# apache/cloudberry

Measured on NVIDIA H100. Metric: TPC-H SF100 Q1 rows/sec, higher is better.
Workload: dtype int64

## Files before the change

### cloudberry_b200/capi.py

```python
import ctypes as C
import os
import re

import numpy as np

from . import plan as P
from .relation import HostRelation, NP_DTYPE

HERE = os.path.dirname(os.path.abspath(__file__))
ROOT = os.path.dirname(HERE)
_GPU = None
_EXEC = None


class CbgpuError(RuntimeError):
    def __init__(self, code, msg):
        super().__init__("cbgpu error %d: %s" % (code, msg))
        self.code = code


class CbgpuVisimapEntry(C.Structure):
    _fields_ = [("first_row_num", C.c_int64), ("data", C.c_void_p), ("len", C.c_int32)]


# ... 222 lines not shown
    global _GPU
    if _GPU is None:
        so = os.path.join(os.environ.get("CBGPU_LIBDIR") or HERE, "libcbgpu.so")
        if not os.path.exists(so):
            raise CbgpuError(-1, "libcbgpu.so is not built (run __graft_entry__.build()); there is no CPU fallback")
        _preload_bundled_nccl()
        L = C.CDLL(so, mode=C.RTLD_GLOBAL)
        vp, i32, i64, u64, dbl = C.c_void_p, C.c_int32, C.c_int64, C.c_uint64, C.c_double
        sig = {
            "cbgpu_ctx_create": (C.c_int, [C.c_int, C.POINTER(vp)]),
            "cbgpu_ctx_destroy": (None, [vp]),
            "cbgpu_last_error": (C.c_char_p, [vp]),
            "cbgpu_sync": (C.c_int, [vp]),
            "cbgpu_check_status": (C.c_int, [vp]),
            "cbgpu_device_count": (C.c_int, []),
            "cbgpu_sm_count": (C.c_int, [vp]),
            "cbgpu_kernel_launches": (i64, [vp]),
            "cbgpu_timer_start": (C.c_int, [vp]),
            "cbgpu_timer_stop_ms": (C.c_int, [vp, C.POINTER(dbl)]),
            "cbgpu_last_kernel_ms": (dbl, [vp]),
            "cbgpu_last_kernel_name": (C.c_char_p, [vp]),
            "cbgpu_kernel_log_reset": (None, [vp]),
            "cbgpu_kernel_log_longest": (C.c_int, [vp, C.c_char_p, C.c_int, C.POINTER(dbl)]),
            "cbgpu_trace_begin": (C.c_int, [vp]),
            "cbgpu_trace_end": (C.c_int, [vp]),
            "cbgpu_trace_get": (C.c_int, [vp, C.c_int, C.c_char_p, C.c_int, C.POINTER(dbl)]),
            "cbgpu_flush_l2": (C.c_int, [vp]),
            "cbgpu_host_alloc": (vp, [C.c_size_t]),
            "cbgpu_host_free": (None, [vp]),
            "cbgpu_hashbpchar": (C.c_uint32, [C.c_char_p, i32]),
            "cbgpu_rel_create": (C.c_int, [vp, i64, i32, C.POINTER(i32), C.POINTER(i32), C.POINTER(vp)]),
            "cbgpu_rel_free": (None, [vp]),
            "cbgpu_rel_nrows": (i64, [vp]),
            "cbgpu_rel_ncols": (i32, [vp]),
            "cbgpu_rel_col_type": (i32, [vp, i32]),
            "cbgpu_rel_col_dscale": (i32, [vp, i32]),
            "cbgpu_rel_load_column": (C.c_int, [vp, i32, vp, vp]),
            "cbgpu_rel_load_column_narrow": (C.c_int, [vp, i32, vp, i32]),
            "cbgpu_rel_read_column": (C.c_int, [vp, i32, i64, i64, vp, vp]),
            "cbgpu_rel_set_visimap": (C.c_int, [vp, vp]),
            "cbgpu_rel_read_visimap": (C.c_int, [vp, vp]),
            "cbgpu_dict_create": (C.c_int, [vp, i32, i64, i32, C.POINTER(vp)]),
            "cbgpu_dict_free": (None, [vp]),
            "cbgpu_aocs_dict_collect": (C.c_int, [vp, vp, i64, i32, i32, i32, vp]),
            "cbgpu_dict_finalize": (C.c_int, [vp, C.POINTER(i32)]),
            "cbgpu_dict_entry": (C.c_int, [vp, i32, C.POINTER(C.c_char_p), C.POINTER(i32)]),
            "cbgpu_dict_lookup": (i32, [vp, C.c_char_p, i32]),
            "cbgpu_aocs_decode_dict_column": (C.c_int, [vp, vp, i64, i32, i32, i32, vp, vp, i32, i64, C.POINTER(i64)]),
            "cbgpu_aocs_apply_visimap": (C.c_int, [vp, vp, i64, i32, vp, i32, vp, i64, C.POINTER(i64)]),
            "cbgpu_rel_set_dict_hash": (C.c_int, [vp, i32, vp, i32]),
            "cbgpu_rel_set_nrows": (C.c_int, [vp, i64]),
            "cbgpu_rel_copy_rows": (C.c_int, [vp, i64, vp, i64, i64]),
            "cbgpu_rel_col_devptr": (vp, [vp, i32]),
            "cbgpu_rel_nbytes": (C.c_size_t, [vp]),
            "cbgpu_ht_build": (C.c_int, [vp, vp, C.POINTER(i32), i32, C.POINTER(vp)]),
            "cbgpu_ht_free": (None, [vp]),
            "cbgpu_ht_nrows": (i64, [vp]),
            "cbgpu_ht_has_duplicates": (C.c_int, [vp]),
            "cbgpu_ht_probe_pairs": (C.c_int, [vp, vp, vp, C.POINTER(i32), i32, vp, i64, vp]),
            "cbgpu_pairs_free": (None, [vp]),
            "cbgpu_merge_sorted_runs": (C.c_int, [vp, vp, C.POINTER(i32), C.POINTER(i32), C.POINTER(i32), i32, i32, C.POINTER(vp),
                                                  C.POINTER(i32)]),
            "cbgpu_dev_free": (None, [vp, vp]),
            "cbgpu_read_u32": (C.c_int, [vp, vp, i64, vp]),
            "cbgpu_motion_unique_id": (C.c_int, [vp]),
            "cbgpu_motion_create": (C.c_int, [vp, C.c_int, C.c_int, vp, C.POINTER(vp)]),
            "cbgpu_motion_create_boot": (C.c_int, [vp, C.c_int, C.c_int, vp, vp, C.POINTER(vp)]),
            "cbgpu_motion_destroy": (None, [vp]),
            "cbgpu_motion_abort": (None, [vp]),
            "cbgpu_motion_host_syncs": (i64, [vp]),
            "cbgpu_motion_collectives": (i64, [vp]),
            "cbgpu_motion_bytes_sent": (i64, [vp]),
            "cbgpu_motion_direct_bytes": (i64, [vp]),
            "cbgpu_motion_direct_available": (C.c_int, [vp]),
            "cbgpu_gen_lineitem": (C.c_int, [vp, vp, u64, i64, i64, i64]),
            "cbgpu_gen_orders": (C.c_int, [vp, vp, u64, i64, i64]),
            "cbgpu_gen_customer": (C.c_int, [vp, vp, u64]),
            "cbgpu_gen_supplier": (C.c_int, [vp, vp, u64]),
            "cbgpu_aocs_decode_column": (C.c_int, [vp, vp, i64, i32, i32, i32, i32, vp, i32, i64, C.POINTER(i64)]),
            "cbgpu_aocs_decode_column_ex": (C.c_int, [vp, vp, i64, i32, i32, i32, i32, i32, vp, i32, i64, C.POINTER(i64)]),
            "cbgpu_gen_customer_range": (C.c_int, [vp, vp, u64, i64]),
            "cbgpu_gen_supplier_range": (C.c_int, [vp, vp, u64, i64]),
            "cbgpu_gen_ssb_lineorder": (C.c_int, [vp, vp, u64, i64, i64, i64, i64]),
        }
        for name, (res, args) in sig.items():
            f = getattr(L, name)
            f.restype = res
            f.argtypes = args
        _GPU = L
    return _GPU


def ex():
    global _EXEC
    if _EXEC is None:
        gpu()
        so = os.path.join(os.environ.get("CBGPU_LIBDIR") or HERE, "libcbexec.so")
        if not os.path.exists(so):
            raise CbgpuError(-1, "libcbexec.so is not built (run __graft_entry__.build())")
        L = C.CDLL(so)
        vp = C.c_void_p
        L.cb_CreateExecutorState.restype = C.POINTER(CbEState)
        L.cb_CreateExecutorState.argtypes = [vp, C.POINTER(vp), C.c_int32]
        L.cb_FreeExecutorState.argtypes = [C.POINTER(CbEState)]
        L.cb_estate_error.restype = C.c_char_p
        L.cb_estate_error.argtypes = [C.POINTER(CbEState)]
# ... 474 lines not shown
```

### cloudberry_b200/csrc/agg.cu

```cuda
#include "common.cuh"

#include <stdlib.h>

static int64_t
next_pow2(int64_t v)
{
	int64_t		p = 1;

	while (p < v)
		p <<= 1;
	return p;
}

struct AggKinds
{
	int32_t		k[CBP_MAX_AGGS];
};

__global__ void
k_agg_init(AggDev t, const AggKinds kk)
{
	const int32_t *kinds = kk.k;
	size_t		cap = (size_t) t.mask + 1;
	size_t		i = (size_t) blockIdx.x * blockDim.x + threadIdx.x;
// ... 403 lines not shown
	int			rc = cbgpu_agg_ngroups(t, &ng);
	int32_t		types[CBP_MAX_KEYS + CBP_MAX_AGGS * 3];
	int			ncols = t->d.nkeys + t->d.naccs * 3;
	cbgpu_rel  *rel;
	AggRelOut	o;
	int			h_flag = 0;

	if (rc)
		return rc;
	for (int k = 0; k < t->d.nkeys; k++)
		types[k] = keytypes[k];
	for (int a = 0; a < t->d.naccs * 3; a++)
		types[t->d.nkeys + a] = CB_INT8;
	rc = cbgpu_rel_create(ctx, ng, ncols, types, NULL, &rel);
	if (rc)
		return rc;
	memset(&o, 0, sizeof(o));
	int			blocks = (int) ((t->capacity + 255) / 256);

	if (blocks > ctx->sm_count * 8)
		blocks = ctx->sm_count * 8;
	h_flag = t->anynull;
	for (int k = 0; k < t->d.nkeys; k++)
	{
		o.key[k] = rel->data[k];
		o.keytype[k] = keytypes[k];
		if (h_flag && ng > 0)
		{
			CB_CUDA(ctx, cudaMallocAsync(&rel->nulls[k], (size_t) ng, ctx->stream));
			o.keynulls[k] = rel->nulls[k];
		}
	}
	for (int a = 0; a < t->d.naccs * 3; a++)
		o.acc[a] = (int64_t *) rel->data[t->d.nkeys + a];
	CB_CUDA(ctx, cudaMallocAsync(&o.counter, sizeof(int32_t), ctx->stream));
	CB_CUDA(ctx, cudaMemsetAsync(o.counter, 0, sizeof(int32_t), ctx->stream));
	if (ng > 0)
	{
		k_agg_to_rel<<<blocks, 256, 0, ctx->stream>>>(t->d, o);
		CB_LAUNCHED(ctx, "k_agg_to_rel");
	}
	CB_CUDA(ctx, cudaFreeAsync(o.counter, ctx->stream));
	*out = rel;
	return CBGPU_OK;
}

#define TOPN_MAXK 64
#define TOPN_MAXKEYS 4

struct TopnParams
{
	const void *key[TOPN_MAXKEYS];
	int32_t		keytype[TOPN_MAXKEYS];
	int32_t		desc[TOPN_MAXKEYS];
	int32_t		uns[TOPN_MAXKEYS];
	int32_t		nkeys;
	int32_t		k;
	const uint32_t *in_idx;
	int64_t		nin;
	uint32_t   *out_idx;
};

__device__ __forceinline__ bool
topn_before(const TopnParams &p, const int64_t *ka, uint32_t ra, const int64_t *kb, uint32_t rb)
{
	for (int i = 0; i < p.nkeys; i++)
	{
		int64_t		x = ka[i],
					y = kb[i];

		if (x == y)
			continue;
		bool		lt = p.uns[i] ? ((uint64_t) x < (uint64_t) y) : (x < y);

		return p.desc[i] ? !lt : lt;
	}
	return ra < rb;
}

__global__ void
k_topn(TopnParams p)
{
	uint32_t	best_row[TOPN_MAXK];
	int64_t		best_key[TOPN_MAXK][TOPN_MAXKEYS];
	int			nbest = 0;
	int64_t		tid = (int64_t) blockIdx.x * blockDim.x + threadIdx.x;
	int64_t		stride = (int64_t) gridDim.x * blockDim.x;

	for (int64_t i = tid; i < p.nin; i += stride)
	{
		uint32_t	row = p.in_idx ? p.in_idx[i] : (uint32_t) i;
		int64_t		key[TOPN_MAXKEYS];

		if (row == 0xFFFFFFFFu)
			continue;
		for (int k = 0; k < p.nkeys; k++)
			key[k] = cb_load_widen(p.key[k], p.keytype[k], row);
		if (nbest == p.k && !topn_before(p, key, row, best_key[nbest - 1], best_row[nbest - 1]))
			continue;
		int			pos = nbest < p.k ? nbest : p.k - 1;

		while (pos > 0 && topn_before(p, key, row, best_key[pos - 1], best_row[pos - 1]))
		{
			best_row[pos] = best_row[pos - 1];
			for (int k = 0; k < p.nkeys; k++)
				best_key[pos][k] = best_key[pos - 1][k];
			pos--;
		}
		best_row[pos] = row;
		for (int k = 0; k < p.nkeys; k++)
			best_key[pos][k] = key[k];
		if (nbest < p.k)
			nbest++;
	}
	for (int j = 0; j < p.k; j++)
		p.out_idx[tid * p.k + j] = j < nbest ? best_row[j] : 0xFFFFFFFFu;
}

#define TOPN_BLOCKS 1024
#define TOPN_CAND 4096

__device__ __forceinline__ unsigned long long
topn_ukey(const TopnParams &p, int i, uint32_t row)
{
	unsigned long long u = (unsigned long long) cb_load_widen(p.key[i], p.keytype[i], row);

	if (!p.uns[i])
		u ^= 0x8000000000000000ull;
	return p.desc[i] ? ~u : u;
}

__global__ void __launch_bounds__(256)
k_topn_min(TopnParams p, int keyi, unsigned long long *bmin, unsigned long long *bmax)
{
	__shared__ unsigned long long smin[8], smax[8];
	unsigned long long lo = ~0ull,
				hi = 0;

	for (int64_t i = (int64_t) blockIdx.x * blockDim.x + threadIdx.x; i < p.nin; i += (int64_t) gridDim.x * blockDim.x)
	{
		const unsigned long long u = topn_ukey(p, keyi, (uint32_t) i);

		lo = u < lo ? u : lo;
		hi = u > hi ? u : hi;
	}
	for (int o = 16; o > 0; o >>= 1)
	{
		const unsigned long long a = __shfl_xor_sync(0xffffffffu, lo, o);
		const unsigned long long b = __shfl_xor_sync(0xffffffffu, hi, o);

		lo = a < lo ? a : lo;
		hi = b > hi ? b : hi;
	}
	if ((threadIdx.x & 31) == 0)
	{
		smin[threadIdx.x >> 5] = lo;
		smax[threadIdx.x >> 5] = hi;
	}
	__syncthreads();
	if (threadIdx.x == 0)
	{
		for (int w = 1; w < 8; w++)
		{
			lo = smin[w] < lo ? smin[w] : lo;
			hi = smax[w] > hi ? smax[w] : hi;
		}
		bmin[blockIdx.x] = lo;
		bmax[blockIdx.x] = hi;
	}
}

__global__ void __launch_bounds__(TOPN_BLOCKS)
k_topn_kth(const unsigned long long *bmin, const unsigned long long *bmax, int nblocks, int k, unsigned long long *out)
{
	__shared__ unsigned long long v[TOPN_BLOCKS];
	__shared__ unsigned long long gmax;
	const int	t = threadIdx.x;

// ... 14 lines not shown

			if (partner > t)
			{
				const bool	up = (t & size) == 0;
				const unsigned long long a = v[t],
							b = v[partner];

				if ((a > b) == up)
				{
					v[t] = b;
					v[partner] = a;
				}
			}
			__syncthreads();
		}
	if (t == 0)
	{
		out[0] = nblocks >= k ? v[k - 1] : gmax;
		out[1] = v[0];
		out[2] = gmax;
	}
}

__global__ void __launch_bounds__(256)
k_topn_filter(TopnParams p, int keyi, const unsigned long long *thr, uint32_t *cand, int *ncand)
{
	const unsigned long long T = thr[0];

	for (int64_t i = (int64_t) blockIdx.x * blockDim.x + threadIdx.x; i < p.nin; i += (int64_t) gridDim.x * blockDim.x)
		if (topn_ukey(p, keyi, (uint32_t) i) <= T)
		{
			const int	pos = atomicAdd(ncand, 1);

			if (pos < TOPN_CAND)
				cand[pos] = (uint32_t) i;
		}
}

__global__ void __launch_bounds__(1024)
k_topn_final(TopnParams p, const uint32_t *cand, const int *ncand, int64_t nall, uint32_t *out)
{
	const int	m = cand ? (*ncand < TOPN_CAND ? *ncand : TOPN_CAND) : (int) nall;

	for (int j = threadIdx.x; j < p.k; j += blockDim.x)
		out[j] = 0xFFFFFFFFu;
	__syncthreads();
	for (int i = threadIdx.x; i < m; i += blockDim.x)
	{
		const uint32_t ri = cand ? cand[i] : (uint32_t) i;
		int64_t		ki[TOPN_MAXKEYS];
		int			rank = 0;

		for (int k = 0; k < p.nkeys; k++)
			ki[k] = cb_load_widen(p.key[k], p.keytype[k], ri);
		for (int j = 0; j < m && rank < p.k; j++)
		{
			const uint32_t rj = cand ? cand[j] : (uint32_t) j;
			int64_t		kj[TOPN_MAXKEYS];

			if (j == i)
				continue;
			for (int k = 0; k < p.nkeys; k++)
				kj[k] = cb_load_widen(p.key[k], p.keytype[k], rj);
			rank += topn_before(p, kj, rj, ki, ri);
		}
		if (rank < p.k)
			out[rank] = ri;
	}
}

#define MERGE_MAXRUNS 64

struct MergeParams
{
	const void *key[TOPN_MAXKEYS];
	const uint8_t *nulls[TOPN_MAXKEYS];
	int32_t		keytype[TOPN_MAXKEYS];
	int32_t		desc[TOPN_MAXKEYS];
	int32_t		uns[TOPN_MAXKEYS];
	int32_t		nkeys;
	int32_t		nruns;
	int64_t		n;
	int64_t		start[MERGE_MAXRUNS + 1];
	int32_t    *nfound;
	unsigned long long *found;
	uint32_t   *order;
};

__device__ __forceinline__ int
merge_cmp(const MergeParams &p, int64_t a, int64_t b)
{
	for (int i = 0; i < p.nkeys; i++)
	{
		const bool	an = p.nulls[i] && p.nulls[i][a];
		const bool	bn = p.nulls[i] && p.nulls[i][b];
		int			c;

		if (an || bn)
			c = (an && bn) ? 0 : (an ? 1 : -1);
		else
		{
			const int64_t x = cb_load_widen(p.key[i], p.keytype[i], (uint32_t) a);
			const int64_t y = cb_load_widen(p.key[i], p.keytype[i], (uint32_t) b);

			if (x == y)
				c = 0;
			else if (p.uns[i])
				c = (uint64_t) x < (uint64_t) y ? -1 : 1;
			else
				c = x < y ? -1 : 1;
		}
		if (p.desc[i])
			c = -c;
		if (c)
			return c;
	}
	return 0;
}

__global__ void
k_merge_find_runs(MergeParams p)
{
	int64_t		i = (int64_t) blockIdx.x * blockDim.x + threadIdx.x + 1;
	const int64_t stride = (int64_t) gridDim.x * blockDim.x;

	for (; i < p.n; i += stride)
		if (merge_cmp(p, i, i - 1) < 0)
		{
			const int	at = atomicAdd(p.nfound, 1);

			if (at < MERGE_MAXRUNS)
				p.found[at] = (unsigned long long) i;
		}
}

__global__ void
k_merge_place(MergeParams p)
{
	int64_t		i = (int64_t) blockIdx.x * blockDim.x + threadIdx.x;
	const int64_t stride = (int64_t) gridDim.x * blockDim.x;

	for (; i < p.n; i += stride)
	{
		int			r = 0;
		int64_t		pos;

		while (r + 1 < p.nruns && p.start[r + 1] <= i)
			r++;
		pos = i - p.start[r];
		for (int q = 0; q < p.nruns; q++)
		{
			int64_t		lo = p.start[q],
						hi = p.start[q + 1];

			if (q == r)
				continue;
			while (lo < hi)
			{
				const int64_t mid = lo + (hi - lo) / 2;
				const int	c = merge_cmp(p, mid, i);

				if (c < 0 || (c == 0 && q < r))
					lo = mid + 1;
				else
					hi = mid;
			}
			pos += lo - p.start[q];
		}
		p.order[pos] = (uint32_t) i;
	}
}

extern "C" int
cbgpu_merge_sorted_runs(cbgpu_ctx *ctx, cbgpu_rel *rel, const int32_t *keycols, const int32_t *descending, const int32_t *unsigned_cmp,
						int32_t nkeys, int32_t max_runs, uint32_t **order_dev, int32_t *nruns_out)
{
	MergeParams p;
	int32_t		nfound = 0;
	unsigned long long found[MERGE_MAXRUNS];
	int			blocks;

	*order_dev = NULL;
	if (nruns_out)
		*nruns_out = rel->nrows > 0;
	if (nkeys < 1 || nkeys > TOPN_MAXKEYS || max_runs < 1 || max_runs > MERGE_MAXRUNS)
		return cb_fail(ctx, CBGPU_ERR_UNSUPPORTED, "merge receive supports 1..4 sort keys and up to 64 senders (%s got %lld keys)", "", nkeys);
	memset(&p, 0, sizeof(p));
	for (int i = 0; i < nkeys; i++)
	{
		if (keycols[i] < 0 || keycols[i] >= rel->ncols)
			return cb_fail(ctx, CBGPU_ERR_INVALID, "cbgpu_merge_sorted_runs: bad key column%s %lld", "", keycols[i]);
		p.key[i] = rel->data[keycols[i]];
		p.nulls[i] = rel->nulls[keycols[i]];
		p.keytype[i] = rel->types[keycols[i]];
		p.desc[i] = descending[i];
		p.uns[i] = unsigned_cmp ? unsigned_cmp[i] : 0;
		if (p.keytype[i] == CB_FLOAT8)
			return cb_fail(ctx, CBGPU_ERR_UNSUPPORTED, "merge receive over a float8 key%s", "", 0);
	}
	p.nkeys = nkeys;
	p.n = rel->nrows;
	if (rel->nrows < 2)
		return CBGPU_OK;
	blocks = (int) ((rel->nrows + 255) / 256);
	if (blocks > ctx->sm_count * 8)
		blocks = ctx->sm_count * 8;
	CB_CUDA(ctx, cudaMallocAsync(&p.nfound, sizeof(int32_t) + MERGE_MAXRUNS * sizeof(unsigned long long) + 8, ctx->stream));
	p.found = (unsigned long long *) ((char *) p.nfound + 8);
	CB_CUDA(ctx, cudaMemsetAsync(p.nfound, 0, sizeof(int32_t), ctx->stream));
	k_merge_find_runs<<<blocks, 256, 0, ctx->stream>>>(p);
	CB_LAUNCHED(ctx, "k_merge_find_runs");
	CB_CUDA(ctx, cudaMemcpyAsync(&nfound, p.nfound, sizeof(int32_t), cudaMemcpyDeviceToHost, ctx->stream));
	CB_CUDA(ctx, cudaMemcpyAsync(found, p.found, sizeof(found), cudaMemcpyDeviceToHost, ctx->stream));
	CB_CUDA(ctx, cudaStreamSynchronize(ctx->stream));
	CB_CUDA(ctx, cudaFreeAsync(p.nfound, ctx->stream));
	if (nfound + 1 > max_runs)
		return cb_fail(ctx, CBGPU_ERR_INVALID, "merge receive: %s%lld sorted runs arrived from fewer senders - a sender's stream is not in the Motion's sort order",
					   "", (long long) nfound + 1);
	if (nruns_out)
		*nruns_out = nfound + 1;
	if (nfound == 0)
		return CBGPU_OK;
	for (int a = 1; a < nfound; a++)
		for (int b = a; b > 0 && found[b] < found[b - 1]; b--)
		{
			unsigned long long t = found[b];

			found[b] = found[b - 1];
			found[b - 1] = t;
		}
	p.nruns = nfound + 1;
	p.start[0] = 0;
	for (int a = 0; a < nfound; a++)
		p.start[a + 1] = (int64_t) found[a];
	p.start[p.nruns] = rel->nrows;
	CB_CUDA(ctx, cudaMallocAsync(&p.order, (size_t) rel->nrows * sizeof(uint32_t), ctx->stream));
	k_merge_place<<<blocks, 256, 0, ctx->stream>>>(p);
	CB_LAUNCHED(ctx, "k_merge_place");
	*order_dev = p.order;
	return CBGPU_OK;
}

extern "C" int
cbgpu_topn(cbgpu_ctx *ctx, cbgpu_rel *rel, const int32_t *keycols, const int32_t *descending, const int32_t *unsigned_cmp,
		   int32_t nkeys, int64_t limit, uint32_t *host_idx, int64_t *nout)
{
	TopnParams	p;
	uint32_t   *cand1 = NULL,
			   *cand2 = NULL;
	int64_t		n1,
				n2;

	if (nkeys < 1 || nkeys > TOPN_MAXKEYS || limit < 1 || limit > TOPN_MAXK)
		return cb_fail(ctx, CBGPU_ERR_UNSUPPORTED, "device top-N supports 1..4 sort keys and LIMIT <= 64 (%s got %lld)", "", limit);
	memset(&p, 0, sizeof(p));
	for (int i = 0; i < nkeys; i++)
	{
		if (keycols[i] < 0 || keycols[i] >= rel->ncols)
			return cb_fail(ctx, CBGPU_ERR_INVALID, "cbgpu_topn: bad key column%s %lld", "", keycols[i]);
		if (rel->nulls[keycols[i]])
			return cb_fail(ctx, CBGPU_ERR_UNSUPPORTED, "device top-N over a nullable sort key (%s column %lld)", "", keycols[i]);
		p.key[i] = rel->data[keycols[i]];
		p.keytype[i] = rel->types[keycols[i]];
		p.desc[i] = descending[i];
		p.uns[i] = unsigned_cmp ? unsigned_cmp[i] : 0;
		if (p.keytype[i] == CB_FLOAT8)
			return cb_fail(ctx, CBGPU_ERR_UNSUPPORTED, "device top-N over a float8 key%s", "", 0);
	}
	p.nkeys = nkeys;
	p.k = (int32_t) limit;
	*nout = 0;
	if (rel->nrows == 0)
		return CBGPU_OK;
	{
		unsigned long long *scratch = NULL;
		uint32_t   *cand = NULL;
		int		   *ncand = NULL;
		unsigned long long h3[3];
		int			hn = 0;
		bool		done = false;

		p.in_idx = NULL;
		p.nin = rel->nrows;
		CB_CUDA(ctx, cudaMallocAsync(&cand1, (TOPN_MAXK + 1) * sizeof(uint32_t), ctx->stream));
		if (rel->nrows <= TOPN_CAND)
		{
			k_topn_final<<<1, 1024, 0, ctx->stream>>>(p, NULL, NULL, rel->nrows, cand1);
			CB_LAUNCHED(ctx, "k_topn_final");
			done = true;
		}
		else
		{
			int			nblocks = (int) ((rel->nrows + 63) / 64);

			if (nblocks > TOPN_BLOCKS)
				nblocks = TOPN_BLOCKS;
			CB_CUDA(ctx, cudaMallocAsync(&scratch, (2 * TOPN_BLOCKS + 3) * sizeof(unsigned long long), ctx->stream));
			CB_CUDA(ctx, cudaMallocAsync(&cand, TOPN_CAND * sizeof(uint32_t), ctx->stream));
			CB_CUDA(ctx, cudaMallocAsync(&ncand, sizeof(int), ctx->stream));
			for (int keyi = 0; keyi < nkeys && !done; keyi++)
			{
				k_topn_min<<<nblocks, 256, 0, ctx->stream>>>(p, keyi, scratch, scratch + TOPN_BLOCKS);
				CB_LAUNCHED(ctx, "k_topn_min");
				k_topn_kth<<<1, TOPN_BLOCKS, 0, ctx->stream>>>(scratch, scratch + TOPN_BLOCKS, nblocks, p.k, scratch + 2 * TOPN_BLOCKS);
				CB_LAUNCHED(ctx, "k_topn_kth");
				CB_CUDA(ctx, cudaMemcpyAsync(h3, scratch + 2 * TOPN_BLOCKS, sizeof(h3), cudaMemcpyDeviceToHost, ctx->stream));
				CB_CUDA(ctx, cudaStreamSynchronize(ctx->stream));
				if (h3[1] == h3[2])
					continue;
				CB_CUDA(ctx, cudaMemsetAsync(ncand, 0, sizeof(int), ctx->stream));
				k_topn_filter<<<nblocks, 256, 0, ctx->stream>>>(p, keyi, scratch + 2 * TOPN_BLOCKS, cand, ncand);
				CB_LAUNCHED(ctx, "k_topn_filter");
				CB_CUDA(ctx, cudaMemcpyAsync(&hn, ncand, sizeof(int), cudaMemcpyDeviceToHost, ctx->stream));
				CB_CUDA(ctx, cudaStreamSynchronize(ctx->stream));
				if (hn <= TOPN_CAND)
				{
// ... 68 lines not shown
```

### cloudberry_b200/csrc/aocs.cu

```cuda
#include "common.cuh"
#include "inflate.cuh"
#include "zstd_dec.cuh"

#include <stdlib.h>
#include <string.h>

struct AocsDir
{
	long long	hoff;
	int32_t		overall;
	int32_t		clen;
	long long	zoff;
	long long	off;
	long long	rowbase;
	long long	first;
	int32_t		rows;
	int32_t		dlen;
};

struct DictSlot
{
	unsigned long long tag;
	uint32_t	off;
	uint32_t	len;
// ... 1227 lines not shown
	int32_t		finalized;
	int32_t		n;
	char	   *texts;
	uint32_t   *off, *len;
	int32_t    *sorted;
};

static int	aocs_decode_impl(cbgpu_ctx *ctx, const void *file_bytes, int64_t nbytes, int32_t checksum, int32_t compress_kind, int32_t attlen,
							 int32_t varkind, int32_t typalign, cbgpu_rel *rel, int32_t col, int64_t row_offset, int64_t *nrows_out,
							 const cbgpu_dict *dict, int dmode);

extern "C" int
cbgpu_aocs_decode_column_ex(cbgpu_ctx *ctx, const void *file_bytes, int64_t nbytes, int32_t checksum, int32_t compress_kind,
							int32_t attlen, int32_t varkind, int32_t typalign, cbgpu_rel *rel, int32_t col, int64_t row_offset,
							int64_t *nrows_out)
{
	if (varkind == CBGPU_AOCS_VAR_DICT)
		return cb_fail(ctx, CBGPU_ERR_INVALID, "dictionary columns are decoded by cbgpu_aocs_decode_dict_column%s (%lld)", "", varkind);
	return aocs_decode_impl(ctx, file_bytes, nbytes, checksum, compress_kind, attlen, varkind, typalign, rel, col, row_offset, nrows_out,
							NULL, 0);
}

static int
aocs_decode_impl(cbgpu_ctx *ctx, const void *file_bytes, int64_t nbytes, int32_t checksum, int32_t compress_kind, int32_t attlen,
				 int32_t varkind, int32_t typalign, cbgpu_rel *rel, int32_t col, int64_t row_offset, int64_t *nrows_out,
				 const cbgpu_dict *dict, int dmode)
{
	const uint8_t *raw = (const uint8_t *) file_bytes;
	AocsDir    *dir = NULL;
	AocsWalk	W;
	int64_t		ndir = 0,
				rows = 0,
				ztotal = 0,
				ncompressed = 0;
	bool		anynull = false;
	int		   *d_flag = NULL;
	uint8_t    *d_scratch = NULL;
	AocsParams	P;
	uint8_t    *d_raw = NULL;
	AocsDir    *d_dir = NULL;
	int			outw;
	int			nblk;

	*nrows_out = 0;
	if (dmode != 1)
	{
		if (col < 0 || col >= rel->ncols)
			return cb_fail(ctx, CBGPU_ERR_INVALID, "cbgpu_aocs_decode_column: bad column%s %lld", "", col);
		outw = cb_type_w(rel->types[col]);
		if (attlen > 0 ? (attlen != outw || (attlen != 1 && attlen != 2 && attlen != 4 && attlen != 8))
			: !((varkind == CBGPU_AOCS_VAR_NUMERIC && rel->types[col] == CB_NUMERIC) || (varkind == CBGPU_AOCS_VAR_BPCHAR1 && outw == 1) ||
				(varkind == CBGPU_AOCS_VAR_DICT && (rel->types[col] == CB_DICT8 || rel->types[col] == CB_DICT32))))
			return cb_fail(ctx, CBGPU_ERR_UNSUPPORTED, "AOCS column of length %s%lld does not decode into this relation column", "", attlen);
	}
	else
		outw = 0;
	if (typalign != 1 && typalign != 2 && typalign != 4 && typalign != 8)
		return cb_fail(ctx, CBGPU_ERR_INVALID, "type alignment %s%lld", "", typalign);
	{
		const int	rc = aocs_walk(ctx, raw, nbytes, checksum, compress_kind < 0 ? 0 : compress_kind, row_offset, &W);

		if (rc)
			return rc;
		dir = W.dir;
		ndir = W.ndir;
		rows = W.rows;
		ztotal = W.ztotal;
		ncompressed = W.ncompressed;
		anynull = W.anynull;
	}
	if (dmode != 1 && (row_offset < 0 || row_offset + rows > rel->capacity))
	{
		free(dir);
		return cb_fail(ctx, CBGPU_ERR_INVALID, "AOCS column file holds %s%lld rows: more than the relation has room for", "", rows);
	}
	if (ndir == 0)
	{
		free(dir);
		return CBGPU_OK;
	}
	CB_CUDA(ctx, cudaSetDevice(ctx->device));
	CB_CUDA(ctx, cudaMallocAsync(&d_raw, (size_t) ((nbytes + 15) / 16 * 16 + ztotal + 16), ctx->stream));
	CB_CUDA(ctx, cudaMallocAsync(&d_dir, sizeof(AocsDir) * (size_t) ndir, ctx->stream));
	CB_CUDA(ctx, cudaMemcpyAsync(d_raw, raw, (size_t) nbytes, cudaMemcpyHostToDevice, ctx->stream));
	CB_CUDA(ctx, cudaMemcpyAsync(d_dir, dir, sizeof(AocsDir) * (size_t) ndir, cudaMemcpyHostToDevice, ctx->stream));
	if (ctx->trace_on)
		cb_trace_mark(ctx, "aocs:h2d");
	nblk = (int) ((ndir + AOCS_WARPS - 1) / AOCS_WARPS);
	if (nblk > ctx->sm_count * 16)
		nblk = ctx->sm_count * 16;
	if (checksum)
	{
		k_aocs_verify<<<nblk, AOCS_WARPS * 32, 0, ctx->stream>>>(d_raw, d_dir, (int) ndir, ctx->d_status);
		CB_LAUNCHED(ctx, "k_aocs_verify");
	}
	if (ncompressed)
	{
		int			flag = 0;

		CB_CUDA(ctx, cudaMallocAsync(&d_flag, sizeof(int), ctx->stream));
		CB_CUDA(ctx, cudaMemsetAsync(d_flag, 0, sizeof(int), ctx->stream));
		if (compress_kind == CBGPU_AOCS_COMPRESS_ZSTD)
		{
			const int	zblk = nblk < ctx->sm_count * 4 ? nblk : ctx->sm_count * 4;

			CB_CUDA(ctx, cudaMallocAsync(&d_scratch, (size_t) zblk * AOCS_WARPS * ZSTD_SCRATCH, ctx->stream));
// ... 586 lines not shown
```

### cloudberry_b200/csrc/common.cuh

```cuda
#pragma once

#include <cuda_runtime.h>
#include <stdint.h>
#include <stdio.h>
#include <string.h>

#include "../../include/cbgpu.h"

#include <stdlib.h>
#include <string.h>

#define CB_MAX_COLS_REL 64

struct cbgpu_ctx
{
	int			device;
	cudaStream_t stream;
	char		err[512];
	int			sm_count;
	int64_t		launches;
	cudaEvent_t ev_t0, ev_t1, ev_k0, ev_k1;
	double		last_kernel_ms;
	const char *last_kernel_name;
	bool		kernel_timed;
// ... 14 lines not shown
	int64_t		status_seen_at;
	bool		opt_debug, opt_no_early_filter, opt_no_keyslot, opt_no_fuse0, opt_no_spec0, opt_no_smem_ht, opt_l2_direct, opt_no_prefilter, opt_prefilter_tma, opt_pf_spec, opt_pf_occ6;
	int			opt_bloom_div;
	int			opt_htb_u;
#define CB_SCRATCH_SLOTS 8
	void	   *scratch[CB_SCRATCH_SLOTS];
	size_t		scratch_bytes[CB_SCRATCH_SLOTS];
#define CB_EARLY_CACHE 16
	struct
	{
		const void *keydata;
		int64_t		nrows;
		const void *red0;
		int			worth;
	}			early_cache[CB_EARLY_CACHE];
	int			early_cache_n;
	uint64_t	pf_cache[32];
	int			pf_cache_n;
	int			opt_pf_keep_div;
	int64_t		opt_pf_min_rows;
	struct AggSnap *agg_snap;
	void	   *small_dev;
	size_t		small_dev_bytes;
};

static inline void *
cb_scratch(cbgpu_ctx *ctx, int slot, size_t bytes)
{
	if (ctx->scratch_bytes[slot] < bytes)
	{
		free(ctx->scratch[slot]);
		ctx->scratch[slot] = malloc(bytes);
		ctx->scratch_bytes[slot] = ctx->scratch[slot] ? bytes : 0;
	}
	if (ctx->scratch[slot])
		memset(ctx->scratch[slot], 0, bytes);
	return ctx->scratch[slot];
}

struct cbgpu_rel
{
	cbgpu_ctx  *ctx;
	int64_t		nrows;
	int64_t		capacity;
	int32_t		ncols;
	int32_t		types[CB_MAX_COLS_REL];
	int32_t		dscales[CB_MAX_COLS_REL];
	void	   *data[CB_MAX_COLS_REL];
	uint8_t	   *nulls[CB_MAX_COLS_REL];
	uint32_t   *dict_hash[CB_MAX_COLS_REL];
	int32_t		dict_n[CB_MAX_COLS_REL];
	uint8_t	   *visimap;
	bool		owns[CB_MAX_COLS_REL];
	void	   *slab;
};

struct AggDev
{
	uint32_t	mask;
	int32_t		nkeys;
	int32_t		naccs;
	int32_t		npart;
	int32_t		part_shift;
	int32_t		part_id;
	int32_t    *state;
	uint32_t   *hash;
	int64_t    *keys;
	uint32_t   *keynull;
	int64_t    *n;
	unsigned long long *sum;
	int32_t    *ngroups;
	int32_t    *full;
};

#define AGG_SNAP_MAXG 64
#define AGG_SNAP_MAXCAP 4096
struct AggSnap
{
	int32_t		ngroups;
	int32_t		full;
	int32_t		anynull;
	int32_t		retry;
	int32_t		audit;
	int32_t		pad[3];
	uint32_t	keynull[AGG_SNAP_MAXG];
	int64_t		keys[AGG_SNAP_MAXG][CBP_MAX_KEYS];
	int64_t		n[AGG_SNAP_MAXG][CBP_MAX_AGGS];
	int64_t		lo[AGG_SNAP_MAXG][CBP_MAX_AGGS];
	int64_t		hi[AGG_SNAP_MAXG][CBP_MAX_AGGS];
};

struct cbgpu_aggtable
{
	cbgpu_ctx  *ctx;
	AggDev		d;
	void	   *base;
	int64_t		capacity;
	int32_t		kinds[CBP_MAX_AGGS];
	bool		counted;
	int64_t		ngroups;
	int32_t		anynull;
	bool		snap_valid;
	AggSnap    *snap;
};

#ifdef __CUDACC__
// ... 429 lines not shown
	asm volatile("ld.global.nc.L1::no_allocate.L2::cache_hint.u64 %0, [%1], %2;" : "=l"(v) : "l"(a), "l"(pol));
	return v;
}
#endif

#ifdef __CUDACC__
__device__ __forceinline__ uint32_t
smem_u32(const void *p)
{
	return (uint32_t) __cvta_generic_to_shared(p);
}

__device__ __forceinline__ void
mbar_init(uint64_t *bar, unsigned count)
{
	asm volatile("mbarrier.init.shared::cta.b64 [%0], %1;" :: "r"(smem_u32(bar)), "r"(count));
}

__device__ __forceinline__ void
mbar_expect_tx(uint64_t *bar, unsigned bytes)
{
	asm volatile("mbarrier.arrive.expect_tx.shared::cta.b64 _, [%0], %1;" :: "r"(smem_u32(bar)), "r"(bytes) : "memory");
}

__device__ __forceinline__ void
mbar_arrive(uint64_t *bar)
{
	asm volatile("mbarrier.arrive.shared::cta.b64 _, [%0];" :: "r"(smem_u32(bar)) : "memory");
}

__device__ __forceinline__ void
mbar_wait(uint64_t *bar, unsigned parity)
{
	asm volatile(
		"{\n"
		".reg .pred p;\n"
		"WAIT_%=:\n"
		"mbarrier.try_wait.parity.shared::cta.b64 p, [%0], %1;\n"
		"@p bra DONE_%=;\n"
		"bra WAIT_%=;\n"
		"DONE_%=:\n"
		"}\n" :: "r"(smem_u32(bar)), "r"(parity) : "memory");
}

__device__ __forceinline__ void
tma_load_1d(void *dst, const void *src, unsigned bytes, uint64_t *bar)
{
	asm volatile("cp.async.bulk.shared::cluster.global.mbarrier::complete_tx::bytes [%0], [%1], %2, [%3];"
				 :: "r"(smem_u32(dst)), "l"(src), "r"(bytes), "r"(smem_u32(bar)) : "memory");
}

#endif

__device__ __forceinline__ int64_t
cb_load_widen(const void *data, int type, uint32_t row)
{
	switch (type)
	{
		case CB_INT4: case CB_DATE: case CB_DICT32:
			return (int64_t) __ldg((const int32_t *) data + row);
		case CB_INT8: case CB_NUMERIC: case CB_FLOAT8:
			return __ldg((const long long *) data + row);
		default:
			return (int64_t) __ldg((const uint8_t *) data + row);
	}
}

__device__ __forceinline__ void
atomic_add128(unsigned long long *acc, unsigned long long lo, unsigned long long hi)
{
	if (lo)
	{
		unsigned long long old = atomicAdd(acc, lo);

		if (old + lo < old)
			hi += 1;
	}
	if (hi)
		atomicAdd(acc + 1, hi);
}

__device__ __forceinline__ void
atomic_add128_signed(unsigned long long *acc, long long v)
{
	atomic_add128(acc, (unsigned long long) v, v < 0 ? ~0ull : 0ull);
}

__device__ __forceinline__ int
agg_find_or_insert(const AggDev &t, uint32_t hash, const int64_t *keys, uint32_t nullmask)
{
	uint32_t	pos = hash & t.mask;
	uint32_t	probes = 0;
	int			result = -2;

	while (result == -2)
	{
		int			s = *((volatile int *) (t.state + pos));

		if (s == 0)
		{
			s = atomicCAS(t.state + pos, 0, 1);
			if (s == 0)
			{
				for (int k = 0; k < t.nkeys; k++)
					t.keys[(size_t) pos * t.nkeys + k] = keys[k];
				t.keynull[pos] = nullmask;
				t.hash[pos] = hash;
				__threadfence();
				*((volatile int *) (t.state + pos)) = 2;
				result = (int) pos;
			}
		}
		if (result == -2 && s == 2)
		{
			bool		same = false;

			__threadfence();
			if (*((volatile uint32_t *) (t.hash + pos)) == hash && *((volatile uint32_t *) (t.keynull + pos)) == nullmask)
			{
// ... 19 lines not shown
```

### cloudberry_b200/csrc/ctx.cu

```cuda
#include "common.cuh"

#include <nvtx3/nvToolsExt.h>

#include <stdlib.h>

extern "C" int
cbgpu_device_count(void)
{
	int			n = 0;

	if (cudaGetDeviceCount(&n) != cudaSuccess)
		return 0;
	return n;
}

extern "C" int
cbgpu_ctx_create(int device, cbgpu_ctx **out)
{
	cbgpu_ctx  *ctx = (cbgpu_ctx *) calloc(1, sizeof(cbgpu_ctx));
	cudaDeviceProp prop;

	if (!ctx)
		return CBGPU_ERR_NOMEM;
	*out = ctx;
	ctx->device = device;
	CB_CUDA(ctx, cudaSetDevice(device));
	CB_CUDA(ctx, cudaGetDeviceProperties(&prop, device));
	ctx->sm_count = prop.multiProcessorCount;
	CB_CUDA(ctx, cudaStreamCreateWithFlags(&ctx->stream, cudaStreamNonBlocking));
	{
		cudaMemPool_t pool;
		unsigned long long keep = ~0ull;

		CB_CUDA(ctx, cudaDeviceGetDefaultMemPool(&pool, device));
		CB_CUDA(ctx, cudaMemPoolSetAttribute(pool, cudaMemPoolAttrReleaseThreshold, &keep));
	}
	CB_CUDA(ctx, cudaEventCreate(&ctx->ev_t0));
	CB_CUDA(ctx, cudaEventCreate(&ctx->ev_t1));
	CB_CUDA(ctx, cudaEventCreate(&ctx->ev_k0));
	CB_CUDA(ctx, cudaEventCreate(&ctx->ev_k1));
	CB_CUDA(ctx, cudaMalloc(&ctx->d_status, sizeof(int)));
	CB_CUDA(ctx, cudaMemsetAsync(ctx->d_status, 0, sizeof(int), ctx->stream));
	CB_CUDA(ctx, cudaMallocHost(&ctx->h_status, sizeof(int)));
	*ctx->h_status = 0;
	CB_CUDA(ctx, cudaMallocHost(&ctx->agg_snap, sizeof(AggSnap)));
	memset(ctx->agg_snap, 0, sizeof(AggSnap));
	ctx->opt_debug = getenv("CBGPU_DEBUG") != NULL;
	ctx->opt_no_early_filter = getenv("CBGPU_NO_EARLY_FILTER") != NULL;
	ctx->opt_no_keyslot = getenv("CBGPU_NO_KEYSLOT") != NULL;
	ctx->opt_no_fuse0 = getenv("CBGPU_NO_FUSE0") != NULL;
	ctx->opt_no_spec0 = getenv("CBGPU_SPEC0") == NULL;
	ctx->opt_no_smem_ht = getenv("CBGPU_NO_SMEM_HT") != NULL;
	ctx->opt_no_prefilter = getenv("CBGPU_NO_PREFILTER") != NULL;
// ... 280 lines not shown
{
	void	   *p = NULL;

	if (cudaMallocHost(&p, bytes ? bytes : 1) != cudaSuccess)
		return NULL;
	return p;
}

extern "C" void
cbgpu_host_free(void *p)
{
	if (p)
		cudaFreeHost(p);
}

extern "C" uint32_t
cbgpu_hashbpchar(const char *s, int32_t len)
{
	while (len > 0 && s[len - 1] == ' ')
		len--;
	return pg_hash_bytes_host((const unsigned char *) s, len);
}

extern "C" int
cbgpu_rel_create(cbgpu_ctx *ctx, int64_t nrows, int32_t ncols, const int32_t *types, const int32_t *dscales,
				 cbgpu_rel **out)
{
	cbgpu_rel  *r;

	if (ncols < 0 || ncols > CB_MAX_COLS_REL || nrows < 0 || nrows > 0xFFFFFFF0ll)
		return cb_fail(ctx, CBGPU_ERR_INVALID, "cbgpu_rel_create: bad shape (%s nrows=%lld)", "", nrows);
	r = (cbgpu_rel *) calloc(1, sizeof(cbgpu_rel));
	if (!r)
		return CBGPU_ERR_NOMEM;
	r->ctx = ctx;
	r->nrows = nrows;
	r->capacity = nrows;
	r->ncols = ncols;
	CB_CUDA(ctx, cudaSetDevice(ctx->device));
	size_t		total = 0;
	size_t		colbytes[CB_MAX_COLS_REL];

	for (int i = 0; i < ncols; i++)
	{
		size_t		bytes = (size_t) (nrows ? nrows : 1) * cb_type_w(types[i]);

		if (cb_type_w(types[i]) == 0)
		{
			free(r);
			return cb_fail(ctx, CBGPU_ERR_INVALID, "cbgpu_rel_create: bad column type%s %lld", "", types[i]);
		}
		r->types[i] = types[i];
		r->dscales[i] = dscales ? dscales[i] : 0;
		colbytes[i] = (bytes + 255) & ~(size_t) 255;
		total += colbytes[i];
	}
	if (ncols > 1 && total <= ((size_t) 64 << 20))
	{
		char	   *base;

		CB_CUDA(ctx, cudaMallocAsync(&base, total, ctx->stream));
		r->slab = base;
		for (int i = 0; i < ncols; i++)
		{
			r->data[i] = base;
			r->owns[i] = false;
			base += colbytes[i];
		}
	}
	else
		for (int i = 0; i < ncols; i++)
		{
			CB_CUDA(ctx, cudaMallocAsync(&r->data[i], colbytes[i], ctx->stream));
			r->owns[i] = true;
		}
	*out = r;
	return CBGPU_OK;
}

extern "C" void
cbgpu_rel_free(cbgpu_rel *rel)
{
	if (!rel)
		return;
	cudaSetDevice(rel->ctx->device);
	for (int i = 0; i < rel->ncols; i++)
	{
		if (rel->owns[i] && rel->data[i])
			cudaFreeAsync(rel->data[i], rel->ctx->stream);
		if (rel->nulls[i])
			cudaFreeAsync(rel->nulls[i], rel->ctx->stream);
		if (rel->dict_hash[i] && rel->dict_n[i] >= 0)
			cudaFreeAsync(rel->dict_hash[i], rel->ctx->stream);
	}
	if (rel->visimap)
		cudaFreeAsync(rel->visimap, rel->ctx->stream);
	if (rel->slab)
		cudaFreeAsync(rel->slab, rel->ctx->stream);
	free(rel);
}

extern "C" int64_t
cbgpu_rel_nrows(const cbgpu_rel *rel)
{
	return rel->nrows;
}

extern "C" int32_t
cbgpu_rel_ncols(const cbgpu_rel *rel)
{
	return rel->ncols;
}

extern "C" int32_t
cbgpu_rel_col_type(const cbgpu_rel *rel, int32_t col)
{
	return (col >= 0 && col < rel->ncols) ? rel->types[col] : 0;
}

extern "C" int32_t
cbgpu_rel_col_dscale(const cbgpu_rel *rel, int32_t col)
{
	return (col >= 0 && col < rel->ncols) ? rel->dscales[col] : 0;
}

extern "C" int
cbgpu_rel_load_column(cbgpu_rel *rel, int32_t col, const void *host, const uint8_t *nulls)
{
	cbgpu_ctx  *ctx = rel->ctx;

	if (col < 0 || col >= rel->ncols)
		return cb_fail(ctx, CBGPU_ERR_INVALID, "cbgpu_rel_load_column: bad column%s %lld", "", col);
	if (rel->nrows == 0)
		return CBGPU_OK;
	CB_CUDA(ctx, cudaMemcpyAsync(rel->data[col], host, (size_t) rel->nrows * cb_type_w(rel->types[col]),
								 cudaMemcpyHostToDevice, ctx->stream));
	if (nulls)
	{
		if (!rel->nulls[col])
			CB_CUDA(ctx, cudaMallocAsync(&rel->nulls[col], (size_t) rel->capacity, ctx->stream));
		CB_CUDA(ctx, cudaMemcpyAsync(rel->nulls[col], nulls, (size_t) rel->nrows, cudaMemcpyHostToDevice, ctx->stream));
	}
	else if (rel->nulls[col])
	{
		cudaFreeAsync(rel->nulls[col], ctx->stream);
		rel->nulls[col] = NULL;
	}
	return CBGPU_OK;
}

template <typename NARROW, typename WIDE>
__global__ void
k_widen(const NARROW *__restrict__ src, WIDE *__restrict__ dst, int64_t n)
{
	int64_t		i = (int64_t) blockIdx.x * blockDim.x + threadIdx.x;
	const int64_t stride = (int64_t) gridDim.x * blockDim.x;

	for (; i < n; i += stride)
		dst[i] = (WIDE) src[i];
}

extern "C" int
cbgpu_rel_load_column_narrow(cbgpu_rel *rel, int32_t col, const void *host, int32_t host_width)
{
	cbgpu_ctx  *ctx = rel->ctx;
	void	   *stage;
	int			w;
	int			blocks;

	if (col < 0 || col >= rel->ncols)
		return cb_fail(ctx, CBGPU_ERR_INVALID, "cbgpu_rel_load_column_narrow: bad column%s %lld", "", col);
	w = cb_type_w(rel->types[col]);
	if (host_width == w)
		return cbgpu_rel_load_column(rel, col, host, NULL);
	if (rel->types[col] == CB_FLOAT8 || (w != 8 && w != 4) || (host_width != 1 && host_width != 2 && host_width != 4) || host_width > w)
		return cb_fail(ctx, CBGPU_ERR_INVALID, "cbgpu_rel_load_column_narrow: a %s%lld-byte host column cannot be widened into this column", "", host_width);
	if (rel->nrows == 0)
		return CBGPU_OK;
	CB_CUDA(ctx, cudaMallocAsync(&stage, (size_t) rel->nrows * host_width, ctx->stream));
	CB_CUDA(ctx, cudaMemcpyAsync(stage, host, (size_t) rel->nrows * host_width, cudaMemcpyHostToDevice, ctx->stream));
	blocks = ctx->sm_count * 8;
	if (w == 8)
	{
		if (host_width == 1)
			k_widen<int8_t, int64_t><<<blocks, 256, 0, ctx->stream>>>((const int8_t *) stage, (int64_t *) rel->data[col], rel->nrows);
		else if (host_width == 2)
			k_widen<int16_t, int64_t><<<blocks, 256, 0, ctx->stream>>>((const int16_t *) stage, (int64_t *) rel->data[col], rel->nrows);
		else
			k_widen<int32_t, int64_t><<<blocks, 256, 0, ctx->stream>>>((const int32_t *) stage, (int64_t *) rel->data[col], rel->nrows);
	}
	else
	{
		if (host_width == 1)
			k_widen<int8_t, int32_t><<<blocks, 256, 0, ctx->stream>>>((const int8_t *) stage, (int32_t *) rel->data[col], rel->nrows);
		else
			k_widen<int16_t, int32_t><<<blocks, 256, 0, ctx->stream>>>((const int16_t *) stage, (int32_t *) rel->data[col], rel->nrows);
	}
	CB_LAUNCHED(ctx, "k_widen");
	CB_CUDA(ctx, cudaFreeAsync(stage, ctx->stream));
	return CBGPU_OK;
}

extern "C" int
cbgpu_rel_read_column(cbgpu_rel *rel, int32_t col, int64_t lo, int64_t hi, void *host, uint8_t *nulls)
{
	cbgpu_ctx  *ctx = rel->ctx;
	int			w;

	if (col < 0 || col >= rel->ncols || lo < 0 || hi > rel->nrows || lo > hi)
		return cb_fail(ctx, CBGPU_ERR_INVALID, "cbgpu_rel_read_column: bad range%s %lld", "", lo);
	w = cb_type_w(rel->types[col]);
	if (hi > lo)
	{
		CB_CUDA(ctx, cudaMemcpyAsync(host, (char *) rel->data[col] + (size_t) lo * w, (size_t) (hi - lo) * w,
									 cudaMemcpyDeviceToHost, ctx->stream));
		if (nulls)
		{
			if (rel->nulls[col])
				CB_CUDA(ctx, cudaMemcpyAsync(nulls, rel->nulls[col] + lo, (size_t) (hi - lo), cudaMemcpyDeviceToHost, ctx->stream));
			else
				memset(nulls, 0, (size_t) (hi - lo));
		}
	}
	CB_CUDA(ctx, cudaStreamSynchronize(ctx->stream));
	return CBGPU_OK;
}

struct ReadRows
{
	const void *data[CB_MAX_COLS_REL];
	const uint8_t *nulls[CB_MAX_COLS_REL];
	int32_t		types[CB_MAX_COLS_REL];
	int32_t		ncols;
	const uint32_t *idx;
	int64_t		n;
	long long  *out;
	uint8_t    *outnull;
};

__global__ void
k_read_rows(ReadRows p)
{
	const int64_t total = p.n * p.ncols;

	for (int64_t i = (int64_t) blockIdx.x * blockDim.x + threadIdx.x; i < total; i += (int64_t) gridDim.x * blockDim.x)
	{
		const int64_t r = i / p.ncols;
		const int	c = (int) (i % p.ncols);
		const uint32_t row = p.idx ? p.idx[r] : (uint32_t) r;

		p.out[i] = cb_load_widen(p.data[c], p.types[c], row);
		p.outnull[i] = p.nulls[c] ? p.nulls[c][row] : (uint8_t) 0;
	}
}

extern "C" int
cbgpu_rel_read_rows(cbgpu_rel *rel, const uint32_t *host_idx, int64_t n, int64_t *out, uint8_t *outnull)
{
	cbgpu_ctx  *ctx = rel->ctx;
	ReadRows	p;
	uint32_t   *d_idx = NULL;
	char	   *d_buf = NULL;
	const int64_t total = n * rel->ncols;

	if (n < 0 || (!host_idx && n > rel->nrows) || rel->ncols > CB_MAX_COLS_REL)
		return cb_fail(ctx, CBGPU_ERR_INVALID, "cbgpu_rel_read_rows: bad row count%s %lld", "", n);
	if (total == 0)
		return CBGPU_OK;
	for (int64_t r = 0; host_idx && r < n; r++)
		if ((int64_t) host_idx[r] >= rel->nrows)
			return cb_fail(ctx, CBGPU_ERR_INVALID, "cbgpu_rel_read_rows: row %s%lld out of range", "", (long long) host_idx[r]);
	memset(&p, 0, sizeof(p));
	for (int c = 0; c < rel->ncols; c++)
	{
		p.data[c] = rel->data[c];
		p.nulls[c] = rel->nulls[c];
		p.types[c] = rel->types[c];
	}
	p.ncols = rel->ncols;
	p.n = n;
	CB_CUDA(ctx, cudaSetDevice(ctx->device));
	CB_CUDA(ctx, cudaMallocAsync(&d_buf, (size_t) total * 9, ctx->stream));
	p.out = (long long *) d_buf;
	p.outnull = (uint8_t *) (d_buf + (size_t) total * 8);
	if (host_idx)
	{
		CB_CUDA(ctx, cudaMallocAsync(&d_idx, (size_t) n * sizeof(uint32_t), ctx->stream));
		CB_CUDA(ctx, cudaMemcpyAsync(d_idx, host_idx, (size_t) n * sizeof(uint32_t), cudaMemcpyHostToDevice, ctx->stream));
		p.idx = d_idx;
	}
	{
		int			blocks = (int) ((total + 255) / 256);

		if (blocks > ctx->sm_count * 8)
			blocks = ctx->sm_count * 8;
		k_read_rows<<<blocks, 256, 0, ctx->stream>>>(p);
		CB_LAUNCHED(ctx, "k_read_rows");
	}
	CB_CUDA(ctx, cudaMemcpyAsync(out, p.out, (size_t) total * 8, cudaMemcpyDeviceToHost, ctx->stream));
	CB_CUDA(ctx, cudaMemcpyAsync(outnull, p.outnull, (size_t) total, cudaMemcpyDeviceToHost, ctx->stream));
	CB_CUDA(ctx, CB_STATUS_RIDE(ctx));
	CB_CUDA(ctx, cudaStreamSynchronize(ctx->stream));
	CB_STATUS_FETCHED(ctx);
	CB_CUDA(ctx, cudaFreeAsync(d_buf, ctx->stream));
	if (d_idx)
		CB_CUDA(ctx, cudaFreeAsync(d_idx, ctx->stream));
	return CBGPU_OK;
}

extern "C" int
cbgpu_rel_set_visimap(cbgpu_rel *rel, const uint8_t *bits)
{
	cbgpu_ctx  *ctx = rel->ctx;
	size_t		bytes = (size_t) ((rel->nrows + 7) / 8);

	if (!bits)
	{
		if (rel->visimap)
		{
			cudaFreeAsync(rel->visimap, ctx->stream);
			rel->visimap = NULL;
		}
		return CBGPU_OK;
	}
	if (!rel->visimap)
		CB_CUDA(ctx, cudaMallocAsync(&rel->visimap, ((bytes + 255) & ~(size_t) 255) + 256, ctx->stream));
	CB_CUDA(ctx, cudaMemcpyAsync(rel->visimap, bits, bytes, cudaMemcpyHostToDevice, ctx->stream));
	return CBGPU_OK;
}

// ... 2 lines not shown
{
	cbgpu_ctx  *ctx = rel->ctx;
	const size_t bytes = (size_t) ((rel->nrows + 7) / 8);

	if (!rel->visimap)
	{
		memset(bits, 0xFF, bytes);
		return CBGPU_OK;
	}
	CB_CUDA(ctx, cudaMemcpyAsync(bits, rel->visimap, bytes, cudaMemcpyDeviceToHost, ctx->stream));
	CB_CUDA(ctx, cudaStreamSynchronize(ctx->stream));
	return CBGPU_OK;
}

extern "C" int
cbgpu_rel_set_dict_hash(cbgpu_rel *rel, int32_t col, const uint32_t *hashes, int32_t n)
{
	cbgpu_ctx  *ctx = rel->ctx;

	if (col < 0 || col >= rel->ncols || n <= 0)
		return cb_fail(ctx, CBGPU_ERR_INVALID, "cbgpu_rel_set_dict_hash: bad argument%s %lld", "", col);
	if (rel->dict_hash[col])
	{
		cudaFreeAsync(rel->dict_hash[col], ctx->stream);
	}
	CB_CUDA(ctx, cudaMallocAsync(&rel->dict_hash[col], (size_t) n * sizeof(uint32_t), ctx->stream));
	CB_CUDA(ctx, cudaMemcpyAsync(rel->dict_hash[col], hashes, (size_t) n * sizeof(uint32_t), cudaMemcpyHostToDevice, ctx->stream));
	CB_CUDA(ctx, cudaStreamSynchronize(ctx->stream));
	rel->dict_n[col] = n;
	return CBGPU_OK;
}

extern "C" int
cbgpu_rel_set_nrows(cbgpu_rel *rel, int64_t nrows)
{
	if (nrows < 0 || nrows > rel->capacity)
		return cb_fail(rel->ctx, CBGPU_ERR_INVALID, "cbgpu_rel_set_nrows: beyond capacity%s %lld", "", nrows);
	rel->nrows = nrows;
	return CBGPU_OK;
}

extern "C" void *
cbgpu_rel_col_devptr(cbgpu_rel *rel, int32_t col)
{
	return (col >= 0 && col < rel->ncols) ? rel->data[col] : NULL;
}

extern "C" size_t
cbgpu_rel_nbytes(const cbgpu_rel *rel)
{
	size_t		b = 0;

	for (int i = 0; i < rel->ncols; i++)
		b += (size_t) rel->nrows * cb_type_w(rel->types[i]);
	return b;
}

extern "C" int
cbgpu_read_u32(cbgpu_ctx *ctx, const uint32_t *dev, int64_t n, uint32_t *host)
{
	if (n > 0)
		CB_CUDA(ctx, cudaMemcpyAsync(host, dev, (size_t) n * sizeof(uint32_t), cudaMemcpyDeviceToHost, ctx->stream));
	CB_CUDA(ctx, cudaStreamSynchronize(ctx->stream));
	return CBGPU_OK;
}

extern "C" int
cbgpu_dev_alloc(cbgpu_ctx *ctx, size_t bytes, void **dev)
{
	CB_CUDA(ctx, cudaSetDevice(ctx->device));
	CB_CUDA(ctx, cudaMallocAsync(dev, bytes ? bytes : 8, ctx->stream));
	CB_CUDA(ctx, cudaMemsetAsync(*dev, 0, bytes ? bytes : 8, ctx->stream));
	return CBGPU_OK;
}

extern "C" int
cbgpu_dev_read(cbgpu_ctx *ctx, const void *dev, size_t bytes, void *host)
{
	CB_CUDA(ctx, cudaMemcpyAsync(host, dev, bytes, cudaMemcpyDeviceToHost, ctx->stream));
	CB_CUDA(ctx, CB_STATUS_RIDE(ctx));
	CB_CUDA(ctx, cudaStreamSynchronize(ctx->stream));
	CB_STATUS_FETCHED(ctx);
	return CBGPU_OK;
}

extern "C" int
cbgpu_dev_write(cbgpu_ctx *ctx, void *dev, size_t bytes, const void *host)
{
	CB_CUDA(ctx, cudaMemcpyAsync(dev, host, bytes, cudaMemcpyHostToDevice, ctx->stream));
	CB_CUDA(ctx, cudaStreamSynchronize(ctx->stream));
	return CBGPU_OK;
}

extern "C" void
cbgpu_dev_free(cbgpu_ctx *ctx, void *dev)
{
	if (!dev)
		return;
	cudaSetDevice(ctx->device);
	cudaFreeAsync(dev, ctx->stream);
}

extern "C" int
cbgpu_rel_add_nullmap(cbgpu_rel *rel, int32_t col)
{
	cbgpu_ctx  *ctx = rel->ctx;

	if (col < 0 || col >= rel->ncols)
		return cb_fail(ctx, CBGPU_ERR_INVALID, "cbgpu_rel_add_nullmap: bad column%s %lld", "", col);
	if (rel->nulls[col])
		return CBGPU_OK;
	CB_CUDA(ctx, cudaMallocAsync(&rel->nulls[col], (size_t) (rel->capacity ? rel->capacity : 1), ctx->stream));
	CB_CUDA(ctx, cudaMemsetAsync(rel->nulls[col], 0, (size_t) (rel->capacity ? rel->capacity : 1), ctx->stream));
	return CBGPU_OK;
}

extern "C" int
cbgpu_rel_copy_rows(cbgpu_rel *dst, int64_t dst_lo, cbgpu_rel *src, int64_t src_lo, int64_t n)
{
	cbgpu_ctx  *ctx = dst->ctx;

	if (dst->ncols != src->ncols || dst_lo < 0 || src_lo < 0 || dst_lo + n > dst->capacity || src_lo + n > src->capacity)
		return cb_fail(ctx, CBGPU_ERR_INVALID, "cbgpu_rel_copy_rows: shape / range mismatch%s (%lld rows)", "", n);
	if (n == 0)
		return CBGPU_OK;
	for (int c = 0; c < dst->ncols; c++)
	{
		int			w = cb_type_w(dst->types[c]);

		if (dst->types[c] != src->types[c])
			return cb_fail(ctx, CBGPU_ERR_INVALID, "cbgpu_rel_copy_rows: column %s%lld type mismatch", "", c);
		CB_CUDA(ctx, cudaMemcpyAsync((char *) dst->data[c] + (size_t) dst_lo * w, (char *) src->data[c] + (size_t) src_lo * w,
									 (size_t) n * w, cudaMemcpyDeviceToDevice, ctx->stream));
		if (src->nulls[c])
		{
			int			rc = cbgpu_rel_add_nullmap(dst, c);

			if (rc)
				return rc;
			CB_CUDA(ctx, cudaMemcpyAsync(dst->nulls[c] + dst_lo, src->nulls[c] + src_lo, (size_t) n, cudaMemcpyDeviceToDevice, ctx->stream));
		}
	}
	return CBGPU_OK;
}

struct TakeRows
{
	const void *src[CB_MAX_COLS_REL];
	void	   *dst[CB_MAX_COLS_REL];
	const uint8_t *snull[CB_MAX_COLS_REL];
	uint8_t    *dnull[CB_MAX_COLS_REL];
	int32_t		width[CB_MAX_COLS_REL];
	int32_t		ncols;
	int64_t		n;
	const uint32_t *idx;
};

__global__ void
k_take_rows(TakeRows p)
{
	int64_t		i = (int64_t) blockIdx.x * blockDim.x + threadIdx.x;
	const int64_t stride = (int64_t) gridDim.x * blockDim.x;

	for (; i < p.n; i += stride)
	{
		const uint32_t r = p.idx[i];

		for (int c = 0; c < p.ncols; c++)
		{
			switch (p.width[c])
			{
				case 1: ((uint8_t *) p.dst[c])[i] = ((const uint8_t *) p.src[c])[r]; break;
				case 4: ((uint32_t *) p.dst[c])[i] = ((const uint32_t *) p.src[c])[r]; break;
				case 16: ((uint4 *) p.dst[c])[i] = ((const uint4 *) p.src[c])[r]; break;
				default: ((unsigned long long *) p.dst[c])[i] = ((const unsigned long long *) p.src[c])[r]; break;
			}
			if (p.dnull[c])
				p.dnull[c][i] = p.snull[c][r];
		}
	}
}

extern "C" int
cbgpu_rel_take_rows(cbgpu_rel *dst, cbgpu_rel *src, const uint32_t *dev_idx, int64_t n)
{
	cbgpu_ctx  *ctx = dst->ctx;
	TakeRows	p;

	if (dst->ncols != src->ncols || n < 0 || n > dst->capacity || dst->ncols > CB_MAX_COLS_REL)
		return cb_fail(ctx, CBGPU_ERR_INVALID, "cbgpu_rel_take_rows: shape / range mismatch%s (%lld rows)", "", n);
	if (n == 0)
		return CBGPU_OK;
	memset(&p, 0, sizeof(p));
	for (int c = 0; c < dst->ncols; c++)
	{
		if (dst->types[c] != src->types[c])
			return cb_fail(ctx, CBGPU_ERR_INVALID, "cbgpu_rel_take_rows: column %s%lld type mismatch", "", c);
		if (src->nulls[c])
		{
			int			rc = cbgpu_rel_add_nullmap(dst, c);

			if (rc)
				return rc;
		}
		p.src[c] = src->data[c];
		p.dst[c] = dst->data[c];
		p.snull[c] = src->nulls[c];
		p.dnull[c] = src->nulls[c] ? dst->nulls[c] : NULL;
		p.width[c] = cb_type_w(dst->types[c]);
	}
	p.ncols = dst->ncols;
	p.n = n;
	p.idx = dev_idx;
	{
		int			blocks = (int) ((n + 255) / 256);

		if (blocks > ctx->sm_count * 8)
			blocks = ctx->sm_count * 8;
		k_take_rows<<<blocks, 256, 0, ctx->stream>>>(p);
		CB_LAUNCHED(ctx, "k_take_rows");
	}
	if (dst->nrows < n)
		dst->nrows = n;
	return CBGPU_OK;
}

extern "C" int
cbgpu_rel_has_nulls(const cbgpu_rel *rel, int32_t col)
{
	return (col >= 0 && col < rel->ncols && rel->nulls[col]) ? 1 : 0;
}

extern "C" const uint32_t *
cbgpu_rel_dict_hash_dev(const cbgpu_rel *rel, int32_t col)
{
	return (col >= 0 && col < rel->ncols) ? rel->dict_hash[col] : NULL;
}

extern "C" const uint8_t *
cbgpu_rel_nulls_dev(const cbgpu_rel *rel, int32_t col)
{
	return (col >= 0 && col < rel->ncols) ? rel->nulls[col] : NULL;
}

extern "C" const uint8_t *
cbgpu_rel_visimap_dev(const cbgpu_rel *rel)
{
	return rel->visimap;
}

extern "C" int
cbgpu_rel_share_dict_hash(cbgpu_rel *dst, int32_t dcol, const cbgpu_rel *src, int32_t scol)
{
	if (dcol < 0 || dcol >= dst->ncols || scol < 0 || scol >= src->ncols)
		return cb_fail(dst->ctx, CBGPU_ERR_INVALID, "cbgpu_rel_share_dict_hash: bad column%s %lld", "", dcol);
	dst->dict_hash[dcol] = src->dict_hash[scol];
	dst->dict_n[dcol] = src->dict_n[scol] > 0 ? -src->dict_n[scol] : (src->dict_n[scol] < 0 ? src->dict_n[scol] : -1);
	return CBGPU_OK;
}
```

### cloudberry_b200/csrc/exec/cb_aocs_load.c

```c
#include "../../../include/cb_exec.h"

#include <errno.h>
#include <fcntl.h>
#include <stdio.h>
#include <stdlib.h>
#include <string.h>
#include <sys/stat.h>
#include <unistd.h>

#define CB_AOCS_FILENUM_MULT 128
#define CB_AOCS_MAX_SEGNO 127

int
cb_aocs_segfile_path(const char *basepath, int segno, int filenum, char *out, size_t outsz)
{
	int			pseudo;
	int			n;

	if (!basepath || !out || segno < 0 || segno > CB_AOCS_MAX_SEGNO || filenum < 1)
		return -1;
	pseudo = (filenum - 1) * CB_AOCS_FILENUM_MULT + segno;
	if (pseudo > 0)
		n = snprintf(out, outsz, "%s.%u", basepath, (unsigned) pseudo);
	else
// ... 94 lines not shown
	if (nrows_out)
		*nrows_out = 0;
	if (nhidden_out)
		*nhidden_out = 0;
	if (err && errsz)
		err[0] = 0;
	if (ncols < 1 || !cols)
		return load_fail(err, errsz, CBGPU_ERR_INVALID, "no columns to load from %s (%lld)", basepath ? basepath : "", (long long) ncols);
	for (int c = 0; c < ncols && rc == CBGPU_OK; c++)
	{
		char		path[4096];
		unsigned char *buf = NULL;
		int64_t		len = 0,
					n = 0;

		if (cb_aocs_segfile_path(basepath, segno, cols[c].filenum, path, sizeof(path)) != 0)
		{
			rc = load_fail(err, errsz, CBGPU_ERR_INVALID, "bad segment file name for %s (column %lld)", basepath ? basepath : "", (long long) c);
			break;
		}
		rc = read_prefix(path, cols[c].eof, &buf, &len, err, errsz);
		if (rc != CBGPU_OK)
			break;
		if (cols[c].varkind == CBGPU_AOCS_VAR_DICT)
			rc = cbgpu_aocs_decode_dict_column(ctx, buf, len, checksum, cols[c].compresstype, cols[c].typalign, cols[c].dict, rel,
											   cols[c].relcol, row_offset, &n);
		else
			rc = cbgpu_aocs_decode_column_ex(ctx, buf, len, checksum, cols[c].compresstype, cols[c].attlen, cols[c].varkind,
											 cols[c].typalign, rel, cols[c].relcol, row_offset, &n);
		if (rc != CBGPU_OK)
		{
			if (err && errsz)
				snprintf(err, errsz, "%s: %s", path, cbgpu_last_error(ctx));
		}
		else if (nrows >= 0 && n != nrows)
			rc = load_fail(err, errsz, CBGPU_ERR_INVALID, "column file %s holds %lld rows, the segment file's other columns differ", path, (long long) n);
		else
			nrows = n;
		if (c == 0 && rc == CBGPU_OK)
		{
			first = buf;
			firstlen = len;
		}
		else
			free(buf);
	}
	if (rc == CBGPU_OK && (nentries > 0 || cbgpu_rel_visimap_dev(rel)) && nrows > 0)
	{
		rc = cbgpu_aocs_apply_visimap(ctx, first, firstlen, checksum, entries, nentries, rel, row_offset, nhidden_out);
		if (rc != CBGPU_OK && err && errsz)
			snprintf(err, errsz, "%s visimap: %s", basepath, cbgpu_last_error(ctx));
	}
	free(first);
	if (rc == CBGPU_OK && nrows_out)
		*nrows_out = nrows < 0 ? 0 : nrows;
	return rc;
}
```

### cloudberry_b200/csrc/exec/cb_exec.c

```c
#include <stdarg.h>
#include <stdio.h>
#include <stdlib.h>
#include <string.h>

#include "../../../include/cb_exec.h"

static int
es_fail(CbEState *es, int code, const char *fmt,...)
{
	va_list		ap;

	if (es->es_errcode == 0)
	{
		va_start(ap, fmt);
		vsnprintf(es->es_errmsg, sizeof(es->es_errmsg), fmt, ap);
		va_end(ap);
		es->es_errcode = code;
		if (es->es_error_hook)
			es->es_error_hook(es, code, es->es_errmsg);
	}
	return code;
}

#define GPU(es, call) \
// ... 147 lines not shown
	int			recv_ready;
	int			xstage;
	PExpr		send_pe[MAX_OUT];
	int			send_nout;
} NodePriv;

static NodePriv *
np(CbPlanState *ps)
{
	return (NodePriv *) ps->priv;
}

static int
pe_add(CbStream *s, const PExpr *e)
{
	for (int i = 0; i < s->npe; i++)
	{
		const PExpr *o = &s->pe[i];

		if (o->kind != e->kind || o->type != e->type || o->dscale != e->dscale)
			continue;
		if (e->kind == PE_COL && o->col == e->col)
			return i;
		if (e->kind == PE_CONST && o->imm == e->imm)
			return i;
		if (e->kind == PE_OP && o->op == e->op && o->l == e->l && o->r == e->r && o->imm == e->imm)
			return i;
		if (e->kind == PE_STATE && o->cn == e->cn && o->clo == e->clo && o->chi == e->chi && o->acckind == e->acckind &&
			o->aggfn == e->aggfn && o->final == e->final)
			return i;
	}
	if (s->npe >= MAX_PE)
		return -1;
	s->pe[s->npe] = *e;
	return s->npe++;
}

static int
stream_add_col(CbStream *s, cbgpu_rel *rel, int col, int src)
{
	const void *data = cbgpu_rel_col_devptr(rel, col);

	for (int i = 0; i < s->pipe.ncols; i++)
		if (s->pipe.cols[i].data == data && s->pipe.cols[i].src == src)
			return i;
	if (s->pipe.ncols >= CBP_MAX_COLS)
		return -1;
	CbpColumn  *c = &s->pipe.cols[s->pipe.ncols];

	c->data = data;
	c->nulls = cbgpu_rel_nulls_dev(rel, col);
	c->dict_hash = cbgpu_rel_dict_hash_dev(rel, col);
	c->type = cbgpu_rel_col_type(rel, col);
	c->src = src;
	s->col_rel[s->pipe.ncols] = rel;
	s->col_idx[s->pipe.ncols] = col;
	return s->pipe.ncols++;
}

static int
pe_col(CbStream *s, cbgpu_rel *rel, int col, int src, int force_nullable)
{
	PExpr		e;
	int			c = stream_add_col(s, rel, col, src);

	if (c < 0)
		return -1;
	memset(&e, 0, sizeof(e));
	e.kind = PE_COL;
	e.type = cbgpu_rel_col_type(rel, col);
	e.dscale = cbgpu_rel_col_dscale(rel, col);
	e.col = c;
	e.maybe_null = force_nullable || cbgpu_rel_has_nulls(rel, col);
	e.l = e.r = -1;
	return pe_add(s, &e);
}

static int
pe_const(CbStream *s, int type, int dscale, int64_t v)
{
	PExpr		e;

	memset(&e, 0, sizeof(e));
	e.kind = PE_CONST;
	e.type = type;
	e.dscale = dscale;
	e.imm = v;
	e.l = e.r = -1;
	return pe_add(s, &e);
}

static int
pe_op(CbStream *s, int op, int l, int r, int type, int dscale, int64_t imm)
{
	PExpr		e;

	memset(&e, 0, sizeof(e));
	e.kind = PE_OP;
	e.op = op;
	e.l = l;
	e.r = r;
	e.imm = imm;
	e.type = type;
	e.dscale = dscale;
	e.maybe_null = (l >= 0 && s->pe[l].maybe_null) || (r >= 0 && s->pe[r].maybe_null);
	return pe_add(s, &e);
// ... 3323 lines not shown
```

### cloudberry_b200/csrc/gen.cu

```cuda
#include "common.cuh"

__host__ __device__ __forceinline__ uint64_t
gen_mix(uint64_t x)
{
	x = (x ^ (x >> 30)) * 0xBF58476D1CE4E5B9ull;
	x = (x ^ (x >> 27)) * 0x94D049BB133111EBull;
	return x ^ (x >> 31);
}

__host__ __device__ __forceinline__ uint64_t
gen_u(uint64_t seed, uint64_t col, uint64_t idx)
{
	return gen_mix(seed * 0x9E3779B97F4A7C15ull + col * 0xD1B54A32D192ED03ull + idx);
}

#define GEN_STARTDATE (-2922)
#define GEN_CURRENTDATE (-1659)
#define GEN_DATE_SPAN 2406

__host__ __device__ __forceinline__ int64_t
gen_order_key(int64_t idx)
{
	return (idx / 8) * 32 + (idx % 8) + 1;
}
// ... 22 lines not shown
	{
		int64_t		j = g.row_lo + i;
		int64_t		oidx = (j / 28) * 7 + off28[j % 28];
		int64_t		odate = GEN_STARTDATE + (int64_t) (gen_u(g.seed, 12, (uint64_t) oidx) % GEN_DATE_SPAN);
		int64_t		qty = 1 + (int64_t) (gen_u(g.seed, 21, (uint64_t) j) % 50);
		int64_t		pk = 1 + (int64_t) (gen_u(g.seed, 22, (uint64_t) j) % g.n_part);
		int64_t		price = 90000 + (pk / 10) % 20001 + 100 * (pk % 1000);
		int64_t		ship = odate + 1 + (int64_t) (gen_u(g.seed, 25, (uint64_t) j) % 121);
		int64_t		receipt = ship + 1 + (int64_t) (gen_u(g.seed, 26, (uint64_t) j) % 30);
		uint8_t		ra = (gen_u(g.seed, 27, (uint64_t) j) % 2 == 0) ? 'R' : 'A';

		g.orderkey[i] = gen_order_key(oidx);
		g.suppkey[i] = (int32_t) (1 + gen_u(g.seed, 23, (uint64_t) j) % g.n_supp);
		g.quantity[i] = qty * 100;
		g.extendedprice[i] = qty * price;
		g.discount[i] = (int64_t) (gen_u(g.seed, 24, (uint64_t) j) % 11);
		g.tax[i] = (int64_t) (gen_u(g.seed, 28, (uint64_t) j) % 9);
		g.returnflag[i] = receipt <= GEN_CURRENTDATE ? ra : (uint8_t) 'N';
		g.linestatus[i] = ship > GEN_CURRENTDATE ? 'O' : 'F';
		g.shipdate[i] = (int32_t) ship;
	}
}

static int
gen_check(cbgpu_ctx *ctx, cbgpu_rel *rel, const int *types, int ncols, const char *name)
{
	if (rel->ncols != ncols)
		return cb_fail(ctx, CBGPU_ERR_INVALID, "generator: relation %s has the wrong column count (%lld)", name, rel->ncols);
	for (int i = 0; i < ncols; i++)
		if (rel->types[i] != types[i])
			return cb_fail(ctx, CBGPU_ERR_INVALID, "generator: relation %s column %lld has the wrong type", name, i);
	return CBGPU_OK;
}

static int
gen_blocks(cbgpu_ctx *ctx, int64_t n)
{
	int64_t		b = (n + 255) / 256;

	if (b > (int64_t) ctx->sm_count * 16)
		b = (int64_t) ctx->sm_count * 16;
	return b < 1 ? 1 : (int) b;
}

extern "C" int
cbgpu_gen_lineitem(cbgpu_ctx *ctx, cbgpu_rel *rel, uint64_t seed, int64_t row_lo, int64_t n_supp, int64_t n_part)
{
	const int	types[9] = {CB_INT8, CB_INT4, CB_NUMERIC, CB_NUMERIC, CB_NUMERIC, CB_NUMERIC, CB_BPCHAR1, CB_BPCHAR1, CB_DATE};
	int			rc = gen_check(ctx, rel, types, 9, "lineitem");
	GenLineitem g;

	if (rc)
		return rc;
	g.orderkey = (int64_t *) rel->data[0];
	g.suppkey = (int32_t *) rel->data[1];
	g.quantity = (int64_t *) rel->data[2];
	g.extendedprice = (int64_t *) rel->data[3];
	g.discount = (int64_t *) rel->data[4];
	g.tax = (int64_t *) rel->data[5];
	g.returnflag = (uint8_t *) rel->data[6];
	g.linestatus = (uint8_t *) rel->data[7];
	g.shipdate = (int32_t *) rel->data[8];
	g.n = rel->nrows;
	g.row_lo = row_lo;
	g.seed = seed;
	g.n_supp = (uint64_t) n_supp;
	g.n_part = (uint64_t) n_part;
	if (rel->nrows == 0)
		return CBGPU_OK;
	k_gen_lineitem<<<gen_blocks(ctx, rel->nrows), 256, 0, ctx->stream>>>(g);
	CB_LAUNCHED(ctx, "k_gen_lineitem");
	return CBGPU_OK;
}

__global__ void
k_gen_orders(int64_t *orderkey, int32_t *custkey, int32_t *orderdate, int32_t *shipprio, int64_t n, int64_t row_lo,
			 uint64_t seed, uint64_t n_cust)
{
	int64_t		i = (int64_t) blockIdx.x * blockDim.x + threadIdx.x;
	int64_t		stride = (int64_t) gridDim.x * blockDim.x;

	for (; i < n; i += stride)
	{
		int64_t		o = row_lo + i;

		orderkey[i] = gen_order_key(o);
		custkey[i] = (int32_t) (1 + gen_u(seed, 11, (uint64_t) o) % n_cust);
		orderdate[i] = (int32_t) (GEN_STARTDATE + (int64_t) (gen_u(seed, 12, (uint64_t) o) % GEN_DATE_SPAN));
		shipprio[i] = 0;
	}
}

extern "C" int
cbgpu_gen_orders(cbgpu_ctx *ctx, cbgpu_rel *rel, uint64_t seed, int64_t row_lo, int64_t n_cust)
{
	const int	types[4] = {CB_INT8, CB_INT4, CB_DATE, CB_INT4};
	int			rc = gen_check(ctx, rel, types, 4, "orders");

	if (rc)
		return rc;
	if (rel->nrows == 0)
		return CBGPU_OK;
	k_gen_orders<<<gen_blocks(ctx, rel->nrows), 256, 0, ctx->stream>>>((int64_t *) rel->data[0], (int32_t *) rel->data[1],
																		  (int32_t *) rel->data[2], (int32_t *) rel->data[3],
																		  rel->nrows, row_lo, seed, (uint64_t) n_cust);
	CB_LAUNCHED(ctx, "k_gen_orders");
	return CBGPU_OK;
}

__global__ void
k_gen_keyed(int32_t *key, int32_t *nation, uint8_t *seg, int64_t n, int64_t row_lo, uint64_t seed, uint64_t col_nation,
			uint64_t col_seg)
{
	int64_t		i = (int64_t) blockIdx.x * blockDim.x + threadIdx.x;
	int64_t		stride = (int64_t) gridDim.x * blockDim.x;

	for (; i < n; i += stride)
	{
		const int64_t r = row_lo + i;

		key[i] = (int32_t) (r + 1);
		nation[i] = (int32_t) (gen_u(seed, col_nation, (uint64_t) r) % 25);
		if (seg)
			seg[i] = (uint8_t) (gen_u(seed, col_seg, (uint64_t) r) % 5);
// ... 134 lines not shown
```

### cloudberry_b200/csrc/hashtable.cu

```cuda
#include "common.cuh"

#include <stdlib.h>

struct BuildParams
{
	HtDev		ht;
	int64_t		nrows;
	int		   *flags;
};

__device__ __forceinline__ bool
ht_row_hash(const HtDev &ht, uint32_t row, uint32_t *hash, int64_t *key0)
{
	uint32_t	h = 0;

	for (int k = 0; k < ht.nkeys; k++)
	{
		if (ht.keynulls[k] && ht.keynulls[k][row])
			return false;
		int64_t		v = cb_load_widen(ht.keydata[k], ht.keytype[k], row);

		if (k == 0)
			*key0 = v;
		h = pg_hash_combine(h, jh_hash_datum(ht.keytype[k], v, ht.keydict[k]), false);
	}
	*hash = h;
	return true;
}

__device__ __forceinline__ bool
ht_keys_equal_rows(const HtDev &ht, uint32_t ra, uint32_t rb)
{
	for (int k = 0; k < ht.nkeys; k++)
		if (cb_load_widen(ht.keydata[k], ht.keytype[k], ra) != cb_load_widen(ht.keydata[k], ht.keytype[k], rb))
			return false;
	return true;
}

__global__ void
k_ht_clear(unsigned long long *slots, size_t n)
{
	size_t		i = (size_t) blockIdx.x * blockDim.x + threadIdx.x;
	size_t		stride = (size_t) gridDim.x * blockDim.x;

	for (; i < n; i += stride)
		slots[i] = HT_EMPTY;
}

template <int HTB_U>
__global__ void __launch_bounds__(256)
k_ht_build(BuildParams p)
{
	const int64_t stride = (int64_t) gridDim.x * blockDim.x;
	int			inserted = 0;
	bool		dup = false;
	bool		outside = false;

	for (int64_t i0 = (int64_t) blockIdx.x * blockDim.x + threadIdx.x; i0 < p.nrows; i0 += stride * HTB_U)
	{
		uint32_t	h[HTB_U], pos[HTB_U], w[HTB_U], bits[HTB_U], word[HTB_U];
		unsigned long long cur[HTB_U], e[HTB_U];
		bool		v[HTB_U];

#pragma unroll
		for (int u = 0; u < HTB_U; u++)
		{
			const int64_t i = i0 + (int64_t) u * stride;
			int64_t		key0 = 0;

			h[u] = 0;
			v[u] = i < p.nrows && ht_row_hash(p.ht, (uint32_t) i, &h[u], &key0);
			if (v[u] && !ht_in_batch(p.ht.nbatch, p.ht.batch_shift, p.ht.batch_id, h[u]))
				v[u] = false;
			if (v[u] && p.ht.keyslot && !ht_key_in_domain(p.ht.keyslot, key0))
			{
				outside = true;
				v[u] = false;
			}
			e[u] = ((unsigned long long) (p.ht.keyslot ? (uint32_t) key0 : h[u]) << 32) | (uint32_t) i;
			pos[u] = h[u] & p.ht.mask;
			bits[u] = ht_bloom_bits(h[u], &w[u], p.ht.bloom_mask);
		}
		if (p.ht.bloom)
		{
#pragma unroll
			for (int u = 0; u < HTB_U; u++)
				word[u] = v[u] ? p.ht.bloom[w[u]] : 0xFFFFFFFFu;
// ... 297 lines not shown
{
	return ht->d.nbatch > 1 ? ht->total_rows : ht->ninserted;
}

extern "C" int
cbgpu_ht_has_duplicates(const cbgpu_hashtable *ht)
{
	return ht->has_dups;
}

extern "C" const uint32_t *
cbgpu_ht_key_dict_hash(const cbgpu_hashtable *ht, int32_t k)
{
	return (k >= 0 && k < ht->d.nkeys) ? ht->d.keydict[k] : NULL;
}

struct ProbeParams
{
	HtDev		ht;
	const void *okey[CBP_MAX_KEYS];
	const uint8_t *onulls[CBP_MAX_KEYS];
	const uint32_t *odict[CBP_MAX_KEYS];
	int32_t		otype[CBP_MAX_KEYS];
	const uint32_t *sel;
	int64_t		n;
	int32_t		left;
	uint8_t    *matched;
	int64_t		ninner;
	unsigned long long *counts;
	uint32_t   *out_outer;
	uint32_t   *out_inner;
};

template <bool WRITE>
__global__ void __launch_bounds__(256)
k_ht_probe_pairs(ProbeParams p)
{
	int64_t		i = (int64_t) blockIdx.x * blockDim.x + threadIdx.x;
	int64_t		stride = (int64_t) gridDim.x * blockDim.x;

	for (; i < p.n; i += stride)
	{
		uint32_t	row = p.sel ? p.sel[i] : (uint32_t) i;
		uint32_t	h = 0;
		int64_t		key[CBP_MAX_KEYS];
		bool		isnull = false;
		unsigned long long cnt = 0;
		unsigned long long base = WRITE ? p.counts[i] : 0;

		for (int k = 0; k < p.ht.nkeys; k++)
		{
			if (p.onulls[k] && p.onulls[k][row])
				isnull = true;
			key[k] = cb_load_widen(p.okey[k], p.otype[k], row);
			h = pg_hash_combine(h, jh_hash_datum(p.otype[k], key[k], p.odict[k]), false);
		}
		if (!isnull && p.ht.bloom)
		{
			uint32_t	w;
			uint32_t	bits = ht_bloom_bits(h, &w, p.ht.bloom_mask);

			if ((__ldg(p.ht.bloom + w) & bits) != bits)
				isnull = true;
		}
		if (!isnull && p.ht.keyslot && !ht_key_in_domain(p.ht.keyslot, key[0]))
			isnull = true;
		if (!isnull && !ht_in_batch(p.ht.nbatch, p.ht.batch_shift, p.ht.batch_id, h))
			isnull = true;
		if (!isnull)
		{
			uint32_t	pos = h & p.ht.mask;

			for (;;)
			{
				unsigned long long e = p.ht.slots[pos];

				if (e == HT_EMPTY)
					break;
				if ((uint32_t) (e >> 32) == (p.ht.keyslot ? (uint32_t) key[0] : h))
				{
					uint32_t	irow = (uint32_t) e;
					bool		eq = true;

					for (int k = 0; k < p.ht.nkeys && !p.ht.keyslot; k++)
						if (cb_load_widen(p.ht.keydata[k], p.ht.keytype[k], irow) != key[k])
							eq = false;
					if (eq)
					{
						if (WRITE)
						{
							p.out_outer[base + cnt] = row;
							p.out_inner[base + cnt] = irow;
						}
						else if (p.matched)
							p.matched[irow] = 1;
						cnt++;
					}
				}
				pos = (pos + 1) & p.ht.mask;
			}
		}
		if (p.left && cnt == 0 && ht_in_batch(p.ht.nbatch, p.ht.batch_shift, p.ht.batch_id, h))
		{
			if (WRITE)
			{
				p.out_outer[base] = row;
				p.out_inner[base] = 0xFFFFFFFFu;
			}
			cnt = 1;
		}
		if (!WRITE)
			p.counts[i] = cnt;
	}
}

__global__ void
k_exclusive_scan_u64(unsigned long long *a, int64_t n)
{
	__shared__ unsigned long long carry;
	__shared__ unsigned long long warp_tot[32];

	if (threadIdx.x == 0)
		carry = 0;
	__syncthreads();
	for (int64_t base = 0; base < n; base += blockDim.x)
	{
		int64_t		i = base + threadIdx.x;
		unsigned long long v = i < n ? a[i] : 0;
		unsigned long long x = v;
		int			lane = threadIdx.x & 31,
					w = threadIdx.x >> 5;

		for (int o = 1; o < 32; o <<= 1)
		{
			unsigned long long y = __shfl_up_sync(0xffffffffu, x, o);

			if (lane >= o)
				x += y;
// ... 185 lines not shown
```

### cloudberry_b200/csrc/motion.cu

```cuda
#include "common.cuh"

#include <nccl.h>
#include <stdlib.h>
#include <string.h>

#include "../../include/cb_chan.h"

struct DxCtl
{
	unsigned long long counter;
	unsigned long long pad[31];
	unsigned long long done[64];
	unsigned long long nmask[64];
	unsigned long long ready[64];
};

struct DxPeers
{
	DxCtl	   *ctl[64];
};

struct DxResult
{
	unsigned long long got;
// ... 440 lines not shown
exchange_rows(cbgpu_motion *m, cbgpu_rel *send, cbgpu_rel *recv, const int64_t *send_off, const int64_t *send_cnt,
			  const int64_t *recv_off, const int64_t *recv_cnt)
{
	cbgpu_ctx  *ctx = m->ctx;
	int			n = m->nranks;

	CB_NCCL(ctx, ncclGroupStart());
	for (int c = 0; c < send->ncols; c++)
	{
		size_t		w = (size_t) cb_type_w(send->types[c]);

		for (int pass = 0; pass < (send->nulls[c] ? 2 : 1); pass++)
		{
			char	   *sp = pass ? (char *) send->nulls[c] : (char *) send->data[c];
			char	   *rp = pass ? (char *) recv->nulls[c] : (char *) recv->data[c];
			size_t		ww = pass ? 1 : w;

			for (int peer = 0; peer < n; peer++)
			{
				if (peer == m->rank)
					continue;
				if (send_cnt[peer] > 0)
				{
					CB_NCCL(ctx, ncclSend(sp + (size_t) send_off[peer] * ww, (size_t) send_cnt[peer] * ww, ncclInt8, peer, m->comm, ctx->stream));
					m->bytes_sent += send_cnt[peer] * (int64_t) ww;
				}
				if (recv_cnt[peer] > 0)
					CB_NCCL(ctx, ncclRecv(rp + (size_t) recv_off[peer] * ww, (size_t) recv_cnt[peer] * ww, ncclInt8, peer, m->comm, ctx->stream));
			}
		}
	}
	CB_NCCL(ctx, ncclGroupEnd());
	if (send_cnt[m->rank] > 0)
		for (int c = 0; c < send->ncols; c++)
		{
			size_t		w = (size_t) cb_type_w(send->types[c]);

			CB_CUDA(ctx, cudaMemcpyAsync((char *) recv->data[c] + (size_t) recv_off[m->rank] * w,
										 (char *) send->data[c] + (size_t) send_off[m->rank] * w,
										 (size_t) send_cnt[m->rank] * w, cudaMemcpyDeviceToDevice, ctx->stream));
			if (send->nulls[c])
				CB_CUDA(ctx, cudaMemcpyAsync(recv->nulls[c] + recv_off[m->rank], send->nulls[c] + send_off[m->rank],
											 (size_t) send_cnt[m->rank], cudaMemcpyDeviceToDevice, ctx->stream));
		}
	if (ctx->trace_on)
		cb_trace_mark(ctx, "nccl:rows");
	m->exchanges++;
	return CBGPU_OK;
}

extern "C" int
cbgpu_motion_redistribute(cbgpu_motion *m, cbgpu_rel *send, const int64_t *counts, const int64_t *offsets, cbgpu_rel **recv)
{
	int			n = m->nranks;
	int64_t    *matrix;
	int64_t		send_off[64], send_cnt[64], recv_off[64], recv_cnt[64];
	int64_t		total = 0;
	int			rc;

	*recv = NULL;
	NEED_NCCL(m, "a staged Redistribute Motion");
	if (n > 64)
		return cb_fail(m->ctx, CBGPU_ERR_UNSUPPORTED, "more than 64 segments%s", "", 0);
	matrix = (int64_t *) calloc((size_t) n * n, sizeof(int64_t));
	if (!matrix)
		return CBGPU_ERR_NOMEM;
	rc = exchange_counts(m, send, counts, matrix);
	if (rc == CBGPU_OK)
	{
		for (int s = 0; s < n; s++)
		{
			send_off[s] = offsets[s];
			send_cnt[s] = counts[s];
			recv_off[s] = total;
			recv_cnt[s] = matrix[(size_t) s * n + m->rank];
			total += recv_cnt[s];
		}
		rc = make_recv(m, send, total, recv);
	}
	if (rc == CBGPU_OK)
		rc = exchange_rows(m, send, *recv, send_off, send_cnt, recv_off, recv_cnt);
	free(matrix);
	return rc;
}

__device__ __forceinline__ unsigned long long
dx_ld_acquire(const unsigned long long *p)
{
	unsigned long long v;

	asm volatile("ld.acquire.sys.global.u64 %0, [%1];" : "=l"(v) : "l"(p) : "memory");
	return v;
}

__device__ __forceinline__ void
dx_st_relaxed(unsigned long long *p, unsigned long long v)
{
	asm volatile("st.relaxed.sys.global.u64 [%0], %1;" :: "l"(p), "l"(v) : "memory");
}

__device__ __forceinline__ unsigned long long
dx_now_ns(void)
{
	unsigned long long t;

	asm volatile("mov.u64 %0, %%globaltimer;" : "=l"(t));
// ... 494 lines not shown
			{
				CopyCols	cc;
				size_t		o = 0;
				int			parts = 0;

				if (res.cnt[s] == 0)
					continue;
				for (int c = 0; c < send->ncols; c++)
				{
					const size_t w = (size_t) cb_type_w(send->types[c]);

					cc.dst[parts] = (char *) (*recv)->data[c] + (size_t) at * w;
					cc.src[parts] = m->win + buf + GX_HDR + (size_t) s * slot + o;
					cc.bytes[parts] = (size_t) res.cnt[s] * w;
					o += gx_pad(cc.bytes[parts]);
					parts++;
				}
				k_copy_cols<<<parts, 256, 0, ctx->stream>>>(cc);
				CB_LAUNCHED(ctx, "k_copy_cols");
				parts = 0;
				for (int c = 0; c < send->ncols; c++)
					if (((unsigned long long) res.sent[s] >> c) & 1)
					{
						cc.dst[parts] = (char *) (*recv)->nulls[c] + (size_t) at;
						cc.src[parts] = m->win + buf + GX_HDR + (size_t) s * slot + o;
						cc.bytes[parts] = (size_t) res.cnt[s];
						o += gx_pad(cc.bytes[parts]);
						parts++;
					}
				if (parts)
				{
					k_copy_cols<<<parts, 256, 0, ctx->stream>>>(cc);
					CB_LAUNCHED(ctx, "k_copy_cols");
				}
				at += res.cnt[s];
			}
		}
		{
			int64_t		roww = 0;

			for (int c = 0; c < send->ncols; c++)
				roww += cb_type_w(send->types[c]);
			m->direct_bytes += nrows * roww * (root < 0 ? n - 1 : (m->rank != root ? 1 : 0));
		}
	}
	dx_release(m);
	m->direct_exchanges++;
	return 1;
}

extern "C" int
cbgpu_motion_gather(cbgpu_motion *m, int root, cbgpu_rel *send, int64_t nrows, cbgpu_rel **recv)
{
	int			n = m->nranks;
	int64_t    *matrix;
	int64_t		mine[64] = {0}, send_off[64], send_cnt[64], recv_off[64], recv_cnt[64];
	int64_t		total = 0;
	int			rc;

	*recv = NULL;
	if (n > 64 || root < 0 || root >= n)
		return cb_fail(m->ctx, CBGPU_ERR_UNSUPPORTED, "Gather Motion to segment %s%lld", "", root);
	rc = gather_direct(m, root, send, nrows, recv);
	if (rc != 0)
		return rc > 0 ? CBGPU_OK : -rc;
	NEED_NCCL(m, "a Gather Motion too large for the window's Gather slots");
	matrix = (int64_t *) calloc((size_t) n * n, sizeof(int64_t));
	if (!matrix)
		return CBGPU_ERR_NOMEM;
	for (int d = 0; d < n; d++)
		mine[d] = d == root ? nrows : 0;
	rc = exchange_counts(m, send, mine, matrix);
	if (rc == CBGPU_OK)
	{
		for (int s = 0; s < n; s++)
		{
			send_off[s] = 0;
			send_cnt[s] = mine[s];
			recv_off[s] = total;
			recv_cnt[s] = matrix[(size_t) s * n + m->rank];
			total += recv_cnt[s];
		}
		rc = make_recv(m, send, total, recv);
	}
	if (rc == CBGPU_OK)
		rc = exchange_rows(m, send, *recv, send_off, send_cnt, recv_off, recv_cnt);
	free(matrix);
	return rc;
}

extern "C" int
cbgpu_motion_broadcast(cbgpu_motion *m, cbgpu_rel *send, int64_t nrows, cbgpu_rel **recv)
{
	int			n = m->nranks;
	int64_t    *matrix;
	int64_t		mine[64] = {0}, send_off[64], send_cnt[64], recv_off[64], recv_cnt[64];
	int64_t		total = 0;
	int			rc;

	*recv = NULL;
	if (n > 64)
		return cb_fail(m->ctx, CBGPU_ERR_UNSUPPORTED, "more than 64 segments%s", "", 0);
	rc = gather_direct(m, -1, send, nrows, recv);
	if (rc != 0)
		return rc > 0 ? CBGPU_OK : -rc;
	NEED_NCCL(m, "a Broadcast Motion too large for the window's Gather slots");
	matrix = (int64_t *) calloc((size_t) n * n, sizeof(int64_t));
	if (!matrix)
		return CBGPU_ERR_NOMEM;
	for (int d = 0; d < n; d++)
		mine[d] = nrows;
	rc = exchange_counts(m, send, mine, matrix);
	if (rc == CBGPU_OK)
	{
		for (int s = 0; s < n; s++)
		{
			send_off[s] = 0;
			send_cnt[s] = nrows;
			recv_off[s] = total;
			recv_cnt[s] = matrix[(size_t) s * n + m->rank];
			total += recv_cnt[s];
		}
		rc = make_recv(m, send, total, recv);
	}
	if (rc == CBGPU_OK)
		rc = exchange_rows(m, send, *recv, send_off, send_cnt, recv_off, recv_cnt);
	free(matrix);
	return rc;
}

static int
win_chan_put(void *arg, int peer, size_t off, const void *src, size_t len)
{
	cbgpu_motion *m = (cbgpu_motion *) arg;

	if (peer < 0 || peer >= m->nranks || off + len > CH_REGION_BYTES)
		return -1;
	return cudaMemcpyAsync(m->peer_win[peer] + DX_CTL_BYTES + off, src, len, cudaMemcpyDefault, m->chan_stream) == cudaSuccess ? 0 : -1;
}

static int
win_chan_get(void *arg, size_t off, void *dst, size_t len)
{
	cbgpu_motion *m = (cbgpu_motion *) arg;

	if (off + len > CH_REGION_BYTES)
// ... 20 lines not shown
```

### cloudberry_b200/csrc/pipeline.cu

```cuda
#include "pipeline.cuh"

#include <stdlib.h>

int
cb_pipeline_to_dev(cbgpu_ctx *ctx, const CbPipeline *p, PipeDev *d)
{
	memset(d, 0, sizeof(*d));
	if (p->nrows < 0 || p->nrows > 0xFFFFFFF0ll)
		return cb_fail(ctx, CBGPU_ERR_UNSUPPORTED, "pipeline over %s%lld rows exceeds 32-bit row ids", "", p->nrows);
	if (p->ncols < 0 || p->ncols > CBP_MAX_COLS || p->nops < 1 || p->nops > CBP_MAX_OPS ||
		p->nprobes < 0 || p->nprobes > CBP_MAX_SRC - 1 || p->drv_nsrc < 0 || p->drv_nsrc > CBP_MAX_SRC)
		return cb_fail(ctx, CBGPU_ERR_UNSUPPORTED, "pipeline descriptor exceeds the GPU path's limits%s (%lld ops)", "", p->nops);
	d->nrows = p->nrows;
	d->visimap = p->visimap;
	d->drv_nsrc = p->drv_nsrc;
	for (int s = 0; s < CBP_MAX_SRC; s++)
		d->drv_idx[s] = s < p->drv_nsrc ? p->drv_idx[s] : NULL;
	d->ncols = p->ncols;
	for (int c = 0; c < p->ncols; c++)
	{
		d->cols[c] = p->cols[c];
		if (p->cols[c].src < 0 || p->cols[c].src >= CBP_MAX_SRC || cb_type_w(p->cols[c].type) == 0)
			return cb_fail(ctx, CBGPU_ERR_INVALID, "pipeline column %s%lld malformed", "", c);
	}
	d->nops = p->nops;
	int			depth = 0;

	for (int i = 0; i < p->nops; i++)
	{
		const CbpOp *op = &p->ops[i];

		d->ops[i] = *op;
		switch (op->code)
		{
			case CBP_LOAD:
				if (op->a < 0 || op->a >= p->ncols)
					return cb_fail(ctx, CBGPU_ERR_INVALID, "pipeline op %s%lld loads a missing column", "", i);
				depth++;
				break;
			case CBP_CONST:
				depth++;
				break;
			case CBP_DUP:
				if (op->a < 0 || op->a >= depth)
					return cb_fail(ctx, CBGPU_ERR_INVALID, "pipeline op %s%lld: DUP out of range", "", i);
				depth++;
				break;
			case CBP_ADD: case CBP_SUB: case CBP_MUL: case CBP_FADD: case CBP_FSUB: case CBP_FMUL:
			case CBP_EQ: case CBP_NE: case CBP_LT: case CBP_LE: case CBP_GT: case CBP_GE:
			case CBP_FEQ: case CBP_FNE: case CBP_FLT: case CBP_FLE: case CBP_FGT: case CBP_FGE:
			case CBP_AND: case CBP_OR:
				if (depth < 2)
					return cb_fail(ctx, CBGPU_ERR_INVALID, "pipeline op %s%lld underflows the stack", "", i);
				depth--;
				break;
			case CBP_NOT: case CBP_I2F: case CBP_F8ORD:
				if (depth < 1)
					return cb_fail(ctx, CBGPU_ERR_INVALID, "pipeline op %s%lld underflows the stack", "", i);
				break;
			case CBP_FILTER: case CBP_POP:
				if (depth < 1)
					return cb_fail(ctx, CBGPU_ERR_INVALID, "pipeline op %s%lld underflows the stack", "", i);
				depth--;
				break;
			case CBP_PROBE:
				if (op->a < 0 || op->a >= p->nprobes || depth < p->probes[op->a].nkeys)
					return cb_fail(ctx, CBGPU_ERR_INVALID, "pipeline op %s%lld: bad PROBE", "", i);
				depth -= p->probes[op->a].nkeys;
				break;
			case CBP_END:
				if (i != p->nops - 1)
					return cb_fail(ctx, CBGPU_ERR_INVALID, "pipeline op %s%lld: END before the last op", "", i);
				break;
			default:
				return cb_fail(ctx, CBGPU_ERR_INVALID, "pipeline op %s%lld: unknown opcode", "", i);
// ... 189 lines not shown
		}
		d->nsrc = d->src_base + p->nprobes;
		for (;;)
		{
			int			words = 0,
						probes = 0,
						pc = 0;

			for (int b = 0; b + 1 < ns; b++)
			{
				for (; pc < d->stage_pc[b + 1]; pc++)
					if (d->ops[pc].code == CBP_PROBE || d->ops[pc].code == XOP_PROBE_COLS)
						probes++;
				d->q_off[b] = words;
				d->q_ew[b] = d->src_base + probes + 1;
				words += 64 * d->q_ew[b];
			}
			d->q_words = words;
			if (words * 4 * 8 <= 24 * 1024 || ns <= 1)
				break;
			ns--;
		}
		d->nstages = ns;
		d->stage_pc[ns] = d->nops;
	}
	d->status = ctx->d_status;
	return CBGPU_OK;
}

__device__ __forceinline__ int
fcmp_pg(double x, double y)
{
	if (x != x)
		return (y != y) ? 0 : 1;
	if (y != y)
		return -1;
	return x < y ? -1 : (x > y ? 1 : 0);
}

__device__ __forceinline__ int64_t
gen_load_col(const PipeDev &P, int ci, const uint32_t *ridx, uint32_t rnull, bool alive, bool *isnull)
{
	const CbpColumn &c = P.cols[ci];
	bool		n = (rnull >> c.src) & 1;
	int64_t		v = 0;

	if (alive && !n)
	{
		uint32_t	r = ridx[c.src];

		if (c.nulls && c.nulls[r])
			n = true;
		else
			v = cb_load_widen(c.data, c.type, r);
	}
	*isnull = n;
	return v;
}

#define GEN_THREADS 256
#define GEN_QCAP 64

__global__ void __launch_bounds__(GEN_THREADS)
k_pipeline_generic(const __grid_constant__ PipeDev P)
{
	extern __shared__ uint32_t gen_smem[];
	const int	lane = threadIdx.x & 31;
	const int	warp_in_cta = threadIdx.x >> 5;
	const int	nq = P.nstages - 1;
	uint32_t   *myq = gen_smem + (size_t) warp_in_cta * P.q_words;
	int			qcnt[CBP_MAX_STAGES];
	const int64_t nchunks = (P.nrows + 31) / 32;
	int64_t		chunk = (int64_t) blockIdx.x * (GEN_THREADS / 32) + warp_in_cta;
	const int64_t chunk_stride = (int64_t) gridDim.x * (GEN_THREADS / 32);

#pragma unroll
	for (int s = 0; s < CBP_MAX_STAGES; s++)
		qcnt[s] = 0;

	for (;;)
	{
		int			stage = -1;
		int			navail = 0;

		for (int s = nq; s >= 1; s--)
			if (qcnt[s - 1] >= 32)
			{
				stage = s;
				navail = 32;
				break;
			}
		if (stage < 0)
		{
			if (chunk < nchunks)
				stage = 0;
			else
			{
				for (int s = 1; s <= nq; s++)
					if (qcnt[s - 1] > 0)
					{
						stage = s;
						navail = qcnt[s - 1];
						break;
					}
				if (stage < 0)
					break;
			}
// ... 121 lines not shown
					}
					snull &= (1ull << sp) - 1;
				}
				else
				{
					const uint64_t kc = (uint64_t) P.ops[pc].imm;

					for (int k = 0; k < pr.nkeys; k++)
					{
						bool		isn;

						key[k] = gen_load_col(P, (int) ((kc >> (8 * k)) & 0xff), ridx, rnull, alive, &isn);
						if (isn)
							knull = true;
					}
				}
				for (int k = 0; k < pr.nkeys; k++)
					h = pg_hash_combine(h, jh_hash_datum(pr.keytype[k], key[k], pr.keydict[k]), false);
				if (knull && pr.null_key_drops)
					alive = false;
				bool		maybe = alive && !knull;

				if (maybe && pr.ht.bloom)
				{
					uint32_t	w;
					uint32_t	bits = ht_bloom_bits(h, &w, pr.ht.bloom_mask);

					maybe = (__ldg(pr.ht.bloom + w) & bits) == bits;
				}
				if (alive && pr.ht.nbatch > 1 &&
					(knull ? pr.ht.batch_id != 0 : !ht_in_batch(pr.ht.nbatch, pr.ht.batch_shift, pr.ht.batch_id, h)))
				{
					alive = false;
					maybe = false;
				}
				if (maybe && pr.ht.keyslot && !ht_key_in_domain(pr.ht.keyslot, key[0]))
					maybe = false;
				if (maybe)
				{
					uint32_t	pos = h & pr.ht.mask;

					for (;;)
					{
						unsigned long long e = pr.ht.slots[pos];

						if (e == HT_EMPTY)
							break;
						if ((uint32_t) (e >> 32) == (pr.ht.keyslot ? (uint32_t) key[0] : h))
						{
							bool		eq = true;

							irow = (uint32_t) e;
							for (int k = 0; k < pr.nkeys && !pr.ht.keyslot; k++)
								if (cb_load_widen(pr.ht.keydata[k], pr.ht.keytype[k], irow) != key[k])
									eq = false;
							if (eq)
							{
								found = true;
								break;
							}
						}
						pos = (pos + 1) & pr.ht.mask;
					}
				}
				switch (pr.jointype)
				{
					case CB_JOIN_INNER:
					case CB_JOIN_SEMI:
						if (!found)
							alive = false;
						break;
					case CB_JOIN_ANTI:
						if (found)
							alive = false;
						break;
					case CB_JOIN_LEFT:
						if (!found)
							rnull |= 1u << (P.src_base + a);
						break;
				}
				ridx[P.src_base + a] = irow;
				continue;
			}
			switch (code)
			{
				case CBP_LOAD:
					{
						const CbpColumn &c = P.cols[a];
						bool		isnull = (rnull >> c.src) & 1;
						int64_t		v = 0;

						if (alive && !isnull)
						{
							uint32_t	r = ridx[c.src];

							if (c.nulls && c.nulls[r])
								isnull = true;
							else
								v = cb_load_widen(c.data, c.type, r);
						}
						st[sp] = v;
						snull = isnull ? (snull | (1ull << sp)) : (snull & ~(1ull << sp));
						sp++;
						break;
					}
				case CBP_CONST:
					st[sp] = P.ops[pc].imm;
					snull &= ~(1ull << sp);
					sp++;
					break;
				case CBP_DUP:
					st[sp] = st[a];
					snull = ((snull >> a) & 1) ? (snull | (1ull << sp)) : (snull & ~(1ull << sp));
					sp++;
					break;
				case CBP_POP:
					sp--;
					break;
				case CBP_ADD: case CBP_SUB: case CBP_MUL:
					{
						int64_t		y = st[sp - 1],
									x = st[sp - 2];
						bool		n = ((snull >> (sp - 1)) | (snull >> (sp - 2))) & 1;
						int64_t		r;
						bool		ovf;

						if (code == CBP_ADD)
						{
							r = (int64_t) ((uint64_t) x + (uint64_t) y);
							ovf = ((x ^ r) & (y ^ r)) < 0;
						}
						else if (code == CBP_SUB)
						{
							r = (int64_t) ((uint64_t) x - (uint64_t) y);
							ovf = ((x ^ y) & (x ^ r)) < 0;
						}
						else
						{
							r = (int64_t) ((uint64_t) x * (uint64_t) y);
							ovf = __mul64hi(x, y) != (r >> 63);
						}
						if (alive && !n && ovf)
							atomicExch(P.status, CBGPU_ERR_OVERFLOW);
						sp--;
						st[sp - 1] = r;
						snull = n ? (snull | (1ull << (sp - 1))) : (snull & ~(1ull << (sp - 1)));
						break;
					}
				case CBP_FADD: case CBP_FSUB: case CBP_FMUL:
					{
						double		y = __longlong_as_double(st[sp - 1]),
									x = __longlong_as_double(st[sp - 2]);
// ... 278 lines not shown
```

### cloudberry_b200/csrc/probe_chain.cu

```cuda
#include "pipeline.cuh"
#include "xmatch.h"

#include <stdio.h>
#include <stdlib.h>

#define PC_THREADS 256
#define PC_TILE 2048
#ifndef PC_BATCH
#define PC_BATCH 1024
#endif
#ifndef PC_OCC
#define PC_OCC 4
#endif
#define PC_U (PC_BATCH / PC_THREADS)
#define PC_Q0CAP (PC_BATCH + PC_TILE)
#define PC_QCAP (2 * PC_BATCH)
#define PC_MAXP 4
#define PC_MAXOUT 8
#define PC_NQ (2 * PC_MAXP + 1)

struct PcCol
{
	const void *data;
	const uint32_t *dict;
	int32_t		type;
	int32_t		src;
};

struct PcFilter
{
	const void *col;
	int32_t		width;
	int32_t		lo;
	uint32_t	span;
};

struct PcProbe
{
	HtDev		ht;
	int32_t		nkeys;
	int32_t		jointype;
	int32_t		kind;
	PcCol		key[2];
	int32_t		keytype[2];
	int32_t		mode;
	int32_t		smem_off;
};

#define PC_MAXEARLY 2
struct PcEarly
{
	const void *col;
	int32_t		width;
	int32_t		hashtype;
	const uint32_t *bloom;
	uint32_t	mask;
};

struct PcParams
{
	int64_t		nrows;
	const uint32_t *sel;
	const uint8_t *visimap;
	int32_t		nfilters;
	int32_t		np;
	PcFilter	filt[2];
	PcProbe		probe[PC_MAXP];
	int32_t		nearly;
	PcEarly		early[PC_MAXEARLY];
	uint32_t   *qmem;
	int64_t		q_cta_words;
	int32_t		q_off[PC_NQ];
	int32_t		q_cap[PC_NQ];
	int32_t		fuse0;
	int32_t		spec0;
	uint32_t	smem_table_bytes;
	int32_t		sink_kind;
	AggDev		agg;
	int32_t		nkeys;
	PcCol		key[CBP_MAX_KEYS];
	int32_t		naccs;
	int32_t		acc_term[CBP_MAX_AGGS];
	int32_t		nterms;
	int32_t		term_kind[2];
	PcCol		term_a[2], term_b[2];
	long long	term_k[2];
	int32_t		nout;
	PcCol		out[PC_MAXOUT];
	void	   *outcol[PC_MAXOUT];
	int32_t		outtype[PC_MAXOUT];
	unsigned long long *out_count;
	int64_t		out_capacity;
	int32_t		nhash;
	int32_t		hashtype[CBP_MAX_KEYS];
	const uint32_t *hashdict[CBP_MAX_KEYS];
	int32_t		nsegs;
	int64_t		seg_capacity;
	void *const *part_cols;
	unsigned long long *const *part_counts;
	int32_t    *part_flags;
	int64_t		seg_base[64];
	int64_t		seg_cap[64];
	int		   *status;
};

struct PcPart
{
	unsigned	count[64];
	unsigned long long base[64];
	uint8_t		seg[PC_BATCH];
	uint16_t	rank[PC_BATCH];
};

struct PcQ
{
	const uint32_t *q;
	uint32_t	cap;
	uint32_t	iota_base;
	const uint32_t *sel;
};

__device__ __forceinline__ uint32_t
pc_row(const PcQ &Q, int src, uint32_t e)
{
	return Q.q ? Q.q[(size_t) src * Q.cap + e] : (Q.sel ? Q.sel[Q.iota_base + e] : Q.iota_base + e);
}

__device__ __forceinline__ int64_t
pc_load(const PcCol &c, const PcQ &Q, uint32_t e)
{
	return cb_load_widen(c.data, c.type, pc_row(Q, c.src, e));
}

__device__ __forceinline__ uint32_t
pc_reserve(unsigned *cnt, bool alive)
{
	const unsigned m = __ballot_sync(0xffffffffu, alive);
	const int	lane = threadIdx.x & 31;
	unsigned	base = 0;

	if (m == 0)
		return 0;
	if (lane == (__ffs(m) - 1))
		base = atomicAdd(cnt, (unsigned) __popc(m));
	base = __shfl_sync(0xffffffffu, base, __ffs(m) - 1);
	return base + __popc(m & ((1u << lane) - 1));
}

template <int KIND>
__device__ __forceinline__ uint32_t
pc_key_hash(const PcProbe &pr, int64_t k0, int64_t k1)
{
	if (KIND == 0)
		return pg_hash_combine(0u, jh_mix32((uint32_t) (int32_t) k0), false);
	if (KIND == 1)
		return pg_hash_combine(0u, jh_int8(k0), false);
	uint32_t	h = pg_hash_combine(0u, jh_hash_datum(pr.keytype[0], k0, pr.key[0].dict), false);

	if (pr.nkeys > 1)
		h = pg_hash_combine(h, jh_hash_datum(pr.keytype[1], k1, pr.key[1].dict), false);
	return h;
}

template <int KIND>
__device__ __forceinline__ int64_t
pc_load_key0(const PcProbe &pr, uint32_t row, uint64_t pol_stream)
{
	if (KIND == 0)
		return pr.key[0].src == 0 ? (int64_t) ldg_stream_s32((const int32_t *) pr.key[0].data + row, pol_stream)
			: (int64_t) __ldg((const int32_t *) pr.key[0].data + row);
	if (KIND == 1)
		return pr.key[0].src == 0 ? ldg_stream_s64((const long long *) pr.key[0].data + row, pol_stream)
			: __ldg((const long long *) pr.key[0].data + row);
	return cb_load_widen(pr.key[0].data, pr.key[0].type, row);
}

template <int KIND>
__device__ __noinline__ void
pc_stage_bloom(const PcProbe &pr, int j, PcQ Q, unsigned base, unsigned n, uint32_t *out, unsigned ocap, unsigned *ocnt)
{
	const bool	use_bloom = pr.ht.bloom != NULL && pr.jointype != CB_JOIN_ANTI;
	const uint64_t pol_stream = l2_policy_evict_first();
	const uint64_t pol_keep = l2_policy_evict_last();
	const int	lane = threadIdx.x & 31;
	uint32_t	e[PC_U], h[PC_U], w[PC_U], bits[PC_U], word[PC_U], bal[PC_U];
	int64_t		k0[PC_U], k1[PC_U];
	bool		v[PC_U];

#pragma unroll
	for (int u = 0; u < PC_U; u++)
	{
		const unsigned i = u * PC_THREADS + threadIdx.x;
		uint32_t	r0;

		v[u] = i < n;
		e[u] = base + (v[u] ? i : 0u);
		r0 = pc_row(Q, pr.key[0].src, e[u]);
		k0[u] = pc_load_key0<KIND>(pr, r0, pol_stream);
		k1[u] = (KIND == 2 && pr.nkeys > 1) ? pc_load(pr.key[1], Q, e[u]) : 0;
	}
#pragma unroll
	for (int u = 0; u < PC_U; u++)
	{
		h[u] = pc_key_hash<KIND>(pr, k0[u], k1[u]);
		bits[u] = ht_bloom_bits(h[u], &w[u], pr.ht.bloom_mask);
	}
	if (use_bloom)
	{
#pragma unroll
		for (int u = 0; u < PC_U; u++)
			word[u] = ldg_hint_u32(pr.ht.bloom + w[u], pol_keep);
	}
	unsigned	tot = 0,
				wb = 0;

#pragma unroll
	for (int u = 0; u < PC_U; u++)
	{
		const bool	pass = v[u] && (!use_bloom || (word[u] & bits[u]) == bits[u]);

		bal[u] = __ballot_sync(0xffffffffu, pass);
		tot += __popc(bal[u]);
	}
	if (tot == 0)
		return;
	if (lane == 0)
		wb = atomicAdd(ocnt, tot);
// ... 26 lines not shown
#pragma unroll
	for (int u = 0; u < PC_U; u++)
	{
		const unsigned i = u * PC_THREADS + threadIdx.x;

		v[u] = i < n;
		e[u] = base + (v[u] ? i : 0u);
		h[u] = Q.q[(size_t) (j + 1) * Q.cap + e[u]];
		pos[u] = h[u] & pr.ht.mask;
	}
#pragma unroll
	for (int u = 0; u < PC_U; u++)
		slot[u] = v[u] ? __ldg(pr.ht.slots + pos[u]) : HT_EMPTY;
	unsigned	tot = 0,
				wb = 0;

#pragma unroll
	for (int u = 0; u < PC_U; u++)
	{
		bool		found = false;

		irow[u] = 0;
		if (slot[u] != HT_EMPTY)
		{
			const int64_t k0 = pc_load_key0<KIND>(pr, pc_row(Q, pr.key[0].src, e[u]), pol_stream);
			const int64_t k1 = (KIND == 2 && pr.nkeys > 1) ? pc_load(pr.key[1], Q, e[u]) : 0;
			unsigned long long x = slot[u];
			uint32_t	p = pos[u];

			if (pr.ht.keyslot)
			{
				const uint32_t tag = (uint32_t) k0;

				if (ht_key_in_domain(pr.ht.keyslot, k0))
					while (x != HT_EMPTY)
					{
						if ((uint32_t) (x >> 32) == tag)
						{
							found = true;
							irow[u] = (uint32_t) x;
							break;
						}
						p = (p + 1) & pr.ht.mask;
						x = __ldg(pr.ht.slots + p);
					}
			}
			else
				while (x != HT_EMPTY)
				{
					if ((uint32_t) (x >> 32) == h[u])
					{
						const uint32_t r = (uint32_t) x;

						if (cb_load_widen(pr.ht.keydata[0], pr.ht.keytype[0], r) == k0 &&
							(KIND != 2 || pr.nkeys < 2 || cb_load_widen(pr.ht.keydata[1], pr.ht.keytype[1], r) == k1))
						{
							found = true;
							irow[u] = r;
							break;
						}
					}
					p = (p + 1) & pr.ht.mask;
					x = __ldg(pr.ht.slots + p);
				}
		}
		bal[u] = __ballot_sync(0xffffffffu, v[u] && (pr.jointype == CB_JOIN_ANTI ? !found : found));
		tot += __popc(bal[u]);
	}
	if (tot == 0)
		return;
	if (lane == 0)
		wb = atomicAdd(ocnt, tot);
	wb = __shfl_sync(0xffffffffu, wb, 0);
#pragma unroll
	for (int u = 0; u < PC_U; u++)
	{
		if ((bal[u] >> lane) & 1)
		{
			const uint32_t opos = wb + __popc(bal[u] & ((1u << lane) - 1));

			for (int s = 0; s <= j; s++)
				out[(size_t) s * ocap + opos] = pc_row(Q, s, e[u]);
			out[(size_t) (j + 1) * ocap + opos] = irow[u];
		}
		wb += __popc(bal[u]);
	}
}

template <int KIND>
__device__ __noinline__ void
pc_stage_direct(const PcProbe &pr, int j, PcQ Q, unsigned base, unsigned n, uint32_t *out, unsigned ocap, unsigned *ocnt, const unsigned long long *slots)
{
	const uint64_t pol_stream = l2_policy_evict_first();
	const int	lane = threadIdx.x & 31;
	uint32_t	e[PC_U], h[PC_U], pos[PC_U], irow[PC_U], bal[PC_U];
	int64_t		k0[PC_U], k1[PC_U];
	unsigned long long slot[PC_U];
	bool		v[PC_U];

#pragma unroll
	for (int u = 0; u < PC_U; u++)
	{
		const unsigned i = u * PC_THREADS + threadIdx.x;

		v[u] = i < n;
		e[u] = base + (v[u] ? i : 0u);
		k0[u] = pc_load_key0<KIND>(pr, pc_row(Q, pr.key[0].src, e[u]), pol_stream);
		k1[u] = (KIND == 2 && pr.nkeys > 1) ? pc_load(pr.key[1], Q, e[u]) : 0;
	}
#pragma unroll
	for (int u = 0; u < PC_U; u++)
	{
		h[u] = pc_key_hash<KIND>(pr, k0[u], k1[u]);
		pos[u] = h[u] & pr.ht.mask;
	}
#pragma unroll
	for (int u = 0; u < PC_U; u++)
		slot[u] = v[u] ? slots[pos[u]] : HT_EMPTY;
	unsigned	tot = 0,
				wb = 0;

#pragma unroll
	for (int u = 0; u < PC_U; u++)
	{
		bool		found = false;
		unsigned long long x = slot[u];
		uint32_t	p = pos[u];

		irow[u] = 0;
		if (pr.ht.keyslot)
		{
			const uint32_t tag = (uint32_t) k0[u];

			if (ht_key_in_domain(pr.ht.keyslot, k0[u]))
				while (x != HT_EMPTY)
				{
					if ((uint32_t) (x >> 32) == tag)
					{
						found = true;
						irow[u] = (uint32_t) x;
						break;
					}
					p = (p + 1) & pr.ht.mask;
					x = slots[p];
				}
		}
		else
			while (x != HT_EMPTY)
			{
				if ((uint32_t) (x >> 32) == h[u])
				{
					const uint32_t r = (uint32_t) x;

					if (cb_load_widen(pr.ht.keydata[0], pr.ht.keytype[0], r) == k0[u] &&
						(KIND != 2 || pr.nkeys < 2 || cb_load_widen(pr.ht.keydata[1], pr.ht.keytype[1], r) == k1[u]))
					{
						found = true;
						irow[u] = r;
						break;
					}
				}
				p = (p + 1) & pr.ht.mask;
				x = slots[p];
			}
		bal[u] = __ballot_sync(0xffffffffu, v[u] && (pr.jointype == CB_JOIN_ANTI ? !found : found));
		tot += __popc(bal[u]);
	}
	if (tot == 0)
		return;
	if (lane == 0)
		wb = atomicAdd(ocnt, tot);
	wb = __shfl_sync(0xffffffffu, wb, 0);
#pragma unroll
	for (int u = 0; u < PC_U; u++)
	{
		if ((bal[u] >> lane) & 1)
		{
			const uint32_t opos = wb + __popc(bal[u] & ((1u << lane) - 1));

			for (int s = 0; s <= j; s++)
				out[(size_t) s * ocap + opos] = pc_row(Q, s, e[u]);
			out[(size_t) (j + 1) * ocap + opos] = irow[u];
		}
		wb += __popc(bal[u]);
	}
}

__device__ __noinline__ void
pc_stage_sink(const PcParams &P, PcQ Q, unsigned base, unsigned n, unsigned long long *s_obase, PcPart *part)
{
	if (P.sink_kind == CBP_SINK_AGG)
	{
		for (unsigned b = 0; b < n; b += PC_THREADS)
		{
			const unsigned i = b + threadIdx.x;

			if (i < n)
			{
				const uint32_t e = base + i;
				int64_t		kv[CBP_MAX_KEYS];
				uint32_t	h = 0;

				for (int k = 0; k < P.nkeys; k++)
				{
					kv[k] = pc_load(P.key[k], Q, e);
					h = pg_hash_combine(h, pg_hash_datum(P.key[k].type, kv[k], P.key[k].dict), false);
				}
				h = pg_murmurhash32(h);
// ... 878 lines not shown
			Q.iota_base = 0;
			Q.sel = NULL;
		}
		if (s == last)
			pc_stage_sink(P, Q, base, n, &s_obase, &part);
		else
		{
			const int	j = (s - 1) >> 1;
			const PcProbe &pr = sprobe[j];
			uint32_t   *out = qg + P.q_off[s];

			if ((s & 1) && pr.mode != 0)
			{
				const unsigned long long *slots = pr.mode == 2 ? s_tables + pr.smem_off : pr.ht.slots;
				uint32_t   *out2 = qg + P.q_off[s + 1];

				if (pr.kind == 0)
					pc_stage_direct<0>(pr, j, Q, base, n, out2, (unsigned) P.q_cap[s + 1], &cnt[s + 1], slots);
				else if (pr.kind == 1)
					pc_stage_direct<1>(pr, j, Q, base, n, out2, (unsigned) P.q_cap[s + 1], &cnt[s + 1], slots);
				else
					pc_stage_direct<2>(pr, j, Q, base, n, out2, (unsigned) P.q_cap[s + 1], &cnt[s + 1], slots);
			}
			else if (s & 1)
			{
				if (pr.kind == 0)
					pc_stage_bloom<0>(pr, j, Q, base, n, out, (unsigned) P.q_cap[s], &cnt[s]);
				else if (pr.kind == 1)
					pc_stage_bloom<1>(pr, j, Q, base, n, out, (unsigned) P.q_cap[s], &cnt[s]);
				else
					pc_stage_bloom<2>(pr, j, Q, base, n, out, (unsigned) P.q_cap[s], &cnt[s]);
			}
			else
			{
				if (pr.kind == 0)
					pc_stage_ht<0>(pr, j, Q, base, n, out, (unsigned) P.q_cap[s], &cnt[s]);
				else if (pr.kind == 1)
					pc_stage_ht<1>(pr, j, Q, base, n, out, (unsigned) P.q_cap[s], &cnt[s]);
				else
					pc_stage_ht<2>(pr, j, Q, base, n, out, (unsigned) P.q_cap[s], &cnt[s]);
			}
		}
	}
}

static bool
pc_col(const CbPipeline *p, int c, PcCol *out, int base)
{
	if (p->cols[c].nulls != NULL || p->cols[c].type == CB_FLOAT8 || p->cols[c].type == CB_NUMERIC128)
		return false;
	out->data = p->cols[c].data;
	out->dict = p->cols[c].dict_hash;
	out->type = p->cols[c].type;
	out->src = p->cols[c].src == 0 ? 0 : p->cols[c].src - base + 1;
	return true;
}

struct PcEarlyBuild
{
	int64_t		nrows;
	HtDev		self;
	int32_t		kc;
	int32_t		hashtype;
	int32_t		nred;
	HtDev		red[PC_MAXP];
	int32_t		red_nkeys[PC_MAXP];
	PcCol		red_key[PC_MAXP][2];
	int32_t		red_keytype[PC_MAXP][2];
	uint32_t   *bloom;
	uint32_t	mask;
	unsigned long long *passed;
};

__global__ void
k_pc_early_build(PcEarlyBuild B)
{
	for (int64_t r = (int64_t) blockIdx.x * blockDim.x + threadIdx.x; r < B.nrows; r += (int64_t) gridDim.x * blockDim.x)
	{
		bool		ok = true;

		for (int k = 0; k < B.self.nkeys; k++)
			if (B.self.keynulls[k] && B.self.keynulls[k][r])
				ok = false;
		for (int m = 0; m < B.nred && ok; m++)
		{
			const HtDev &T = B.red[m];
			int64_t		kv[2] = {0, 0};
			uint32_t	h = 0;
			bool		found = false;

			for (int i = 0; i < B.red_nkeys[m]; i++)
			{
				kv[i] = cb_load_widen(B.red_key[m][i].data, B.red_key[m][i].type, (uint32_t) r);
				h = pg_hash_combine(h, jh_hash_datum(B.red_keytype[m][i], kv[i], B.red_key[m][i].dict), false);
			}
			uint32_t	pos = h & T.mask;

			for (; !(T.keyslot && !ht_key_in_domain(T.keyslot, kv[0]));)
			{
				const unsigned long long e = T.slots[pos];

				if (e == HT_EMPTY)
					break;
				if ((uint32_t) (e >> 32) == (T.keyslot ? (uint32_t) kv[0] : h))
				{
					const uint32_t ir = (uint32_t) e;

					if (T.keyslot || (cb_load_widen(T.keydata[0], T.keytype[0], ir) == kv[0] &&
									  (B.red_nkeys[m] < 2 || cb_load_widen(T.keydata[1], T.keytype[1], ir) == kv[1])))
					{
						found = true;
						break;
					}
				}
				pos = (pos + 1) & T.mask;
			}
			ok = found;
		}
		if (ok && !B.bloom)
			atomicAdd(B.passed, 1ull);
		if (ok && B.bloom)
		{
			uint32_t	w;
			const int64_t kv = cb_load_widen(B.self.keydata[B.kc], B.self.keytype[B.kc], (uint32_t) r);
			const uint32_t bits = ht_bloom_bits(pg_hash_combine(0u, jh_hash_datum(B.hashtype, kv, NULL), false), &w, B.mask);

			atomicOr(B.bloom + w, bits);
		}
	}
}

#define PC_REJECT(n) \
	do { \
		if (ctx->opt_debug) \
			fprintf(stderr, "k_probe_chain: pipeline not matched (reason %d, line %d)\n", n, __LINE__); \
		return CBGPU_OK; \
	} while (0)

int
cb_try_probe_chain(cbgpu_ctx *ctx, const CbPipeline *p, const PipeDev *d, bool *handled)
{
	XProg	   *xp = (XProg *) cb_scratch(ctx, 2, sizeof(XProg));
	PcParams   *Pp = (PcParams *) cb_scratch(ctx, 3, sizeof(PcParams));
	if (!xp || !Pp)
		return CBGPU_ERR_NOMEM;
	XProg	   &x = *xp;
	PcParams   &P = *Pp;
	const CbpSink *s = &p->sink;
	int			np = 0;
	int			base = 1;
	int			term_node[2] = {-1, -1};

	*handled = false;
	if (p->nprobes < 0 || p->nprobes > PC_MAXP || p->drv_nsrc != 0)
		PC_REJECT(1);
	if (s->kind != CBP_SINK_AGG && s->kind != CBP_SINK_MATERIALIZE && s->kind != CBP_SINK_PARTITION)
		PC_REJECT(2);
	if (s->kind == CBP_SINK_PARTITION && s->nsegs > 64)
		PC_REJECT(2);
	if (!xm_decompile(p, &x))
		PC_REJECT(3);
	memset(&P, 0, sizeof(P));
	for (int i = 0; i < x.nsections; i++)
	{
		XSection   *sec = &x.sections[i];

		if (sec->kind == 0)
		{
			int			code, col;
			int64_t		v, lo = INT32_MIN, hi = INT32_MAX;

			if (np > 0)
				PC_REJECT(4);
			if (!xm_is_cmp_const(&x, sec->node, &code, &col, &v) || p->cols[col].src != 0 || p->cols[col].nulls ||
				(cb_type_w(p->cols[col].type) != 4 && cb_type_w(p->cols[col].type) != 1))
				PC_REJECT(5);
			if (cb_type_w(p->cols[col].type) == 1)
// ... 538 lines not shown
```

### cloudberry_b200/csrc/scan_agg.cu

```cuda
#include "pipeline.cuh"
#include "xmatch.h"

#define SA_NSUM 6

struct SmallAggParams
{
	int64_t		nrows;
	const long long *colA;
	const long long *colB;
	const long long *colC;
	const long long *colD;
	long long	k,
				k2;
	const int32_t *fcol;
	int32_t		flo;
	uint32_t	fspan;
	const uint8_t *key0;
	const uint8_t *key1;
	const uint8_t *visimap;
	AggDev		agg;
	int32_t		nkeys;
	int32_t		keytype[2];
	const uint32_t *keydict[2];
	int32_t		naccs;
	int32_t		accsum[CBP_MAX_AGGS];
	int32_t		want_chg;
	int		   *status;
	int		   *retry;
	int		   *audit;
	AggSnap    *snap;
	int			snap_groups;
	unsigned long long *scratch;
	unsigned   *skeys;
};

template <int G>
struct SaAcc
{
	unsigned	cnt[G];
	long long	s[G][SA_NSUM];
};

template <bool NARROW>
__device__ __forceinline__ void
sa_madd(long long &acc, unsigned hit, long long v)
{
	if (NARROW)
		asm("mad.wide.u32 %0, %1, %2, %0;" : "+l"(acc) : "r"(hit), "r"((unsigned) v));
	else
		asm("{\n\t"
			".reg .b32 vlo, vhi, tlo, thi;\n\t"
			".reg .b64 t;\n\t"
			"mov.b64 {vlo, vhi}, %2;\n\t"
			"mad.wide.u32 t, %1, vlo, %0;\n\t"
			"mov.b64 {tlo, thi}, t;\n\t"
			"mad.lo.u32 thi, %1, vhi, thi;\n\t"
			"mov.b64 %0, {tlo, thi};\n\t"
			"}"
			: "+l"(acc) : "r"(hit), "l"(v));
}

template <int G>
__device__ __noinline__ void
sa_insert_key(unsigned *gkeys, unsigned key, int *retry)
{
	bool		placed = false;

	for (int g = 0; g < G && !placed; g++)
	{
		unsigned	cur = ((volatile unsigned *) gkeys)[g];

		if (cur == 0)
			cur = atomicCAS(gkeys + g, 0u, key);
		if (cur == 0 || cur == key)
			placed = true;
	}
	if (!placed)
		atomicExch(retry, 1);
}

#define SA_TILE 896
#define SA_STAGES 5
#define SA_NCONS(G) ((G) <= 4 ? 448 : 224)

struct __align__(128) SaStage
{
	long long	a[SA_TILE];
	long long	b[SA_TILE];
	long long	c[SA_TILE];
	long long	d[SA_TILE];
	int32_t		f[SA_TILE];
	uint8_t		k0[SA_TILE];
	uint8_t		k1[SA_TILE];
};

template <int G>
struct SaState
{
	SaAcc<G>	acc;
	unsigned	gk[G];
	unsigned long long magAB,
				magC, magD;
	unsigned	rows_seen;
};

template <int G, int MASK, bool NARROW, int SHAPE, bool CHECK>
__device__ __forceinline__ void
sa_row(const SmallAggParams &P, SaState<G> &S, unsigned *gkeys, const SaStage *st, int r, int rows, int64_t r0)
{
	const bool	hasF = SHAPE ? true : P.fcol != NULL;
	const bool	hasK0 = SHAPE == 1 ? true : (SHAPE == 2 ? false : P.key0 != NULL);
	const bool	hasK1 = SHAPE == 1 ? true : (SHAPE == 2 ? false : P.key1 != NULL);
	bool		pass = true;
	long long	a = (MASK & 1) ? st->a[r] : 0;
	long long	b = st->b[r];
	long long	c = st->c[r];
	long long	d = (MASK & 0x28) ? st->d[r] : 0;
	int32_t		f = hasF ? st->f[r] : P.flo;
	unsigned	k0 = hasK0 ? st->k0[r] : 0;
	unsigned	k1 = hasK1 ? st->k1[r] : 0;

	if (CHECK)
	{
		pass = r < rows;
		if (!pass)
			a = b = c = d = 0;
		if (P.visimap && pass)
		{
			const int64_t gr = r0 + r;

			pass = (__ldg(P.visimap + (gr >> 3)) >> (gr & 7)) & 1;
		}
	}
	pass = pass && ((unsigned) (f - P.flo) <= P.fspan);
	long long	kc = P.k - c;
	long long	rev = b * kc;
	long long	chg = (MASK & 0x20) ? rev * (P.k2 + d) : 0;
	unsigned	key = pass ? (0x10000u | k0 | (k1 << 8)) : 0xFFFFFFFFu;
	unsigned	hit[G];
	unsigned	known = 0;

#pragma unroll
	for (int g = 0; g < G; g++)
	{
		hit[g] = key == S.gk[g] ? 1u : 0u;
		known |= hit[g];
	}
	if (pass && !known)
	{
		sa_insert_key<G>(gkeys, key, P.retry);
#pragma unroll
		for (int g = 0; g < G; g++)
		{
			S.gk[g] = ((volatile unsigned *) gkeys)[g];
			hit[g] = key == S.gk[g] ? 1u : 0u;
		}
	}
	S.magAB |= (unsigned long long) (a | b);
	S.magC |= (unsigned long long) c;
	S.magD |= (unsigned long long) d;
	S.rows_seen += pass ? 1u : 0u;
#pragma unroll
	for (int g = 0; g < G; g++)
	{
		S.acc.cnt[g] += hit[g];
		if (MASK & 0x01)
			sa_madd<NARROW>(S.acc.s[g][0], hit[g], a);
		if (MASK & 0x02)
			sa_madd<NARROW>(S.acc.s[g][1], hit[g], b);
		if (MASK & 0x04)
			sa_madd<NARROW>(S.acc.s[g][2], hit[g], c);
		if (MASK & 0x08)
			sa_madd<NARROW>(S.acc.s[g][3], hit[g], d);
		if (MASK & 0x10)
			sa_madd<NARROW>(S.acc.s[g][4], hit[g], rev);
		if (MASK & 0x20)
			sa_madd<false>(S.acc.s[g][5], hit[g], chg);
	}
}

template <int G, int MASK, bool NARROW, int SHAPE>
__global__ void __launch_bounds__(SA_NCONS(G) + 32, 1)
k_scan_agg_small(const __grid_constant__ SmallAggParams P)
{
	extern __shared__ __align__(128) unsigned char smem_raw[];
	SaStage    *stages = (SaStage *) smem_raw;
	__shared__ uint64_t full_bar[SA_STAGES];
	__shared__ uint64_t empty_bar[SA_STAGES];
	__shared__ unsigned gkeys[G];
	__shared__ unsigned long long red[G][SA_NSUM + 1][2];
	constexpr int NCONS = SA_NCONS(G);
	SaState<G>	S;
	const int	warp = threadIdx.x >> 5;
	const int	lane = threadIdx.x & 31;
	const int64_t ntiles = (P.nrows + SA_TILE - 1) / SA_TILE;

	if (threadIdx.x == 0)
	{
		for (int s = 0; s < SA_STAGES; s++)
		{
			mbar_init(&full_bar[s], 1);
			mbar_init(&empty_bar[s], NCONS / 32);
		}
		asm volatile("fence.mbarrier_init.release.cluster;" ::: "memory");
	}
	if (threadIdx.x < G)
		gkeys[threadIdx.x] = 0;
	for (int i = threadIdx.x; i < G * (SA_NSUM + 1) * 2; i += blockDim.x)
		(&red[0][0][0])[i] = 0;
	S.magAB = S.magC = S.magD = 0;
	S.rows_seen = 0;
#pragma unroll
	for (int g = 0; g < G; g++)
	{
		S.acc.cnt[g] = 0;
		S.gk[g] = 0;
#pragma unroll
		for (int s = 0; s < SA_NSUM; s++)
			S.acc.s[g][s] = 0;
	}
	__syncthreads();

	if (warp == 0)
	{
		if (lane == 0)
		{
			int			it = 0;

			for (int64_t t = blockIdx.x; t < ntiles; t += gridDim.x, it++)
			{
				const int	s = it % SA_STAGES;
				const unsigned ph = (it / SA_STAGES) & 1;
				const int64_t r0 = t * SA_TILE;
				const int64_t rows = P.nrows - r0 < SA_TILE ? P.nrows - r0 : SA_TILE;
				const unsigned b8 = (unsigned) (rows * 8 + 15) & ~15u;
				const unsigned b4 = (unsigned) (rows * 4 + 15) & ~15u;
				const unsigned b1 = (unsigned) (rows + 15) & ~15u;
				const bool	wantA = (MASK & 1) != 0;
				const bool	wantD = (MASK & 0x28) != 0;
				unsigned	total = 2 * b8 + (wantA ? b8 : 0) + (wantD ? b8 : 0) + (P.fcol ? b4 : 0) +
					(P.key0 ? b1 : 0) + (P.key1 ? b1 : 0);
				SaStage    *st = &stages[s];

				mbar_wait(&empty_bar[s], ph ^ 1);
				mbar_expect_tx(&full_bar[s], total);
				tma_load_1d(st->b, P.colB + r0, b8, &full_bar[s]);
				tma_load_1d(st->c, P.colC + r0, b8, &full_bar[s]);
				if (wantA)
					tma_load_1d(st->a, P.colA + r0, b8, &full_bar[s]);
				if (wantD)
					tma_load_1d(st->d, P.colD + r0, b8, &full_bar[s]);
				if (P.fcol)
					tma_load_1d(st->f, P.fcol + r0, b4, &full_bar[s]);
				if (P.key0)
					tma_load_1d(st->k0, P.key0 + r0, b1, &full_bar[s]);
				if (P.key1)
					tma_load_1d(st->k1, P.key1 + r0, b1, &full_bar[s]);
			}
		}
	}
	else
	{
		const int	ct = threadIdx.x - 32;
		int			it = 0;

		for (int64_t t = blockIdx.x; t < ntiles; t += gridDim.x, it++)
		{
			const int	s = it % SA_STAGES;
			const unsigned ph = (it / SA_STAGES) & 1;
			const int64_t r0 = t * SA_TILE;
			const int	rows = (int) (P.nrows - r0 < SA_TILE ? P.nrows - r0 : SA_TILE);
			const SaStage *st = &stages[s];

			mbar_wait(&full_bar[s], ph);
			if (rows == SA_TILE && !P.visimap)
			{
#pragma unroll
				for (int j = 0; j < SA_TILE / NCONS; j++)
					sa_row<G, MASK, NARROW, SHAPE, false>(P, S, gkeys, st, ct + j * NCONS, rows, r0);
			}
			else
			{
#pragma unroll
				for (int j = 0; j < SA_TILE / NCONS; j++)
					sa_row<G, MASK, NARROW, SHAPE, true>(P, S, gkeys, st, ct + j * NCONS, rows, r0);
			}
			__syncwarp();
			if (lane == 0)
				mbar_arrive(&empty_bar[s]);
		}
	}

	{
		int			bab = 64 - __clzll(S.magAB),
					bc = 64 - __clzll(S.magC),
					bd = 64 - __clzll(S.magD);
		unsigned long long ak = (unsigned long long) (P.k < 0 ? -P.k : P.k),
					ak2 = (unsigned long long) (P.k2 < 0 ? -P.k2 : P.k2);
		int			bk = 64 - __clzll(ak),
					bk2 = 64 - __clzll(ak2);
		int			brev = bab + (bc > bk ? bc : bk) + 1;
		int			bchg = (MASK & 0x20) ? brev + (bd > bk2 ? bd : bk2) + 1 : 0;
		int			brows = 32 - __clz(S.rows_seen);
		int			worst = brev > bchg ? brev : bchg;

		if (bc > worst)
			worst = bc;
		if (bd > worst)
			worst = bd;
		if (worst + brows >= 63)
			atomicExch(P.audit, 1);
		if (NARROW && (bab > 32 || bc > 32 || bd > 32 || ((MASK & 0x10) && brev > 32)))
			atomicExch(P.audit, 1);
		if ((long long) (S.magAB | S.magC | S.magD) < 0)
			atomicExch(P.audit, 1);
	}

#pragma unroll
	for (int g = 0; g < G; g++)
	{
#pragma unroll
		for (int s = 0; s <= SA_NSUM; s++)
		{
			long long	v = s < SA_NSUM ? S.acc.s[g][s < SA_NSUM ? s : 0] : (long long) S.acc.cnt[g];

			if (s < SA_NSUM && !((MASK >> s) & 1))
				continue;
			unsigned long long lo = (unsigned long long) v;
			long long	hi = v < 0 ? -1 : 0;

#pragma unroll
			for (int o = 16; o; o >>= 1)
			{
				unsigned long long lo2 = __shfl_xor_sync(0xffffffffu, lo, o);
				long long	hi2 = __shfl_xor_sync(0xffffffffu, hi, o);
				unsigned long long nl = lo + lo2;

				hi = hi + hi2 + (nl < lo ? 1 : 0);
				lo = nl;
			}
			if (lane == 0 && (lo | (unsigned long long) hi))
			{
// ... 19 lines not shown
		if (threadIdx.x == 0)
		{
			P.snap->retry = *P.retry;
			P.snap->audit = *P.audit;
			P.snap->ngroups = -1;
			__threadfence_system();
		}
		return;
	}
	if (threadIdx.x == 0)
		P.snap->retry = P.snap->audit = 0;
	for (int e = blockIdx.x * blockDim.x + threadIdx.x; e < nblocks * G; e += gridDim.x * blockDim.x)
	{
		unsigned	key = P.skeys[e];
		const unsigned long long *r = P.scratch + (size_t) e * (SA_NSUM + 1) * 2;
		unsigned long long cnt = r[SA_NSUM * 2];

		if (key == 0 || cnt == 0)
			continue;
		int64_t		kv[2] = {(int64_t) (key & 0xff), (int64_t) ((key >> 8) & 0xff)};
		uint32_t	h = 0;

		for (int k = 0; k < P.nkeys; k++)
			h = pg_hash_combine(h, pg_hash_datum(P.keytype[k], kv[k], P.keydict[k]), false);
		h = pg_murmurhash32(h);
		int			slot = agg_find_or_insert(P.agg, h, kv, 0);

		if (slot < 0)
			continue;
		for (int a = 0; a < P.naccs; a++)
		{
			int			s = P.accsum[a];

			atomicAdd((unsigned long long *) (P.agg.n + (size_t) slot * P.agg.naccs + a), cnt);
			if (s >= 0)
				atomic_add128(P.agg.sum + ((size_t) slot * P.agg.naccs + a) * 2, r[s * 2], r[s * 2 + 1]);
		}
	}
	__syncthreads();
	if (P.snap_groups)
		agg_snapshot_block(P.agg, P.snap);
	else
	{
		if (threadIdx.x == 0)
			P.snap->ngroups = -1;
		__threadfence_system();
	}
}

static bool
col_plain(const CbPipeline *p, int c, int width)
{
	return p->cols[c].src == 0 && p->cols[c].nulls == NULL && cb_type_w(p->cols[c].type) == width &&
		p->cols[c].type != CB_FLOAT8;
}

static int
try_small_agg(cbgpu_ctx *ctx, const CbPipeline *p, const PipeDev *d, bool *handled)
{
	XProg	   *xp = (XProg *) cb_scratch(ctx, 5, sizeof(XProg));
	if (!xp)
		return CBGPU_ERR_NOMEM;
	XProg	   &x = *xp;
	SmallAggParams P;
	int			colB = -1,
				colC = -1,
				colD = -1,
				colA = -1;
	int64_t		k = 0,
				k2 = 0;
	bool		have_rev = false,
				have_chg = false;
	const CbpSink *s = &p->sink;

	*handled = false;
	if (s->kind != CBP_SINK_AGG || p->nprobes != 0 || p->drv_nsrc != 0 || s->nkeys > 2)
		return CBGPU_OK;
	if (!xm_decompile(p, &x) || x.depth < s->nkeys)
		return CBGPU_OK;
	memset(&P, 0, sizeof(P));
	P.fspan = 0xFFFFFFFFu;
	if (x.nsections > 1)
		return CBGPU_OK;
	if (x.nsections == 1)
	{
		int			code,
					col;
		int64_t		v;

		if (x.sections[0].kind != 0 || !xm_is_cmp_const(&x, x.sections[0].node, &code, &col, &v) ||
			!col_plain(p, col, 4) || v < INT32_MIN || v > INT32_MAX)
			return CBGPU_OK;
		int64_t		lo = INT32_MIN,
					hi = INT32_MAX;

		switch (code)
		{
			case CBP_EQ: lo = hi = v; break;
			case CBP_LT: hi = v - 1; break;
			case CBP_LE: hi = v; break;
			case CBP_GT: lo = v + 1; break;
			case CBP_GE: lo = v; break;
			default: return CBGPU_OK;
		}
		if (lo > hi)
			lo = hi = (int64_t) INT32_MAX + 1;
// ... 44 lines not shown
			if ((have_rev || have_chg) && (b != colB || c != colC || kk != k))
				return CBGPU_OK;
			colB = b; colC = c; k = kk;
			have_rev = true;
		}
	}
	if (!have_rev && !have_chg)
		return CBGPU_OK;
	P.naccs = s->naccs;
	for (int a = 0; a < s->naccs; a++)
	{
		int			b,
					c,
					dd,
					col;
		int64_t		kk,
					kk2;

		if (s->accs[a].kind == CBP_ACC_COUNT)
		{
			P.accsum[a] = -1;
			continue;
		}
		int			node = x.stack[s->nkeys + s->accs[a].arg];

		if (xm_is_chg(&x, node, &b, &kk, &c, &kk2, &dd))
			P.accsum[a] = 5;
		else if (xm_is_rev(&x, node, &b, &kk, &c))
			P.accsum[a] = 4;
		else if (xm_is_load(&x, node, &col))
		{
			if (col == colB)
				P.accsum[a] = 1;
			else if (col == colC)
				P.accsum[a] = 2;
			else if (col == colD)
				P.accsum[a] = 3;
			else if (colA < 0 || col == colA)
			{
				colA = col;
				P.accsum[a] = 0;
			}
			else if (colD < 0)
			{
				colD = col;
				P.accsum[a] = 3;
			}
			else
				return CBGPU_OK;
		}
		else
			return CBGPU_OK;
	}
	if (!col_plain(p, colB, 8) || !col_plain(p, colC, 8) || (colA >= 0 && !col_plain(p, colA, 8)) ||
		(colD >= 0 && !col_plain(p, colD, 8)))
		return CBGPU_OK;
	P.nrows = p->nrows;
	P.colA = colA >= 0 ? (const long long *) p->cols[colA].data : NULL;
	P.colB = (const long long *) p->cols[colB].data;
	P.colC = (const long long *) p->cols[colC].data;
	P.colD = colD >= 0 ? (const long long *) p->cols[colD].data : NULL;
	P.k = k;
	P.k2 = k2;
	P.visimap = p->visimap;
	P.agg = d->sink.agg;
	P.nkeys = s->nkeys;
	P.status = ctx->d_status;

	P.want_chg = have_chg;

	int			need = 0;

	for (int a = 0; a < s->naccs; a++)
		if (P.accsum[a] >= 0)
			need |= 1 << P.accsum[a];
	if (have_chg)
		need |= 0x20;

	static const int masks[3] = {0x10, 0x37, 0x3f};
	int			mask = -1;

	for (int i = 0; i < 3 && mask < 0; i++)
		if ((need & ~masks[i]) == 0 && (!(masks[i] & 0x01) || P.colA) && (!(masks[i] & 0x28) || P.colD))
			mask = masks[i];
	if (mask < 0)
		return CBGPU_OK;
	const int	shape = (P.fcol && P.key0 && P.key1) ? 1 : ((P.fcol && !P.key0 && !P.key1) ? 2 : 0);

	int		   *d_flags;
	int64_t		ntiles = (p->nrows + SA_TILE - 1) / SA_TILE;
	int			blocks = ctx->sm_count;
	const size_t smem = sizeof(SaStage) * SA_STAGES;
	int			G = 4;
	bool		narrow = true;

	if (blocks > ntiles)
		blocks = (int) ntiles;
	{
		const size_t sbytes = (size_t) blocks * 8 * (SA_NSUM + 1) * 2 * sizeof(unsigned long long);
		const size_t kbytes = (size_t) blocks * 8 * sizeof(unsigned);
		const size_t need = 256 + sbytes + ((kbytes + 255) & ~(size_t) 255);

		if (ctx->small_dev_bytes < need)
		{
			if (ctx->small_dev)
			{
				CB_CUDA(ctx, cudaStreamSynchronize(ctx->stream));
				CB_CUDA(ctx, cudaFree(ctx->small_dev));
				ctx->small_dev = NULL;
				ctx->small_dev_bytes = 0;
			}
			CB_CUDA(ctx, cudaMalloc(&ctx->small_dev, need));
			ctx->small_dev_bytes = need;
		}
		d_flags = (int *) ctx->small_dev;
		P.scratch = (unsigned long long *) ((char *) ctx->small_dev + 256);
		P.skeys = (unsigned *) ((char *) ctx->small_dev + 256 + sbytes);
	}
	P.retry = d_flags;
	P.audit = d_flags + 1;
	P.snap = ctx->agg_snap;
	P.snap_groups = s->agg->capacity <= AGG_SNAP_MAXCAP;
	for (;;)
	{
		CB_CUDA(ctx, cudaMemsetAsync(d_flags, 0, 2 * sizeof(int), ctx->stream));
		CB_CUDA(ctx, cudaEventRecord(ctx->ev_k0, ctx->stream));
		int			kl = cb_klog_begin(ctx, "k_scan_agg_small");
#define SA_LAUNCH(GG, MM, NN, SS) \
		do { \
			static bool attr_done = false; \
			if (!attr_done) \
			{ \
				CB_CUDA(ctx, cudaFuncSetAttribute(k_scan_agg_small<GG, MM, NN, SS>, cudaFuncAttributeMaxDynamicSharedMemorySize, (int) smem)); \
				attr_done = true; \
			} \
			k_scan_agg_small<GG, MM, NN, SS><<<blocks, SA_NCONS(GG) + 32, smem, ctx->stream>>>(P); \
			ctx->last_kernel_name = "k_scan_agg_small<" #GG "," #MM "," #NN "," #SS ">"; \
			if (kl >= 0) \
				ctx->klog_name[kl] = ctx->last_kernel_name; \
		} while (0)
#define SA_PICK_SHAPE(MM, NN) \
		do { \
			if (shape == 1) SA_LAUNCH(4, MM, NN, 1); \
			else if (shape == 2) SA_LAUNCH(4, MM, NN, 2); \
			else SA_LAUNCH(4, MM, NN, 0); \
		} while (0)
#define SA_PICK(NN) \
		do { \
			if (mask == 0x10) SA_PICK_SHAPE(0x10, NN); \
			else if (mask == 0x37) SA_PICK_SHAPE(0x37, NN); \
			else SA_PICK_SHAPE(0x3f, NN); \
		} while (0)
		if (G == 8)
		{
			if (!P.colA || !P.colD)
				break;
			SA_LAUNCH(8, 0x3f, false, 0);
		}
		else if (narrow)
			SA_PICK(true);
		else
			SA_PICK(false);
		CB_LAUNCHED(ctx, "k_scan_agg_small");
		cb_klog_end(ctx, kl);
		CB_CUDA(ctx, cudaEventRecord(ctx->ev_k1, ctx->stream));
		ctx->kernel_timed = true;
		ctx->agg_snap->ngroups = -1;
		ctx->agg_snap->retry = ctx->agg_snap->audit = 0;
		k_small_commit<<<1, 256, 0, ctx->stream>>>(P, G, blocks);
		CB_LAUNCHED(ctx, "k_small_commit");
		CB_CUDA(ctx, CB_STATUS_RIDE(ctx));
		CB_CUDA(ctx, cudaStreamSynchronize(ctx->stream));
		CB_STATUS_FETCHED(ctx);
		const int	h_flags[2] = {ctx->agg_snap->retry, ctx->agg_snap->audit};

		if (h_flags[1])
		{
			if (!narrow || G == 8)
				break;
			narrow = false;
			continue;
		}
		if (h_flags[0])
		{
			if (G == 8)
				break;
			G = 8;
			continue;
		}
		*handled = true;
		cb_agg_adopt_snapshot((cbgpu_aggtable *) s->agg, ctx->agg_snap);
		break;
	}
	return CBGPU_OK;
}

// ... 10 lines not shown
```

### include/cbgpu.h

```cpp
#ifndef CBGPU_H
#define CBGPU_H

#include <stdint.h>
#include <stddef.h>
#include "cb_plan.h"

#ifdef __cplusplus
extern "C" {
#endif

#define CBGPU_OK 0
#define CBGPU_ERR_CUDA (-1)
#define CBGPU_ERR_INVALID (-2)
#define CBGPU_ERR_UNSUPPORTED (-3)
#define CBGPU_ERR_OVERFLOW (-4)
#define CBGPU_ERR_NOMEM (-5)
#define CBGPU_ERR_CORRUPT (-6)
#define CBGPU_ERR_PEER (-7)
#define CBGPU_ERR_INTERRUPTED (-8)

typedef struct cbgpu_ctx cbgpu_ctx;
typedef struct cbgpu_rel cbgpu_rel;
typedef struct cbgpu_hashtable cbgpu_hashtable;
typedef struct cbgpu_aggtable cbgpu_aggtable;
typedef struct cbgpu_motion cbgpu_motion;

int			cbgpu_ctx_create(int device, cbgpu_ctx **out);
void		cbgpu_ctx_destroy(cbgpu_ctx *ctx);
const char *cbgpu_last_error(cbgpu_ctx *ctx);
int			cbgpu_sync(cbgpu_ctx *ctx);
int			cbgpu_check_status(cbgpu_ctx *ctx);
int			cbgpu_device_count(void);
int			cbgpu_sm_count(cbgpu_ctx *ctx);
int64_t		cbgpu_kernel_launches(cbgpu_ctx *ctx);
int			cbgpu_timer_start(cbgpu_ctx *ctx);
int			cbgpu_timer_stop_ms(cbgpu_ctx *ctx, double *ms);
double		cbgpu_last_kernel_ms(cbgpu_ctx *ctx);
void		cbgpu_kernel_log_reset(cbgpu_ctx *ctx);
int			cbgpu_kernel_log_longest(cbgpu_ctx *ctx, char *name, int namelen, double *ms);
const char *cbgpu_last_kernel_name(cbgpu_ctx *ctx);
int			cbgpu_trace_begin(cbgpu_ctx *ctx);
int			cbgpu_trace_end(cbgpu_ctx *ctx);
int			cbgpu_trace_get(cbgpu_ctx *ctx, int i, char *name, int namelen, double *ms);
void		cbgpu_range_push(const char *name);
void		cbgpu_range_pop(void);
int			cbgpu_flush_l2(cbgpu_ctx *ctx);
void	   *cbgpu_host_alloc(size_t bytes);
void		cbgpu_host_free(void *p);

uint32_t	cbgpu_hashbpchar(const char *s, int32_t len);

int			cbgpu_rel_create(cbgpu_ctx *ctx, int64_t nrows, int32_t ncols, const int32_t *types,
							 const int32_t *dscales, cbgpu_rel **out);
void		cbgpu_rel_free(cbgpu_rel *rel);
int64_t		cbgpu_rel_nrows(const cbgpu_rel *rel);
int32_t		cbgpu_rel_ncols(const cbgpu_rel *rel);
int32_t		cbgpu_rel_col_type(const cbgpu_rel *rel, int32_t col);
int32_t		cbgpu_rel_col_dscale(const cbgpu_rel *rel, int32_t col);
int			cbgpu_rel_load_column(cbgpu_rel *rel, int32_t col, const void *host, const uint8_t *nulls);
int			cbgpu_rel_load_column_narrow(cbgpu_rel *rel, int32_t col, const void *host, int32_t host_width);
int			cbgpu_rel_read_column(cbgpu_rel *rel, int32_t col, int64_t lo, int64_t hi, void *host, uint8_t *nulls);
int			cbgpu_rel_set_visimap(cbgpu_rel *rel, const uint8_t *bits);
int			cbgpu_rel_read_visimap(cbgpu_rel *rel, uint8_t *bits);
int			cbgpu_rel_set_dict_hash(cbgpu_rel *rel, int32_t col, const uint32_t *hashes, int32_t n);
int			cbgpu_rel_set_nrows(cbgpu_rel *rel, int64_t nrows);
int			cbgpu_rel_take_rows(cbgpu_rel *dst, cbgpu_rel *src, const uint32_t *dev_idx, int64_t n);
int			cbgpu_rel_read_rows(cbgpu_rel *rel, const uint32_t *host_idx, int64_t n, int64_t *out, uint8_t *outnull);
void	   *cbgpu_rel_col_devptr(cbgpu_rel *rel, int32_t col);
size_t		cbgpu_rel_nbytes(const cbgpu_rel *rel);

#define CBP_MAX_SRC 8
#define CBP_MAX_COLS 40
#define CBP_MAX_OPS 128
#define CBP_MAX_KEYS 4
#define CBP_MAX_AGGS 16
#define CBP_MAX_OUT 48
#define CBP_STACK 48

typedef enum CbpOpCode
{
	CBP_END = 0,
	CBP_LOAD,
	CBP_CONST,
	CBP_ADD, CBP_SUB, CBP_MUL,
	CBP_FADD, CBP_FSUB, CBP_FMUL,
	CBP_I2F,
	CBP_EQ, CBP_NE, CBP_LT, CBP_LE, CBP_GT, CBP_GE,
	CBP_FEQ, CBP_FNE, CBP_FLT, CBP_FLE, CBP_FGT, CBP_FGE,
	CBP_AND, CBP_OR, CBP_NOT,
	CBP_FILTER,
	CBP_PROBE,
	CBP_DUP,
	CBP_POP,
	CBP_F8ORD
} CbpOpCode;

typedef struct CbpOp
{
	int32_t		code;
	int32_t		a;
	int64_t		imm;
} CbpOp;

typedef struct CbpColumn
{
	const void *data;
	const uint8_t *nulls;
	const uint32_t *dict_hash;
	int32_t		type;
	int32_t		src;
} CbpColumn;

typedef struct CbpProbe
{
	const cbgpu_hashtable *ht;
	int32_t		jointype;
	int32_t		nkeys;
	int32_t		keytype[CBP_MAX_KEYS];
	const uint32_t *key_dict_hash[CBP_MAX_KEYS];
	int32_t		null_key_drops;
} CbpProbe;

typedef enum CbpSinkKind
{
	CBP_SINK_AGG = 1,
	CBP_SINK_MATERIALIZE,
	CBP_SINK_PARTITION
} CbpSinkKind;

typedef enum CbpAggKind
{
	CBP_ACC_COUNT = 1,
	CBP_ACC_SUM_INT,
	CBP_ACC_SUM_FLOAT,
	CBP_ACC_MIN, CBP_ACC_MAX,
	CBP_ACC_MERGE_INT,
	CBP_ACC_MERGE_FLOAT,
	CBP_ACC_MERGE_COUNT,
	CBP_ACC_MERGE_MIN,
	CBP_ACC_MERGE_MAX
} CbpAggKind;

typedef struct CbpAcc
{
	int32_t		kind;
	int32_t		arg;
} CbpAcc;

typedef struct CbpSink
{
	int32_t		kind;
	cbgpu_aggtable *agg;
	int32_t		nkeys;
	int32_t		keytype[CBP_MAX_KEYS];
	const uint32_t *key_dict_hash[CBP_MAX_KEYS];
	int32_t		naccs;
	CbpAcc		accs[CBP_MAX_AGGS];
	int32_t		nout;
	cbgpu_rel  *out;
	int64_t	   *out_count;
	int32_t		nhash;
	int32_t		hashtype[CBP_MAX_KEYS];
	const uint32_t *hash_dict_hash[CBP_MAX_KEYS];
// ... 175 lines not shown
```

Before: 77.16 billion.

## Store NUMERIC columns at narrowest fitting width and scan them narrow

At load time, NUMERIC columns are scanned for min/max and re-encoded to 1/2/4-byte storage when the values fit. Every consumer (top-N, row reads, copies, AOCS decode) gets a per-column width. The small-group scan-agg kernel TMA-loads narrow tiles with variable stage offsets, and the pipeline stage count now depends on shared-memory size. The aim is to cut HBM traffic in bandwidth-bound Q1 scans, at the cost of an extra minmax pass and host sync at load, widen kernels on readback, and wider code paths that could mis-handle width.

New measurement: 112.3 billion, median of 6. 45.6% higher.

```diff
diff --git a/cloudberry_b200/capi.py b/cloudberry_b200/capi.py
--- a/cloudberry_b200/capi.py
+++ b/cloudberry_b200/capi.py
@@ -298,6 +298,9 @@
             "cbgpu_rel_set_nrows": (C.c_int, [vp, i64]),
             "cbgpu_rel_copy_rows": (C.c_int, [vp, i64, vp, i64, i64]),
             "cbgpu_rel_col_devptr": (vp, [vp, i32]),
+            "cbgpu_rel_col_width": (i32, [vp, i32]),
+            "cbgpu_rel_narrow_column": (C.c_int, [vp, i32]),
+            "cbgpu_rel_read_rows": (C.c_int, [vp, vp, i64, vp, vp]),
             "cbgpu_rel_nbytes": (C.c_size_t, [vp]),
             "cbgpu_ht_build": (C.c_int, [vp, vp, C.POINTER(i32), i32, C.POINTER(vp)]),
             "cbgpu_ht_free": (None, [vp]),
diff --git a/cloudberry_b200/csrc/agg.cu b/cloudberry_b200/csrc/agg.cu
--- a/cloudberry_b200/csrc/agg.cu
+++ b/cloudberry_b200/csrc/agg.cu
@@ -479,6 +479,7 @@
 {
 	const void *key[TOPN_MAXKEYS];
 	int32_t		keytype[TOPN_MAXKEYS];
+	int32_t		width[TOPN_MAXKEYS];
 	int32_t		desc[TOPN_MAXKEYS];
 	int32_t		uns[TOPN_MAXKEYS];
 	int32_t		nkeys;
@@ -522,7 +523,7 @@
 		if (row == 0xFFFFFFFFu)
 			continue;
 		for (int k = 0; k < p.nkeys; k++)
-			key[k] = cb_load_widen(p.key[k], p.keytype[k], row);
+			key[k] = cb_load_widen(p.key[k], p.keytype[k], p.width[k], row);
 		if (nbest == p.k && !topn_before(p, key, row, best_key[nbest - 1], best_row[nbest - 1]))
 			continue;
 		int			pos = nbest < p.k ? nbest : p.k - 1;
@@ -550,7 +551,7 @@
 __device__ __forceinline__ unsigned long long
 topn_ukey(const TopnParams &p, int i, uint32_t row)
 {
-	unsigned long long u = (unsigned long long) cb_load_widen(p.key[i], p.keytype[i], row);
+	unsigned long long u = (unsigned long long) cb_load_widen(p.key[i], p.keytype[i], p.width[i], row);
 
 	if (!p.uns[i])
 		u ^= 0x8000000000000000ull;
@@ -671,7 +672,7 @@
 		int			rank = 0;
 
 		for (int k = 0; k < p.nkeys; k++)
-			ki[k] = cb_load_widen(p.key[k], p.keytype[k], ri);
+			ki[k] = cb_load_widen(p.key[k], p.keytype[k], p.width[k], ri);
 		for (int j = 0; j < m && rank < p.k; j++)
 		{
 			const uint32_t rj = cand ? cand[j] : (uint32_t) j;
@@ -680,7 +681,7 @@
 			if (j == i)
 				continue;
 			for (int k = 0; k < p.nkeys; k++)
-				kj[k] = cb_load_widen(p.key[k], p.keytype[k], rj);
+				kj[k] = cb_load_widen(p.key[k], p.keytype[k], p.width[k], rj);
 			rank += topn_before(p, kj, rj, ki, ri);
 		}
 		if (rank < p.k)
@@ -695,6 +696,7 @@
 	const void *key[TOPN_MAXKEYS];
 	const uint8_t *nulls[TOPN_MAXKEYS];
 	int32_t		keytype[TOPN_MAXKEYS];
+	int32_t		width[TOPN_MAXKEYS];
 	int32_t		desc[TOPN_MAXKEYS];
 	int32_t		uns[TOPN_MAXKEYS];
 	int32_t		nkeys;
@@ -719,8 +721,8 @@
 			c = (an && bn) ? 0 : (an ? 1 : -1);
 		else
 		{
-			const int64_t x = cb_load_widen(p.key[i], p.keytype[i], (uint32_t) a);
-			const int64_t y = cb_load_widen(p.key[i], p.keytype[i], (uint32_t) b);
+			const int64_t x = cb_load_widen(p.key[i], p.keytype[i], p.width[i], (uint32_t) a);
+			const int64_t y = cb_load_widen(p.key[i], p.keytype[i], p.width[i], (uint32_t) b);
 
 			if (x == y)
 				c = 0;
@@ -812,6 +814,7 @@
 		p.key[i] = rel->data[keycols[i]];
 		p.nulls[i] = rel->nulls[keycols[i]];
 		p.keytype[i] = rel->types[keycols[i]];
+		p.width[i] = rel->width[keycols[i]];
 		p.desc[i] = descending[i];
 		p.uns[i] = unsigned_cmp ? unsigned_cmp[i] : 0;
 		if (p.keytype[i] == CB_FLOAT8)
@@ -881,6 +884,7 @@
 			return cb_fail(ctx, CBGPU_ERR_UNSUPPORTED, "device top-N over a nullable sort key (%s column %lld)", "", keycols[i]);
 		p.key[i] = rel->data[keycols[i]];
 		p.keytype[i] = rel->types[keycols[i]];
+		p.width[i] = rel->width[keycols[i]];
 		p.desc[i] = descending[i];
 		p.uns[i] = unsigned_cmp ? unsigned_cmp[i] : 0;
 		if (p.keytype[i] == CB_FLOAT8)
diff --git a/cloudberry_b200/csrc/aocs.cu b/cloudberry_b200/csrc/aocs.cu
--- a/cloudberry_b200/csrc/aocs.cu
+++ b/cloudberry_b200/csrc/aocs.cu
@@ -1303,6 +1303,12 @@
 			: !((varkind == CBGPU_AOCS_VAR_NUMERIC && rel->types[col] == CB_NUMERIC) || (varkind == CBGPU_AOCS_VAR_BPCHAR1 && outw == 1) ||
 				(varkind == CBGPU_AOCS_VAR_DICT && (rel->types[col] == CB_DICT8 || rel->types[col] == CB_DICT32))))
 			return cb_fail(ctx, CBGPU_ERR_UNSUPPORTED, "AOCS column of length %s%lld does not decode into this relation column", "", attlen);
+		{
+			const int	rc = cb_rel_restore_wide(rel, col);
+
+			if (rc)
+				return rc;
+		}
 	}
 	else
 		outw = 0;
diff --git a/cloudberry_b200/csrc/common.cuh b/cloudberry_b200/csrc/common.cuh
--- a/cloudberry_b200/csrc/common.cuh
+++ b/cloudberry_b200/csrc/common.cuh
@@ -90,6 +90,7 @@
 	int32_t		dict_n[CB_MAX_COLS_REL];
 	uint8_t	   *visimap;
 	bool		owns[CB_MAX_COLS_REL];
+	int8_t		width[CB_MAX_COLS_REL];
 	void	   *slab;
 };
 
@@ -625,19 +626,47 @@
 
 #endif
 
+CB_HD int
+cb_full_w(int type)
+{
+	switch (type)
+	{
+		case CB_INT4: case CB_DATE: case CB_DICT32:
+			return 4;
+		case CB_INT8: case CB_NUMERIC: case CB_FLOAT8:
+			return 8;
+		default:
+			return 1;
+	}
+}
+
+#ifdef __CUDACC__
 __device__ __forceinline__ int64_t
-cb_load_widen(const void *data, int type, uint32_t row)
+cb_load_widen(const void *data, int type, int width, uint32_t row)
 {
 	switch (type)
 	{
 		case CB_INT4: case CB_DATE: case CB_DICT32:
 			return (int64_t) __ldg((const int32_t *) data + row);
-		case CB_INT8: case CB_NUMERIC: case CB_FLOAT8:
+		case CB_INT8: case CB_FLOAT8:
 			return __ldg((const long long *) data + row);
+		case CB_NUMERIC:
+			if (width == 8)
+				return __ldg((const long long *) data + row);
+			if (width == 4)
+				return (int64_t) __ldg((const int32_t *) data + row);
+			if (width == 2)
+				return (int64_t) __ldg((const int16_t *) data + row);
+			return (int64_t) (int8_t) __ldg((const uint8_t *) data + row);
 		default:
 			return (int64_t) __ldg((const uint8_t *) data + row);
 	}
 }
+#endif
+
+int			cb_rel_restore_wide(cbgpu_rel *rel, int col);
+int			cb_widen_copy(cbgpu_ctx *ctx, int64_t *dst, const void *src, int width, int64_t n);
+int			cb_rel_wide_copy(cbgpu_rel *rel, cbgpu_rel **out);
 
 __device__ __forceinline__ void
 atomic_add128(unsigned long long *acc, unsigned long long lo, unsigned long long hi)
diff --git a/cloudberry_b200/csrc/ctx.cu b/cloudberry_b200/csrc/ctx.cu
--- a/cloudberry_b200/csrc/ctx.cu
+++ b/cloudberry_b200/csrc/ctx.cu
@@ -1,4 +1,6 @@
 #include "common.cuh"
+
+#include <limits.h>
 
 #include <nvtx3/nvToolsExt.h>
 
@@ -385,6 +387,7 @@
 		}
 		r->types[i] = types[i];
 		r->dscales[i] = dscales ? dscales[i] : 0;
+		r->width[i] = (int8_t) cb_type_w(types[i]);
 		colbytes[i] = (bytes + 255) & ~(size_t) 255;
 		total += colbytes[i];
 	}
@@ -457,15 +460,243 @@
 	return (col >= 0 && col < rel->ncols) ? rel->dscales[col] : 0;
 }
 
+extern "C" int32_t
+cbgpu_rel_col_width(const cbgpu_rel *rel, int32_t col)
+{
+	return (col >= 0 && col < rel->ncols) ? rel->width[col] : 0;
+}
+
+static int
+rel_set_storage(cbgpu_rel *rel, int col, int width)
+{
+	cbgpu_ctx  *ctx = rel->ctx;
+	void	   *buf;
+	const size_t bytes = ((size_t) (rel->capacity ? rel->capacity : 1) * width + 255) & ~(size_t) 255;
+
+	if (rel->width[col] == width)
+		return CBGPU_OK;
+	if (!rel->owns[col] && width <= cb_type_w(rel->types[col]))
+	{
+		rel->width[col] = (int8_t) width;
+		return CBGPU_OK;
+	}
+	CB_CUDA(ctx, cudaMallocAsync(&buf, bytes, ctx->stream));
+	if (rel->owns[col])
+		CB_CUDA(ctx, cudaFreeAsync(rel->data[col], ctx->stream));
+	rel->data[col] = buf;
+	rel->owns[col] = true;
+	rel->width[col] = (int8_t) width;
+	return CBGPU_OK;
+}
+
+template <typename NARROW, typename WIDE>
+__global__ void k_widen(const NARROW *__restrict__ src, WIDE *__restrict__ dst, int64_t n);
+
+template <typename NARROW>
+__global__ void
+k_narrow(const long long *__restrict__ src, NARROW *__restrict__ dst, int64_t n)
+{
+	for (int64_t i = (int64_t) blockIdx.x * blockDim.x + threadIdx.x; i < n; i += (int64_t) gridDim.x * blockDim.x)
+		dst[i] = (NARROW) src[i];
+}
+
+static int
+launch_blocks(cbgpu_ctx *ctx, int64_t n)
+{
+	const int64_t b = (n + 255) / 256;
+
+	return (int) (b < 1 ? 1 : (b > ctx->sm_count * 8 ? ctx->sm_count * 8 : b));
+}
+
+int
+cb_widen_copy(cbgpu_ctx *ctx, int64_t *dst, const void *src, int width, int64_t n)
+{
+	const int	blocks = launch_blocks(ctx, n);
+
+	if (n <= 0)
+		return CBGPU_OK;
+	if (width == 8)
+	{
+		CB_CUDA(ctx, cudaMemcpyAsync(dst, src, (size_t) n * 8, cudaMemcpyDeviceToDevice, ctx->stream));
+		return CBGPU_OK;
+	}
+	if (width == 1)
+		k_widen<int8_t, int64_t><<<blocks, 256, 0, ctx->stream>>>((const int8_t *) src, dst, n);
+	else if (width == 2)
+		k_widen<int16_t, int64_t><<<blocks, 256, 0, ctx->stream>>>((const int16_t *) src, dst, n);
+	else
+		k_widen<int32_t, int64_t><<<blocks, 256, 0, ctx->stream>>>((const int32_t *) src, dst, n);
+	CB_LAUNCHED(ctx, "k_widen");
+	return CBGPU_OK;
+}
+
+static int
+narrow_copy(cbgpu_ctx *ctx, void *dst, const long long *src, int width, int64_t n)
+{
+	const int	blocks = launch_blocks(ctx, n);
+
+	if (n <= 0)
+		return CBGPU_OK;
+	if (width == 1)
+		k_narrow<int8_t><<<blocks, 256, 0, ctx->stream>>>(src, (int8_t *) dst, n);
+	else if (width == 2)
+		k_narrow<int16_t><<<blocks, 256, 0, ctx->stream>>>(src, (int16_t *) dst, n);
+	else
+		k_narrow<int32_t><<<blocks, 256, 0, ctx->stream>>>(src, (int32_t *) dst, n);
+	CB_LAUNCHED(ctx, "k_narrow");
+	return CBGPU_OK;
+}
+
+static int
+rel_reencode(cbgpu_rel *rel, int col, int width)
+{
+	cbgpu_ctx  *ctx = rel->ctx;
+	const int	ow = rel->width[col];
+	const int64_t n = rel->nrows;
+	void	   *old = rel->data[col];
+	void	   *dst = NULL,
+			   *src = old,
+			   *tmp = NULL;
+	cudaError_t e;
+	int			rc;
+
+	if (ow == width)
+		return CBGPU_OK;
+	if (rel->owns[col])
+		e = cudaMallocAsync(&dst, (((size_t) (rel->capacity ? rel->capacity : 1) * width) + 255) & ~(size_t) 255, ctx->stream);
+	else
+	{
+		dst = old;
+		e = cudaMallocAsync(&tmp, (size_t) (n ? n : 1) * ow, ctx->stream);
+		if (e == cudaSuccess)
+			e = cudaMemcpyAsync(tmp, old, (size_t) n * ow, cudaMemcpyDeviceToDevice, ctx->stream);
+		src = tmp;
+	}
+	if (e != cudaSuccess)
+	{
+		if (rel->owns[col] && dst)
+			cudaFreeAsync(dst, ctx->stream);
+		if (tmp)
+			cudaFreeAsync(tmp, ctx->stream);
+		(void) cudaGetLastError();
+		snprintf(ctx->err, sizeof(ctx->err), "re-encoding column %d: %s", col, cudaGetErrorString(e));
+		return e == cudaErrorMemoryAllocation ? CBGPU_ERR_NOMEM : CBGPU_ERR_CUDA;
+	}
+	rc = width < ow ? narrow_copy(ctx, dst, (const long long *) src, width, n)
+		: cb_widen_copy(ctx, (int64_t *) dst, src, ow, n);
+	if (rc)
+	{
+		if (rel->owns[col])
+			cudaFreeAsync(dst, ctx->stream);
+		if (tmp)
+			cudaFreeAsync(tmp, ctx->stream);
+		return rc;
+	}
+	CB_CUDA(ctx, cudaFreeAsync(rel->owns[col] ? old : tmp, ctx->stream));
+	rel->data[col] = dst;
+	rel->width[col] = (int8_t) width;
+	return CBGPU_OK;
+}
+
+int
+cb_rel_restore_wide(cbgpu_rel *rel, int col)
+{
+	return rel_reencode(rel, col, cb_type_w(rel->types[col]));
+}
+
+__global__ void
+k_minmax64(const long long *__restrict__ v, int64_t n, long long *out)
+{
+	long long	lo = LLONG_MAX,
+				hi = LLONG_MIN;
+
+	for (int64_t i = (int64_t) blockIdx.x * blockDim.x + threadIdx.x; i < n; i += (int64_t) gridDim.x * blockDim.x)
+	{
+		const long long x = __ldg(v + i);
+
+		lo = x < lo ? x : lo;
+		hi = x > hi ? x : hi;
+	}
+	for (int o = 16; o; o >>= 1)
+	{
+		const long long l2 = __shfl_xor_sync(0xffffffffu, lo, o),
+					h2 = __shfl_xor_sync(0xffffffffu, hi, o);
+
+		lo = l2 < lo ? l2 : lo;
+		hi = h2 > hi ? h2 : hi;
+	}
+	if ((threadIdx.x & 31) == 0)
+	{
+		atomicMin(out, lo);
+		atomicMax(out + 1, hi);
+	}
+}
+
+extern "C" int
+cbgpu_rel_narrow_column(cbgpu_rel *rel, int32_t col)
+{
+	cbgpu_ctx  *ctx = rel->ctx;
+	long long	h[2] = {LLONG_MAX, LLONG_MIN};
+	long long  *d;
+	int			w,
+				rc;
+	cudaError_t e;
+	bool		owned;
+
+	if (col < 0 || col >= rel->ncols)
+		return cb_fail(ctx, CBGPU_ERR_INVALID, "cbgpu_rel_narrow_column: bad column%s %lld", "", col);
+	if (rel->types[col] != CB_NUMERIC || rel->width[col] != 8 || rel->nrows == 0)
+		return CBGPU_OK;
+	CB_CUDA(ctx, cudaSetDevice(ctx->device));
+	CB_CUDA(ctx, cudaMallocAsync(&d, sizeof(h), ctx->stream));
+	e = cudaMemcpyAsync(d, h, sizeof(h), cudaMemcpyHostToDevice, ctx->stream);
+	if (e == cudaSuccess)
+	{
+		k_minmax64<<<launch_blocks(ctx, rel->nrows), 256, 0, ctx->stream>>>((const long long *) rel->data[col], rel->nrows, d);
+		ctx->launches++;
+		e = cudaGetLastError();
+	}
+	if (e == cudaSuccess)
+		e = cudaMemcpyAsync(h, d, sizeof(h), cudaMemcpyDeviceToHost, ctx->stream);
+	if (e == cudaSuccess)
+		e = cudaStreamSynchronize(ctx->stream);
+	cudaFreeAsync(d, ctx->stream);
+	CB_CUDA(ctx, e);
+	if (h[0] >= INT8_MIN && h[1] <= INT8_MAX)
+		w = 1;
+	else if (h[0] >= INT16_MIN && h[1] <= INT16_MAX)
+		w = 2;
+	else if (h[0] >= INT32_MIN && h[1] <= INT32_MAX)
+		w = 4;
+	else
+		return CBGPU_OK;
+	owned = rel->owns[col];
+	rc = rel_reencode(rel, col, w);
+	if (rc || !owned)
+		return rc;
+	{
+		cudaMemPool_t pool;
+
+		CB_CUDA(ctx, cudaStreamSynchronize(ctx->stream));
+		CB_CUDA(ctx, cudaDeviceGetDefaultMemPool(&pool, ctx->device));
+		CB_CUDA(ctx, cudaMemPoolTrimTo(pool, 0));
+	}
+	return CBGPU_OK;
+}
+
 extern "C" int
 cbgpu_rel_load_column(cbgpu_rel *rel, int32_t col, const void *host, const uint8_t *nulls)
 {
 	cbgpu_ctx  *ctx = rel->ctx;
+	int			rc;
 
 	if (col < 0 || col >= rel->ncols)
 		return cb_fail(ctx, CBGPU_ERR_INVALID, "cbgpu_rel_load_column: bad column%s %lld", "", col);
 	if (rel->nrows == 0)
 		return CBGPU_OK;
+	rc = rel_set_storage(rel, col, cb_type_w(rel->types[col]));
+	if (rc)
+		return rc;
 	CB_CUDA(ctx, cudaMemcpyAsync(rel->data[col], host, (size_t) rel->nrows * cb_type_w(rel->types[col]),
 								 cudaMemcpyHostToDevice, ctx->stream));
 	if (nulls)
@@ -479,7 +710,7 @@
 		cudaFreeAsync(rel->nulls[col], ctx->stream);
 		rel->nulls[col] = NULL;
 	}
-	return CBGPU_OK;
+	return cbgpu_rel_narrow_column(rel, col);
 }
 
 template <typename NARROW, typename WIDE>
@@ -510,6 +741,20 @@
 		return cb_fail(ctx, CBGPU_ERR_INVALID, "cbgpu_rel_load_column_narrow: a %s%lld-byte host column cannot be widened into this column", "", host_width);
 	if (rel->nrows == 0)
 		return CBGPU_OK;
+	if (rel->types[col] == CB_NUMERIC)
+	{
+		int			rc = rel_set_storage(rel, col, host_width);
+
+		if (rc)
+			return rc;
+		if (rel->nulls[col])
+		{
+			cudaFreeAsync(rel->nulls[col], ctx->stream);
+			rel->nulls[col] = NULL;
+		}
+		CB_CUDA(ctx, cudaMemcpyAsync(rel->data[col], host, (size_t) rel->nrows * host_width, cudaMemcpyHostToDevice, ctx->stream));
+		return CBGPU_OK;
+	}
 	CB_CUDA(ctx, cudaMallocAsync(&stage, (size_t) rel->nrows * host_width, ctx->stream));
 	CB_CUDA(ctx, cudaMemcpyAsync(stage, host, (size_t) rel->nrows * host_width, cudaMemcpyHostToDevice, ctx->stream));
 	blocks = ctx->sm_count * 8;
@@ -543,10 +788,39 @@
 	if (col < 0 || col >= rel->ncols || lo < 0 || hi > rel->nrows || lo > hi)
 		return cb_fail(ctx, CBGPU_ERR_INVALID, "cbgpu_rel_read_column: bad range%s %lld", "", lo);
 	w = cb_type_w(rel->types[col]);
-	if (hi > lo)
-	{
+	if (hi > lo && rel->width[col] != w)
+	{
+		const int64_t chunk = (int64_t) 4 << 20;
+		const int	sw = rel->width[col];
+		int64_t    *stage;
+
+		CB_CUDA(ctx, cudaMallocAsync(&stage, (size_t) (hi - lo < chunk ? hi - lo : chunk) * 8, ctx->stream));
+		for (int64_t at = lo; at < hi; at += chunk)
+		{
+			const int64_t n = hi - at < chunk ? hi - at : chunk;
+			int			rc = cb_widen_copy(ctx, stage, (const char *) rel->data[col] + (size_t) at * sw, sw, n);
+
+			cudaError_t e = cudaSuccess;
+
+			if (rc == CBGPU_OK)
+				e = cudaMemcpyAsync((int64_t *) host + (at - lo), stage, (size_t) n * 8, cudaMemcpyDeviceToHost, ctx->stream);
+			if (rc == CBGPU_OK && e == cudaSuccess)
+				e = cudaStreamSynchronize(ctx->stream);
+			if (rc || e != cudaSuccess)
+			{
+				cudaFreeAsync(stage, ctx->stream);
+				if (rc)
+					return rc;
+				CB_CUDA(ctx, e);
+			}
+		}
+		CB_CUDA(ctx, cudaFreeAsync(stage, ctx->stream));
+	}
+	else if (hi > lo)
 		CB_CUDA(ctx, cudaMemcpyAsync(host, (char *) rel->data[col] + (size_t) lo * w, (size_t) (hi - lo) * w,
 									 cudaMemcpyDeviceToHost, ctx->stream));
+	if (hi > lo)
+	{
 		if (nulls)
 		{
 			if (rel->nulls[col])
@@ -564,6 +838,7 @@
 	const void *data[CB_MAX_COLS_REL];
 	const uint8_t *nulls[CB_MAX_COLS_REL];
 	int32_t		types[CB_MAX_COLS_REL];
+	int32_t		width[CB_MAX_COLS_REL];
 	int32_t		ncols;
 	const uint32_t *idx;
 	int64_t		n;
@@ -582,7 +857,7 @@
 		const int	c = (int) (i % p.ncols);
 		const uint32_t row = p.idx ? p.idx[r] : (uint32_t) r;
 
-		p.out[i] = cb_load_widen(p.data[c], p.types[c], row);
+		p.out[i] = cb_load_widen(p.data[c], p.types[c], p.width[c], row);
 		p.outnull[i] = p.nulls[c] ? p.nulls[c][row] : (uint8_t) 0;
 	}
 }
@@ -609,6 +884,7 @@
 		p.data[c] = rel->data[c];
 		p.nulls[c] = rel->nulls[c];
 		p.types[c] = rel->types[c];
+		p.width[c] = rel->width[c];
 	}
 	p.ncols = rel->ncols;
 	p.n = n;
@@ -717,7 +993,7 @@
 	size_t		b = 0;
 
 	for (int i = 0; i < rel->ncols; i++)
-		b += (size_t) rel->nrows * cb_type_w(rel->types[i]);
+		b += (size_t) rel->nrows * rel->width[i];
 	return b;
 }
 
@@ -792,11 +1068,24 @@
 	for (int c = 0; c < dst->ncols; c++)
 	{
 		int			w = cb_type_w(dst->types[c]);
+		int			sw,
+					rc;
 
 		if (dst->types[c] != src->types[c])
 			return cb_fail(ctx, CBGPU_ERR_INVALID, "cbgpu_rel_copy_rows: column %s%lld type mismatch", "", c);
-		CB_CUDA(ctx, cudaMemcpyAsync((char *) dst->data[c] + (size_t) dst_lo * w, (char *) src->data[c] + (size_t) src_lo * w,
-									 (size_t) n * w, cudaMemcpyDeviceToDevice, ctx->stream));
+		rc = cb_rel_restore_wide(dst, c);
+		if (rc)
+			return rc;
+		sw = src->width[c];
+		if (sw != w)
+		{
+			rc = cb_widen_copy(ctx, (int64_t *) dst->data[c] + dst_lo, (const char *) src->data[c] + (size_t) src_lo * sw, sw, n);
+			if (rc)
+				return rc;
+		}
+		else
+			CB_CUDA(ctx, cudaMemcpyAsync((char *) dst->data[c] + (size_t) dst_lo * w, (char *) src->data[c] + (size_t) src_lo * w,
+										 (size_t) n * w, cudaMemcpyDeviceToDevice, ctx->stream));
 		if (src->nulls[c])
 		{
 			int			rc = cbgpu_rel_add_nullmap(dst, c);
@@ -816,6 +1105,7 @@
 	const uint8_t *snull[CB_MAX_COLS_REL];
 	uint8_t    *dnull[CB_MAX_COLS_REL];
 	int32_t		width[CB_MAX_COLS_REL];
+	int32_t		swidth[CB_MAX_COLS_REL];
 	int32_t		ncols;
 	int64_t		n;
 	const uint32_t *idx;
@@ -833,7 +1123,9 @@
 
 		for (int c = 0; c < p.ncols; c++)
 		{
-			switch (p.width[c])
+			if (p.swidth[c] != p.width[c])
+				((long long *) p.dst[c])[i] = cb_load_widen(p.src[c], CB_NUMERIC, p.swidth[c], r);
+			else switch (p.width[c])
 			{
 				case 1: ((uint8_t *) p.dst[c])[i] = ((const uint8_t *) p.src[c])[r]; break;
 				case 4: ((uint32_t *) p.dst[c])[i] = ((const uint32_t *) p.src[c])[r]; break;
@@ -861,6 +1153,12 @@
 	{
 		if (dst->types[c] != src->types[c])
 			return cb_fail(ctx, CBGPU_ERR_INVALID, "cbgpu_rel_take_rows: column %s%lld type mismatch", "", c);
+		{
+			int			rc = cb_rel_restore_wide(dst, c);
+
+			if (rc)
+				return rc;
+		}
 		if (src->nulls[c])
 		{
 			int			rc = cbgpu_rel_add_nullmap(dst, c);
@@ -873,6 +1171,7 @@
 		p.snull[c] = src->nulls[c];
 		p.dnull[c] = src->nulls[c] ? dst->nulls[c] : NULL;
 		p.width[c] = cb_type_w(dst->types[c]);
+		p.swidth[c] = src->width[c];
 	}
 	p.ncols = dst->ncols;
 	p.n = n;
@@ -923,3 +1222,28 @@
 	dst->dict_n[dcol] = src->dict_n[scol] > 0 ? -src->dict_n[scol] : (src->dict_n[scol] < 0 ? src->dict_n[scol] : -1);
 	return CBGPU_OK;
 }
+
+int
+cb_rel_wide_copy(cbgpu_rel *rel, cbgpu_rel **out)
+{
+	bool		narrow = false;
+	int			rc;
+
+	*out = NULL;
+	for (int c = 0; c < rel->ncols; c++)
+		narrow |= rel->width[c] != cb_type_w(rel->types[c]);
+	if (!narrow)
+		return CBGPU_OK;
+	rc = cbgpu_rel_create(rel->ctx, rel->nrows, rel->ncols, rel->types, rel->dscales, out);
+	if (rc == CBGPU_OK)
+		rc = cbgpu_rel_copy_rows(*out, 0, rel, 0, rel->nrows);
+	for (int c = 0; c < rel->ncols && rc == CBGPU_OK; c++)
+		if (rel->dict_hash[c])
+			rc = cbgpu_rel_share_dict_hash(*out, c, rel, c);
+	if (rc && *out)
+	{
+		cbgpu_rel_free(*out);
+		*out = NULL;
+	}
+	return rc;
+}
diff --git a/cloudberry_b200/csrc/exec/cb_aocs_load.c b/cloudberry_b200/csrc/exec/cb_aocs_load.c
--- a/cloudberry_b200/csrc/exec/cb_aocs_load.c
+++ b/cloudberry_b200/csrc/exec/cb_aocs_load.c
@@ -170,6 +170,9 @@
 			snprintf(err, errsz, "%s visimap: %s", basepath, cbgpu_last_error(ctx));
 	}
 	free(first);
+	if (rc == CBGPU_OK && nrows > 0 && row_offset + nrows == cbgpu_rel_nrows(rel))
+		for (int c = 0; c < ncols && rc == CBGPU_OK; c++)
+			rc = cbgpu_rel_narrow_column(rel, cols[c].relcol);
 	if (rc == CBGPU_OK && nrows_out)
 		*nrows_out = nrows < 0 ? 0 : nrows;
 	return rc;
diff --git a/cloudberry_b200/csrc/exec/cb_exec.c b/cloudberry_b200/csrc/exec/cb_exec.c
--- a/cloudberry_b200/csrc/exec/cb_exec.c
+++ b/cloudberry_b200/csrc/exec/cb_exec.c
@@ -223,6 +223,7 @@
 	c->nulls = cbgpu_rel_nulls_dev(rel, col);
 	c->dict_hash = cbgpu_rel_dict_hash_dev(rel, col);
 	c->type = cbgpu_rel_col_type(rel, col);
+	c->width = cbgpu_rel_col_width(rel, col);
 	c->src = src;
 	s->col_rel[s->pipe.ncols] = rel;
 	s->col_idx[s->pipe.ncols] = col;
diff --git a/cloudberry_b200/csrc/gen.cu b/cloudberry_b200/csrc/gen.cu
--- a/cloudberry_b200/csrc/gen.cu
+++ b/cloudberry_b200/csrc/gen.cu
@@ -98,6 +98,12 @@
 
 	if (rc)
 		return rc;
+	for (int c = 2; c <= 5; c++)
+	{
+		rc = cb_rel_restore_wide(rel, c);
+		if (rc)
+			return rc;
+	}
 	g.orderkey = (int64_t *) rel->data[0];
 	g.suppkey = (int32_t *) rel->data[1];
 	g.quantity = (int64_t *) rel->data[2];
@@ -116,6 +122,12 @@
 		return CBGPU_OK;
 	k_gen_lineitem<<<gen_blocks(ctx, rel->nrows), 256, 0, ctx->stream>>>(g);
 	CB_LAUNCHED(ctx, "k_gen_lineitem");
+	for (int c = 2; c <= 5; c++)
+	{
+		rc = cbgpu_rel_narrow_column(rel, c);
+		if (rc)
+			return rc;
+	}
 	return CBGPU_OK;
 }
 
diff --git a/cloudberry_b200/csrc/hashtable.cu b/cloudberry_b200/csrc/hashtable.cu
--- a/cloudberry_b200/csrc/hashtable.cu
+++ b/cloudberry_b200/csrc/hashtable.cu
@@ -18,7 +18,7 @@
 	{
 		if (ht.keynulls[k] && ht.keynulls[k][row])
 			return false;
-		int64_t		v = cb_load_widen(ht.keydata[k], ht.keytype[k], row);
+		int64_t		v = cb_load_widen(ht.keydata[k], ht.keytype[k], cb_full_w(ht.keytype[k]), row);
 
 		if (k == 0)
 			*key0 = v;
@@ -32,7 +32,7 @@
 ht_keys_equal_rows(const HtDev &ht, uint32_t ra, uint32_t rb)
 {
 	for (int k = 0; k < ht.nkeys; k++)
-		if (cb_load_widen(ht.keydata[k], ht.keytype[k], ra) != cb_load_widen(ht.keydata[k], ht.keytype[k], rb))
+		if (cb_load_widen(ht.keydata[k], ht.keytype[k], cb_full_w(ht.keytype[k]), ra) != cb_load_widen(ht.keydata[k], ht.keytype[k], cb_full_w(ht.keytype[k]), rb))
 			return false;
 	return true;
 }
@@ -436,7 +436,7 @@
 		{
 			if (p.onulls[k] && p.onulls[k][row])
 				isnull = true;
-			key[k] = cb_load_widen(p.okey[k], p.otype[k], row);
+			key[k] = cb_load_widen(p.okey[k], p.otype[k], cb_full_w(p.otype[k]), row);
 			h = pg_hash_combine(h, jh_hash_datum(p.otype[k], key[k], p.odict[k]), false);
 		}
 		if (!isnull && p.ht.bloom)
@@ -467,7 +467,7 @@
 					bool		eq = true;
 
 					for (int k = 0; k < p.ht.nkeys && !p.ht.keyslot; k++)
-						if (cb_load_widen(p.ht.keydata[k], p.ht.keytype[k], irow) != key[k])
+						if (cb_load_widen(p.ht.keydata[k], p.ht.keytype[k], cb_full_w(p.ht.keytype[k]), irow) != key[k])
 							eq = false;
 					if (eq)
 					{
diff --git a/cloudberry_b200/csrc/motion.cu b/cloudberry_b200/csrc/motion.cu
--- a/cloudberry_b200/csrc/motion.cu
+++ b/cloudberry_b200/csrc/motion.cu
@@ -516,6 +516,19 @@
 extern "C" int
 cbgpu_motion_redistribute(cbgpu_motion *m, cbgpu_rel *send, const int64_t *counts, const int64_t *offsets, cbgpu_rel **recv)
 {
+	{
+		cbgpu_rel  *wide;
+		int			wrc = cb_rel_wide_copy(send, &wide);
+
+		if (wrc)
+			return wrc;
+		if (wide)
+		{
+			wrc = cbgpu_motion_redistribute(m, wide, counts, offsets, recv);
+			cbgpu_rel_free(wide);
+			return wrc;
+		}
+	}
 	int			n = m->nranks;
 	int64_t    *matrix;
 	int64_t		send_off[64], send_cnt[64], recv_off[64], recv_cnt[64];
@@ -1116,6 +1129,19 @@
 extern "C" int
 cbgpu_motion_gather(cbgpu_motion *m, int root, cbgpu_rel *send, int64_t nrows, cbgpu_rel **recv)
 {
+	{
+		cbgpu_rel  *wide;
+		int			wrc = cb_rel_wide_copy(send, &wide);
+
+		if (wrc)
+			return wrc;
+		if (wide)
+		{
+			wrc = cbgpu_motion_gather(m, root, wide, nrows, recv);
+			cbgpu_rel_free(wide);
+			return wrc;
+		}
+	}
 	int			n = m->nranks;
 	int64_t    *matrix;
 	int64_t		mine[64] = {0}, send_off[64], send_cnt[64], recv_off[64], recv_cnt[64];
@@ -1156,6 +1182,19 @@
 extern "C" int
 cbgpu_motion_broadcast(cbgpu_motion *m, cbgpu_rel *send, int64_t nrows, cbgpu_rel **recv)
 {
+	{
+		cbgpu_rel  *wide;
+		int			wrc = cb_rel_wide_copy(send, &wide);
+
+		if (wrc)
+			return wrc;
+		if (wide)
+		{
+			wrc = cbgpu_motion_broadcast(m, wide, nrows, recv);
+			cbgpu_rel_free(wide);
+			return wrc;
+		}
+	}
 	int			n = m->nranks;
 	int64_t    *matrix;
 	int64_t		mine[64] = {0}, send_off[64], send_cnt[64], recv_off[64], recv_cnt[64];
diff --git a/cloudberry_b200/csrc/pipeline.cu b/cloudberry_b200/csrc/pipeline.cu
--- a/cloudberry_b200/csrc/pipeline.cu
+++ b/cloudberry_b200/csrc/pipeline.cu
@@ -20,7 +20,10 @@
 	for (int c = 0; c < p->ncols; c++)
 	{
 		d->cols[c] = p->cols[c];
-		if (p->cols[c].src < 0 || p->cols[c].src >= CBP_MAX_SRC || cb_type_w(p->cols[c].type) == 0)
+		const int	w = p->cols[c].width;
+
+		if (p->cols[c].src < 0 || p->cols[c].src >= CBP_MAX_SRC || cb_type_w(p->cols[c].type) == 0 ||
+			(w != cb_type_w(p->cols[c].type) && (p->cols[c].type != CB_NUMERIC || (w != 1 && w != 2 && w != 4))))
 			return cb_fail(ctx, CBGPU_ERR_INVALID, "pipeline column %s%lld malformed", "", c);
 	}
 	d->nops = p->nops;
@@ -316,7 +319,7 @@
 		if (c.nulls && c.nulls[r])
 			n = true;
 		else
-			v = cb_load_widen(c.data, c.type, r);
+			v = cb_load_widen(c.data, c.type, c.width, r);
 	}
 	*isnull = n;
 	return v;
@@ -544,7 +547,7 @@
 
 							irow = (uint32_t) e;
 							for (int k = 0; k < pr.nkeys && !pr.ht.keyslot; k++)
-								if (cb_load_widen(pr.ht.keydata[k], pr.ht.keytype[k], irow) != key[k])
+								if (cb_load_widen(pr.ht.keydata[k], pr.ht.keytype[k], cb_full_w(pr.ht.keytype[k]), irow) != key[k])
 									eq = false;
 							if (eq)
 							{
@@ -589,7 +592,7 @@
 							if (c.nulls && c.nulls[r])
 								isnull = true;
 							else
-								v = cb_load_widen(c.data, c.type, r);
+								v = cb_load_widen(c.data, c.type, c.width, r);
 						}
 						st[sp] = v;
 						snull = isnull ? (snull | (1ull << sp)) : (snull & ~(1ull << sp));
diff --git a/cloudberry_b200/csrc/probe_chain.cu b/cloudberry_b200/csrc/probe_chain.cu
--- a/cloudberry_b200/csrc/probe_chain.cu
+++ b/cloudberry_b200/csrc/probe_chain.cu
@@ -24,7 +24,8 @@
 	const void *data;
 	const uint32_t *dict;
 	int32_t		type;
-	int32_t		src;
+	int16_t		width;
+	int16_t		src;
 };
 
 struct PcFilter
@@ -129,7 +130,7 @@
 __device__ __forceinline__ int64_t
 pc_load(const PcCol &c, const PcQ &Q, uint32_t e)
 {
-	return cb_load_widen(c.data, c.type, pc_row(Q, c.src, e));
+	return cb_load_widen(c.data, c.type, c.width, pc_row(Q, c.src, e));
 }
 
 __device__ __forceinline__ uint32_t
@@ -172,7 +173,7 @@
 	if (KIND == 1)
 		return pr.key[0].src == 0 ? ldg_stream_s64((const long long *) pr.key[0].data + row, pol_stream)
 			: __ldg((const long long *) pr.key[0].data + row);
-	return cb_load_widen(pr.key[0].data, pr.key[0].type, row);
+	return cb_load_widen(pr.key[0].data, pr.key[0].type, pr.key[0].width, row);
 }
 
 template <int KIND>
@@ -305,8 +306,8 @@
 					{
 						const uint32_t r = (uint32_t) x;
 
-						if (cb_load_widen(pr.ht.keydata[0], pr.ht.keytype[0], r) == k0 &&
-							(KIND != 2 || pr.nkeys < 2 || cb_load_widen(pr.ht.keydata[1], pr.ht.keytype[1], r) == k1))
+						if (cb_load_widen(pr.ht.keydata[0], pr.ht.keytype[0], cb_full_w(pr.ht.keytype[0]), r) == k0 &&
+							(KIND != 2 || pr.nkeys < 2 || cb_load_widen(pr.ht.keydata[1], pr.ht.keytype[1], cb_full_w(pr.ht.keytype[1]), r) == k1))
 						{
 							found = true;
 							irow[u] = r;
@@ -405,8 +406,8 @@
 				{
 					const uint32_t r = (uint32_t) x;
 
-					if (cb_load_widen(pr.ht.keydata[0], pr.ht.keytype[0], r) == k0[u] &&
-						(KIND != 2 || pr.nkeys < 2 || cb_load_widen(pr.ht.keydata[1], pr.ht.keytype[1], r) == k1[u]))
+					if (cb_load_widen(pr.ht.keydata[0], pr.ht.keytype[0], cb_full_w(pr.ht.keytype[0]), r) == k0[u] &&
+						(KIND != 2 || pr.nkeys < 2 || cb_load_widen(pr.ht.keydata[1], pr.ht.keytype[1], cb_full_w(pr.ht.keytype[1]), r) == k1[u]))
 					{
 						found = true;
 						irow[u] = r;
@@ -1391,7 +1392,8 @@
 	out->data = p->cols[c].data;
 	out->dict = p->cols[c].dict_hash;
 	out->type = p->cols[c].type;
-	out->src = p->cols[c].src == 0 ? 0 : p->cols[c].src - base + 1;
+	out->width = (int16_t) p->cols[c].width;
+	out->src = (int16_t) (p->cols[c].src == 0 ? 0 : p->cols[c].src - base + 1);
 	return true;
 }
 
@@ -1430,7 +1432,7 @@
 
 			for (int i = 0; i < B.red_nkeys[m]; i++)
 			{
-				kv[i] = cb_load_widen(B.red_key[m][i].data, B.red_key[m][i].type, (uint32_t) r);
+				kv[i] = cb_load_widen(B.red_key[m][i].data, B.red_key[m][i].type, B.red_key[m][i].width, (uint32_t) r);
 				h = pg_hash_combine(h, jh_hash_datum(B.red_keytype[m][i], kv[i], B.red_key[m][i].dict), false);
 			}
 			uint32_t	pos = h & T.mask;
@@ -1445,8 +1447,8 @@
 				{
 					const uint32_t ir = (uint32_t) e;
 
-					if (T.keyslot || (cb_load_widen(T.keydata[0], T.keytype[0], ir) == kv[0] &&
-									  (B.red_nkeys[m] < 2 || cb_load_widen(T.keydata[1], T.keytype[1], ir) == kv[1])))
+					if (T.keyslot || (cb_load_widen(T.keydata[0], T.keytype[0], cb_full_w(T.keytype[0]), ir) == kv[0] &&
+									  (B.red_nkeys[m] < 2 || cb_load_widen(T.keydata[1], T.keytype[1], cb_full_w(T.keytype[1]), ir) == kv[1])))
 					{
 						found = true;
 						break;
@@ -1461,7 +1463,7 @@
 		if (ok && B.bloom)
 		{
 			uint32_t	w;
-			const int64_t kv = cb_load_widen(B.self.keydata[B.kc], B.self.keytype[B.kc], (uint32_t) r);
+			const int64_t kv = cb_load_widen(B.self.keydata[B.kc], B.self.keytype[B.kc], cb_full_w(B.self.keytype[B.kc]), (uint32_t) r);
 			const uint32_t bits = ht_bloom_bits(pg_hash_combine(0u, jh_hash_datum(B.hashtype, kv, NULL), false), &w, B.mask);
 
 			atomicOr(B.bloom + w, bits);
diff --git a/cloudberry_b200/csrc/scan_agg.cu b/cloudberry_b200/csrc/scan_agg.cu
--- a/cloudberry_b200/csrc/scan_agg.cu
+++ b/cloudberry_b200/csrc/scan_agg.cu
@@ -6,10 +6,14 @@
 struct SmallAggParams
 {
 	int64_t		nrows;
-	const long long *colA;
-	const long long *colB;
-	const long long *colC;
-	const long long *colD;
+	const void *colA;
+	const void *colB;
+	const void *colC;
+	const void *colD;
+	int32_t		wa, wb, wc, wd;
+	int32_t		off_a, off_b, off_c, off_d, off_f, off_k0, off_k1;
+	int32_t		stage_bytes;
+	int32_t		nstages;
 	long long	k,
 				k2;
 	const int32_t *fcol;
@@ -80,19 +84,25 @@
 }
 
 #define SA_TILE 896
-#define SA_STAGES 5
+#define SA_SMEM (5 * SA_TILE * 38)
+#define SA_MAXSTAGES 16
+#define SA_WT(a, b, c, d) ((a) | (b) << 4 | (c) << 8 | (d) << 12)
+#define SA_WT_LINEITEM SA_WT(2, 4, 1, 1)
 #define SA_NCONS(G) ((G) <= 4 ? 448 : 224)
 
-struct __align__(128) SaStage
-{
-	long long	a[SA_TILE];
-	long long	b[SA_TILE];
-	long long	c[SA_TILE];
-	long long	d[SA_TILE];
-	int32_t		f[SA_TILE];
-	uint8_t		k0[SA_TILE];
-	uint8_t		k1[SA_TILE];
-};
+__device__ __forceinline__ long long
+sa_ld(const unsigned char *st, int off, int w, int r)
+{
+	const unsigned char *p = st + off;
+
+	if (w == 1)
+		return (signed char) p[r];
+	if (w == 2)
+		return ((const short *) p)[r];
+	if (w == 4)
+		return ((const int *) p)[r];
+	return ((const long long *) p)[r];
+}
 
 template <int G>
 struct SaState
@@ -106,19 +116,20 @@
 
 template <int G, int MASK, bool NARROW, int SHAPE, bool CHECK>
 __device__ __forceinline__ void
-sa_row(const SmallAggParams &P, SaState<G> &S, unsigned *gkeys, const SaStage *st, int r, int rows, int64_t r0)
+sa_row(const SmallAggParams &P, SaState<G> &S, unsigned *gkeys, const unsigned char *st, int r, int rows, int64_t r0)
 {
 	const bool	hasF = SHAPE ? true : P.fcol != NULL;
-	const bool	hasK0 = SHAPE == 1 ? true : (SHAPE == 2 ? false : P.key0 != NULL);
-	const bool	hasK1 = SHAPE == 1 ? true : (SHAPE == 2 ? false : P.key1 != NULL);
+	const bool	hasK0 = (SHAPE == 1 || SHAPE == 3) ? true : (SHAPE == 2 ? false : P.key0 != NULL);
+	const bool	hasK1 = (SHAPE == 1 || SHAPE == 3) ? true : (SHAPE == 2 ? false : P.key1 != NULL);
 	bool		pass = true;
-	long long	a = (MASK & 1) ? st->a[r] : 0;
-	long long	b = st->b[r];
-	long long	c = st->c[r];
-	long long	d = (MASK & 0x28) ? st->d[r] : 0;
-	int32_t		f = hasF ? st->f[r] : P.flo;
-	unsigned	k0 = hasK0 ? st->k0[r] : 0;
-	unsigned	k1 = hasK1 ? st->k1[r] : 0;
+	constexpr int WT = SHAPE == 1 ? SA_WT_LINEITEM : 0;
+	long long	a = (MASK & 1) ? sa_ld(st, P.off_a, WT ? (WT & 15) : P.wa, r) : 0;
+	long long	b = sa_ld(st, P.off_b, WT ? ((WT >> 4) & 15) : P.wb, r);
+	long long	c = sa_ld(st, P.off_c, WT ? ((WT >> 8) & 15) : P.wc, r);
+	long long	d = (MASK & 0x28) ? sa_ld(st, P.off_d, WT ? ((WT >> 12) & 15) : P.wd, r) : 0;
+	int32_t		f = hasF ? ((const int32_t *) (st + P.off_f))[r] : P.flo;
+	unsigned	k0 = hasK0 ? st[P.off_k0 + r] : 0;
+	unsigned	k1 = hasK1 ? st[P.off_k1 + r] : 0;
 
 	if (CHECK)
 	{
@@ -184,9 +195,8 @@
 k_scan_agg_small(const __grid_constant__ SmallAggParams P)
 {
 	extern __shared__ __align__(128) unsigned char smem_raw[];
-	SaStage    *stages = (SaStage *) smem_raw;
-	__shared__ uint64_t full_bar[SA_STAGES];
-	__shared__ uint64_t empty_bar[SA_STAGES];
+	__shared__ uint64_t full_bar[SA_MAXSTAGES];
+	__shared__ uint64_t empty_bar[SA_MAXSTAGES];
 	__shared__ unsigned gkeys[G];
 	__shared__ unsigned long long red[G][SA_NSUM + 1][2];
 	constexpr int NCONS = SA_NCONS(G);
@@ -197,7 +207,7 @@
 
 	if (threadIdx.x == 0)
 	{
-		for (int s = 0; s < SA_STAGES; s++)
+		for (int s = 0; s < P.nstages; s++)
 		{
 			mbar_init(&full_bar[s], 1);
 			mbar_init(&empty_bar[s], NCONS / 32);
@@ -225,52 +235,54 @@
 	{
 		if (lane == 0)
 		{
-			int			it = 0;
-
-			for (int64_t t = blockIdx.x; t < ntiles; t += gridDim.x, it++)
-			{
-				const int	s = it % SA_STAGES;
-				const unsigned ph = (it / SA_STAGES) & 1;
+			int			s = 0;
+			unsigned	ph = 0;
+
+			for (int64_t t = blockIdx.x; t < ntiles; t += gridDim.x)
+			{
 				const int64_t r0 = t * SA_TILE;
 				const int64_t rows = P.nrows - r0 < SA_TILE ? P.nrows - r0 : SA_TILE;
-				const unsigned b8 = (unsigned) (rows * 8 + 15) & ~15u;
-				const unsigned b4 = (unsigned) (rows * 4 + 15) & ~15u;
-				const unsigned b1 = (unsigned) (rows + 15) & ~15u;
+#define SA_BYTES(w) ((unsigned) (rows * (w) + 15) & ~15u)
 				const bool	wantA = (MASK & 1) != 0;
 				const bool	wantD = (MASK & 0x28) != 0;
-				unsigned	total = 2 * b8 + (wantA ? b8 : 0) + (wantD ? b8 : 0) + (P.fcol ? b4 : 0) +
-					(P.key0 ? b1 : 0) + (P.key1 ? b1 : 0);
-				SaStage    *st = &stages[s];
+				unsigned	total = SA_BYTES(P.wb) + SA_BYTES(P.wc) + (wantA ? SA_BYTES(P.wa) : 0) + (wantD ? SA_BYTES(P.wd) : 0) +
+					(P.fcol ? SA_BYTES(4) : 0) + (P.key0 ? SA_BYTES(1) : 0) + (P.key1 ? SA_BYTES(1) : 0);
+				unsigned char *st = smem_raw + (size_t) s * P.stage_bytes;
 
 				mbar_wait(&empty_bar[s], ph ^ 1);
 				mbar_expect_tx(&full_bar[s], total);
-				tma_load_1d(st->b, P.colB + r0, b8, &full_bar[s]);
-				tma_load_1d(st->c, P.colC + r0, b8, &full_bar[s]);
+				tma_load_1d(st + P.off_b, (const char *) P.colB + r0 * P.wb, SA_BYTES(P.wb), &full_bar[s]);
+				tma_load_1d(st + P.off_c, (const char *) P.colC + r0 * P.wc, SA_BYTES(P.wc), &full_bar[s]);
 				if (wantA)
-					tma_load_1d(st->a, P.colA + r0, b8, &full_bar[s]);
+					tma_load_1d(st + P.off_a, (const char *) P.colA + r0 * P.wa, SA_BYTES(P.wa), &full_bar[s]);
 				if (wantD)
-					tma_load_1d(st->d, P.colD + r0, b8, &full_bar[s]);
+					tma_load_1d(st + P.off_d, (const char *) P.colD + r0 * P.wd, SA_BYTES(P.wd), &full_bar[s]);
 				if (P.fcol)
-					tma_load_1d(st->f, P.fcol + r0, b4, &full_bar[s]);
+					tma_load_1d(st + P.off_f, P.fcol + r0, SA_BYTES(4), &full_bar[s]);
 				if (P.key0)
-					tma_load_1d(st->k0, P.key0 + r0, b1, &full_bar[s]);
+					tma_load_1d(st + P.off_k0, P.key0 + r0, SA_BYTES(1), &full_bar[s]);
 				if (P.key1)
-					tma_load_1d(st->k1, P.key1 + r0, b1, &full_bar[s]);
+					tma_load_1d(st + P.off_k1, P.key1 + r0, SA_BYTES(1), &full_bar[s]);
+#undef SA_BYTES
+				if (++s == P.nstages)
+				{
+					s = 0;
+					ph ^= 1;
+				}
 			}
 		}
 	}
 	else
 	{
 		const int	ct = threadIdx.x - 32;
-		int			it = 0;
-
-		for (int64_t t = blockIdx.x; t < ntiles; t += gridDim.x, it++)
-		{
-			const int	s = it % SA_STAGES;
-			const unsigned ph = (it / SA_STAGES) & 1;
+		int			s = 0;
+		unsigned	ph = 0;
+
+		for (int64_t t = blockIdx.x; t < ntiles; t += gridDim.x)
+		{
 			const int64_t r0 = t * SA_TILE;
 			const int	rows = (int) (P.nrows - r0 < SA_TILE ? P.nrows - r0 : SA_TILE);
-			const SaStage *st = &stages[s];
+			const unsigned char *st = smem_raw + (size_t) s * P.stage_bytes;
 
 			mbar_wait(&full_bar[s], ph);
 			if (rows == SA_TILE && !P.visimap)
@@ -288,6 +300,11 @@
 			__syncwarp();
 			if (lane == 0)
 				mbar_arrive(&empty_bar[s]);
+			if (++s == P.nstages)
+			{
+				s = 0;
+				ph ^= 1;
+			}
 		}
 	}
 
@@ -413,6 +430,13 @@
 col_plain(const CbPipeline *p, int c, int width)
 {
 	return p->cols[c].src == 0 && p->cols[c].nulls == NULL && cb_type_w(p->cols[c].type) == width &&
+		p->cols[c].width == width && p->cols[c].type != CB_FLOAT8;
+}
+
+static bool
+col_plain_int(const CbPipeline *p, int c)
+{
+	return p->cols[c].src == 0 && p->cols[c].nulls == NULL && cb_type_w(p->cols[c].type) == 8 &&
 		p->cols[c].type != CB_FLOAT8;
 }
 
@@ -563,14 +587,18 @@
 		else
 			return CBGPU_OK;
 	}
-	if (!col_plain(p, colB, 8) || !col_plain(p, colC, 8) || (colA >= 0 && !col_plain(p, colA, 8)) ||
-		(colD >= 0 && !col_plain(p, colD, 8)))
+	if (!col_plain_int(p, colB) || !col_plain_int(p, colC) || (colA >= 0 && !col_plain_int(p, colA)) ||
+		(colD >= 0 && !col_plain_int(p, colD)))
 		return CBGPU_OK;
 	P.nrows = p->nrows;
-	P.colA = colA >= 0 ? (const long long *) p->cols[colA].data : NULL;
-	P.colB = (const long long *) p->cols[colB].data;
-	P.colC = (const long long *) p->cols[colC].data;
-	P.colD = colD >= 0 ? (const long long *) p->cols[colD].data : NULL;
+	P.colA = colA >= 0 ? p->cols[colA].data : NULL;
+	P.colB = p->cols[colB].data;
+	P.colC = p->cols[colC].data;
+	P.colD = colD >= 0 ? p->cols[colD].data : NULL;
+	P.wa = colA >= 0 ? p->cols[colA].width : 8;
+	P.wb = p->cols[colB].width;
+	P.wc = p->cols[colC].width;
+	P.wd = colD >= 0 ? p->cols[colD].width : 8;
 	P.k = k;
 	P.k2 = k2;
 	P.visimap = p->visimap;
@@ -597,11 +625,25 @@
 	if (mask < 0)
 		return CBGPU_OK;
 	const int	shape = (P.fcol && P.key0 && P.key1) ? 1 : ((P.fcol && !P.key0 && !P.key1) ? 2 : 0);
-
+	const int	wt = SA_WT(P.colA ? P.wa : 0, P.wb, P.wc, P.colD ? P.wd : 0);
+
+	{
+		int			off = 0;
+
+		P.off_b = off; off += SA_TILE * P.wb;
+		P.off_c = off; off += SA_TILE * P.wc;
+		P.off_a = off; off += P.colA ? SA_TILE * P.wa : 0;
+		P.off_d = off; off += P.colD ? SA_TILE * P.wd : 0;
+		P.off_f = off; off += P.fcol ? SA_TILE * 4 : 0;
+		P.off_k0 = off; off += P.key0 ? SA_TILE : 0;
+		P.off_k1 = off; off += P.key1 ? SA_TILE : 0;
+		P.stage_bytes = (off + 127) & ~127;
+		P.nstages = SA_SMEM / P.stage_bytes < SA_MAXSTAGES ? SA_SMEM / P.stage_bytes : SA_MAXSTAGES;
+	}
 	int		   *d_flags;
 	int64_t		ntiles = (p->nrows + SA_TILE - 1) / SA_TILE;
 	int			blocks = ctx->sm_count;
-	const size_t smem = sizeof(SaStage) * SA_STAGES;
+	const size_t smem = (size_t) P.stage_bytes * P.nstages;
 	int			G = 4;
 	bool		narrow = true;
 
@@ -642,7 +684,7 @@
 			static bool attr_done = false; \
 			if (!attr_done) \
 			{ \
-				CB_CUDA(ctx, cudaFuncSetAttribute(k_scan_agg_small<GG, MM, NN, SS>, cudaFuncAttributeMaxDynamicSharedMemorySize, (int) smem)); \
+				CB_CUDA(ctx, cudaFuncSetAttribute(k_scan_agg_small<GG, MM, NN, SS>, cudaFuncAttributeMaxDynamicSharedMemorySize, SA_SMEM)); \
 				attr_done = true; \
 			} \
 			k_scan_agg_small<GG, MM, NN, SS><<<blocks, SA_NCONS(GG) + 32, smem, ctx->stream>>>(P); \
@@ -652,7 +694,8 @@
 		} while (0)
 #define SA_PICK_SHAPE(MM, NN) \
 		do { \
-			if (shape == 1) SA_LAUNCH(4, MM, NN, 1); \
+			if (shape == 1 && wt == SA_WT_LINEITEM) SA_LAUNCH(4, MM, NN, 1); \
+			else if (shape == 1) SA_LAUNCH(4, MM, NN, 3); \
 			else if (shape == 2) SA_LAUNCH(4, MM, NN, 2); \
 			else SA_LAUNCH(4, MM, NN, 0); \
 		} while (0)
diff --git a/include/cbgpu.h b/include/cbgpu.h
--- a/include/cbgpu.h
+++ b/include/cbgpu.h
@@ -59,6 +59,8 @@
 int32_t		cbgpu_rel_col_dscale(const cbgpu_rel *rel, int32_t col);
 int			cbgpu_rel_load_column(cbgpu_rel *rel, int32_t col, const void *host, const uint8_t *nulls);
 int			cbgpu_rel_load_column_narrow(cbgpu_rel *rel, int32_t col, const void *host, int32_t host_width);
+int			cbgpu_rel_narrow_column(cbgpu_rel *rel, int32_t col);
+int32_t		cbgpu_rel_col_width(const cbgpu_rel *rel, int32_t col);
 int			cbgpu_rel_read_column(cbgpu_rel *rel, int32_t col, int64_t lo, int64_t hi, void *host, uint8_t *nulls);
 int			cbgpu_rel_set_visimap(cbgpu_rel *rel, const uint8_t *bits);
 int			cbgpu_rel_read_visimap(cbgpu_rel *rel, uint8_t *bits);
@@ -109,6 +111,7 @@
 	const uint32_t *dict_hash;
 	int32_t		type;
 	int32_t		src;
+	int32_t		width;
 } CbpColumn;
 
 typedef struct CbpProbe
```
